# Jaureguy760/HaploHyped-VarAwareML

Measured on AMD Instinct MI355X. Metric: variants/sec encode+compress, 3M-variant x 2.5k-sample VCF, higher is better.
Workload: dtype u8

## Files before the change

### haplohyped_varawareml_amd/_lib.py

```python
import ctypes as C
import os

HERE = os.path.dirname(os.path.abspath(__file__))
LIB_PATH = os.environ.get("HHGT_LIB") or os.path.join(HERE, "libhhgt.so")

OK = 0
BLOSC1 = 1
BLOSC2 = 2
N_STAGES = 16
STAGE_NAMES = ["index", "fixed", "encode", "general", "lz4", "frame", "decode", "onehot", "inflate", "pairs", "ld_transpose",
               "ld", "ld_prune", "ld_walk", "grm", "assoc"]


class HhgtError(RuntimeError):

    def __init__(self, code, msg):
        super().__init__(f"{msg} (hhgt rc={code})")
        self.code = code


class Layout(C.Structure):
    _fields_ = [("n_samples", C.c_int32), ("sc", C.c_int32), ("vc", C.c_int32), ("ring", C.c_int32),
                ("v_capacity", C.c_uint64)]


class Window(C.Structure):
    _fields_ = [("ref_ptr", C.c_uint64), ("ref_len", C.c_uint64), ("win_start", C.c_int64),
                ("var_start_ptr", C.c_uint64), ("var_ref_ptr", C.c_uint64), ("var_alt_ptr", C.c_uint64),
                ("geno_ptr", C.c_uint64), ("geno_first", C.c_uint32), ("var_lo", C.c_uint32),
                ("var_hi", C.c_uint32), ("reserved", C.c_uint32)]


class BlockSel(C.Structure):
    _fields_ = [("src_ptr", C.c_uint64), ("src_bytes", C.c_uint64), ("dst_off", C.c_uint64), ("block", C.c_uint32),
                ("lo", C.c_uint32), ("hi", C.c_uint32), ("reserved", C.c_uint32)]


class CountSel(C.Structure):
    _fields_ = [("src_ptr", C.c_uint64), ("src_bytes", C.c_uint64), ("row_mask", C.c_uint64), ("out_row", C.c_uint64),
                ("part", C.c_uint32), ("lo", C.c_uint32), ("hi", C.c_uint32), ("reserved", C.c_uint32)]


class SampleSel(C.Structure):
    _fields_ = [("src_ptr", C.c_uint64), ("src_bytes", C.c_uint64), ("row_mask", C.c_uint64), ("out_row", C.c_uint64),
                ("mask_word", C.c_uint64), ("part", C.c_uint32), ("lo", C.c_uint32), ("hi", C.c_uint32),
                ("reserved", C.c_uint32)]


class PlaneSel(C.Structure):
    _fields_ = [("src_ptr", C.c_uint64), ("src_bytes", C.c_uint64), ("row_mask", C.c_uint64), ("out_row", C.c_uint64),
                ("mask_word", C.c_uint64), ("out_word", C.c_uint64), ("part", C.c_uint32), ("lo", C.c_uint32),
                ("hi", C.c_uint32), ("reserved", C.c_uint32)]


class GatherSel(C.Structure):
    _fields_ = [("src_ptr", C.c_uint64), ("src_bytes", C.c_uint64), ("row_mask", C.c_uint64), ("out_row", C.c_uint64),
                ("mask_word", C.c_uint64), ("out_col", C.c_uint64), ("part", C.c_uint32), ("lo", C.c_uint32),
                ("hi", C.c_uint32), ("reserved", C.c_uint32)]


class EncodeStats(C.Structure):
    _fields_ = [(n, C.c_uint64) for n in (
        "n_lines", "n_records", "n_kept", "n_drop_region", "n_drop_filter", "n_haploid_padded",
        "n_malformed", "n_general_lines", "n_chrom_runs")]

    def asdict(self):
        return {n: int(getattr(self, n)) for n, _ in self._fields_}


RESULT_RUNS = 16


class EncodeResultRec(C.Structure):
    _fields_ = [("stats", EncodeStats), ("cursor_before", C.c_uint64), ("cursor_after", C.c_uint64),
                ("n_lines_over", C.c_uint64), ("err_density", C.c_uint64), ("run_first", C.c_uint64 * RESULT_RUNS),
                ("run_names", (C.c_char * 32) * RESULT_RUNS), ("v_capacity", C.c_uint64), ("done", C.c_uint32),
                ("reserved", C.c_uint32)]

    def chrom_runs(self):
        n = min(int(self.stats.n_chrom_runs), RESULT_RUNS)
        return [(int(self.run_first[i]), bytes(self.run_names[i]).split(b"\0")[0].decode()) for i in range(n)]


_vp, _u64, _u32, _i32, _str = C.c_void_p, C.c_uint64, C.c_uint32, C.c_int, C.c_char_p
_lay, _pu64, _pi32, _pvp = C.POINTER(Layout), C.POINTER(C.c_uint64), C.POINTER(C.c_int), C.POINTER(C.c_void_p)
PROTOTYPES = {
    "hhgt_version": (_str, []),
    "hhgt_last_error": (_str, []),
    "hhgt_device_count": (_i32, []),
    "hhgt_ctx_create": (_i32, [_i32, C.POINTER(_vp)]),
    "hhgt_ctx_destroy": (None, [_vp]),
    "hhgt_layout_bytes": (_u64, [_lay]),
    "hhgt_layout_offset": (_u64, [_lay, _u32, _u64]),
    "hhgt_encode_text": (_i32, [_vp, _vp, _u64, _str, _lay, _u64, _vp, _vp, _vp, _vp, _vp, C.POINTER(EncodeStats), _vp]),
    "hhgt_encode_text_async": (_i32, [_vp, _vp, _u64, _str, _lay, _vp, _u32, _vp, _vp, _vp, _vp, _vp, _vp, _vp]),
    "hhgt_encode_text_planes_async": (_i32, [_vp, _vp, _u64, _str, _lay, _vp, _u32, _vp, _vp, _vp, _vp, _vp, _vp, _vp, _vp]),
    "hhgt_encode_result_status": (_i32, [_vp]),
    "hhgt_encode_chrom_runs": (_i32, [_vp, _u32, _vp, _vp, C.POINTER(_u32)]),
    "hhgt_pad_tail": (_i32, [_vp, _lay, _u64, _u64, _u64, _vp, _vp]),
    "hhgt_pad_tail_cursor": (_i32, [_vp, _lay, _vp, _vp, _vp]),
    "hhgt_planes_bytes": (_u64, [_lay]),
    "hhgt_pad_tail_planes": (_i32, [_vp, _lay, _u64, _u64, _u64, _vp, _vp]),
    "hhgt_pad_tail_planes_cursor": (_i32, [_vp, _lay, _vp, _vp, _vp]),
    "hhgt_compress_planes": (_i32, [_vp, _lay, _vp, _vp, _u32, _u32, _i32, _vp, _u64, _vp, _pu64, _vp]),
    "hhgt_planes_expand": (_i32, [_vp, _lay, _vp, _vp, _u32, _u32, _vp, _vp]),
    "hhgt_set_clevel": (_i32, [_vp, _i32]),
    "hhgt_reserve": (_i32, [_vp, _u64, _u32, _u64, _u64, _i32, _i32]),
    "hhgt_set_keep_multiallelic": (_i32, [_vp, _i32]),
    "hhgt_set_index_mode": (_i32, [_vp, _i32]),
    "hhgt_stream_create": (_i32, [_vp, _i32, C.POINTER(_vp)]),
    "hhgt_stream_destroy": (_i32, [_vp, _vp]),
    "hhgt_set_frame_stream": (_i32, [_vp, _vp]),
    "hhgt_compress_bound": (_u64, [_u64, _u64, _i32, _i32]),
    "hhgt_compress_chunks": (_i32, [_vp, _vp, _u64, _u64, _i32, _i32, _i32, _vp, _u64, _vp, _pu64, _vp]),
    "hhgt_decompress_chunks": (_i32, [_vp, _vp, _vp, _u64, _u64, _i32, _i32, _vp, _pu64, _vp]),
    "hhgt_decompress_blocks": (_i32, [_vp, _vp, _u32, _u64, _i32, _i32, _vp, _pu64, _vp]),
    "hhgt_count_alleles": (_i32, [_vp, _vp, _u32, _u32, _u32, _i32, _i32, _vp, _u64, _pu64, _vp]),
    "hhgt_count_samples": (_i32, [_vp, _vp, _u32, _u32, _u32, _i32, _i32, _vp, _u64, _vp, _u64, _pu64, _vp]),
    "hhgt_genotype_planes": (_i32, [_vp, _vp, _u32, _u32, _u32, _i32, _i32, _vp, _u64, _vp, _u64, _u64, _pu64, _vp]),
    "hhgt_gather_calls": (_i32, [_vp, _vp, _u32, _u32, _u32, _i32, _i32, _vp, _u64, _vp, _u64, _vp, _i32, _vp, _u64, _u64, _u64,
                                 _pu64, _vp]),
    "hhgt_pair_counts": (_i32, [_vp, _vp, _u64, _u64, _u64, _u64, _vp, _vp]),
    "hhgt_grm": (_i32, [_vp, _vp, _u64, _u64, _u64, _u64, _vp, _vp, _vp]),
    "hhgt_variant_planes": (_i32, [_vp, _vp, _u64, _u64, _u64, _u64, _vp, _vp]),
    "hhgt_ld_counts": (_i32, [_vp, _vp, _u64, _u64, _u32, _vp, _vp]),
    "hhgt_ld_prune": (_i32, [_vp, _vp, _u64, _u32, C.c_double, _vp, _vp]),
    "hhgt_ld_decisions": (_i32, [_vp, _vp, _u64, _u32, C.c_double, _vp, C.c_int64, _vp, _vp]),
    "hhgt_ld_clump": (_i32, [_vp, _vp, _u64, _u32, _vp, _vp, _vp, C.POINTER(_u32), _vp]),
    "hhgt_assoc_sums": (_i32, [_vp, _vp, _u64, _u64, _vp, _u32, _vp, _vp]),
    "hhgt_logistic_fit": (_i32, [_vp, _vp, _u64, _u64, _vp, _vp, _u32, _vp, _vp, _vp, _vp]),
    "hhgt_score_sums": (_i32, [_vp, _vp, _u64, _u64, _u64, _u64, _vp, _u32, _vp, _vp]),
    "hhgt_bgzf_scan": (_i32, [_vp, _u64, _u64, _vp, _vp, _vp, _vp, _pu64, _pu64]),
    "hhgt_inflate_members": (_i32, [_vp, _vp, _u64, _vp, _vp, _vp, _vp, _u64, _vp, _u64, _vp, _vp, _pu64, _vp]),
    "hhgt_onehot_windows": (_i32, [_vp, _vp, _u32, _u32, _vp, _i32, _vp, _vp, _vp]),
    "hhgt_onehot_bases_u8": (_i32, [_vp, _vp, _u64, _vp, _i32, _vp, _vp]),
    "hhgt_profile_enable": (_i32, [_vp, _i32]),
    "hhgt_profile_reset": (_i32, [_vp]),
    "hhgt_profile_read": (_i32, [_vp, C.POINTER(C.c_double), _pu64]),
    "hhgt_synth_render_fixed": (_i32, [_vp, _vp, _u64, _vp, _vp, _vp, _vp, _vp, _u64, _u64, _str, _i32, _u64, _vp]),
    "hhgt_synth_render_mixed": (_i32, [_vp, _vp, _u64, _vp, _vp, _vp, _vp, _vp, _vp, _u64, _u64, _str, _i32, _u64, _vp]),
    "hhgt_synth_write_bgzf": (_i32, [_str, _vp, _u64, _i32, _i32]),
    "hhgt_reader_open": (_i32, [_str, _u64, _i32, _i32, _pvp]),
    "hhgt_reader_close": (None, [_vp]),
    "hhgt_reader_is_bgzf": (_i32, [_vp]),
    "hhgt_reader_next": (_i32, [_vp, _pvp, _pu64]),
    "hhgt_reader_acquire": (_i32, [_vp, _pvp, _pu64, _pi32, _pi32]),
    "hhgt_reader_release": (_i32, [_vp, _i32]),
    "hhgt_reader_copy_async": (_i32, [_vp, _vp, _u64, _vp, _vp]),
    "hhgt_reader_stats": (_i32, [_vp, _pu64, _pu64]),
    "hhgt_reader_trim_pool": (None, []),
    "hhgt_reader_prewarm": (_i32, [_u64, _i32]),
    "hhgt_effective_cpus": (_i32, []),
    "hhgt_crc32": (_u32, [_vp, _u64]),
    "hhgt_fast_inflate": (_i32, [_vp, _u64, _vp, _u64]),
}

_lib = None


def load():
    global _lib
    if _lib is not None:
        return _lib
    import torch
    if not os.path.exists(LIB_PATH):
        raise ImportError(
            f"{LIB_PATH} is missing. Build it with `python -m haplohyped_varawareml_amd.build` "
            "(hipcc, gfx950). There is no CPU fallback for this path.")
    L = C.CDLL(LIB_PATH)
    for name, (restype, argtypes) in PROTOTYPES.items():
        fn = getattr(L, name)
        fn.restype, fn.argtypes = restype, argtypes
    _lib = L
    return L


def check(rc):
    if rc != OK:
        raise HhgtError(rc, load().hhgt_last_error().decode(errors="replace"))
```

### haplohyped_varawareml_amd/csrc/api.hip

```cpp
#include "common.h"
#include <chrono>
#include <vector>
#include <stdarg.h>
#include <stdio.h>
#include <string.h>
#include <stdlib.h>

static thread_local char g_err[512] = "";

void hhgt_set_error(const char *fmt, ...)
{
    va_list ap;
    va_start(ap, fmt);
    vsnprintf(g_err, sizeof(g_err), fmt, ap);
    va_end(ap);
}

extern "C" const char *hhgt_last_error(void) { return g_err; }
extern "C" const char *hhgt_version(void) { return "hhgt 0.1 (gfx950)"; }

extern "C" int hhgt_device_count(void)
{
    int n = 0;
    if (hipGetDeviceCount(&n) != hipSuccess) return 0;
// ... 109 lines not shown
    return on_device(c, stream, work, [&](hipStream_t st) { return timed(c, st, stage, [&] { return launch(st); }); });
}

extern "C" int hhgt_ctx_create(int device, hhgt_ctx **out)
{
    if (!out) return HHGT_ERR_ARG;
    *out = nullptr;
    int n = hhgt_device_count();
    if (n <= 0 || device < 0 || device >= n) {
        hhgt_set_error("no usable HIP device (count=%d, requested=%d): libhhgt has no CPU path", n, device);
        return HHGT_ERR_NO_DEVICE;
    }
    HIP_TRY(hipSetDevice(device));
    hhgt_ctx *c = new hhgt_ctx();
    c->device = device;
    int rc = HHGT_OK;
    hipError_t e = hipGetDeviceProperties(&c->prop, device);
    if (e != hipSuccess) {
        hhgt_set_error("hipGetDeviceProperties failed: %s", hipGetErrorString(e));
        rc = HHGT_ERR_HIP;
    } else if (strncmp(c->prop.gcnArchName, "gfx950", 6) != 0) {
        hhgt_set_error("device %d is %s; libhhgt carries gfx950 code objects only", device, c->prop.gcnArchName);
        rc = HHGT_ERR_NO_DEVICE;
    }
    if (rc == HHGT_OK && (e = hipHostMalloc(reinterpret_cast<void **>(&c->h_counters), sizeof(DevCounters), hipHostMallocDefault)) != hipSuccess) {
        hhgt_set_error("hipHostMalloc failed: %s", hipGetErrorString(e));
        rc = HHGT_ERR_HIP;
    }
    if (rc == HHGT_OK && (e = hipHostMalloc(reinterpret_cast<void **>(&c->h_result_pinned), sizeof(hhgt_encode_result), hipHostMallocDefault)) != hipSuccess) {
        hhgt_set_error("hipHostMalloc failed: %s", hipGetErrorString(e));
        rc = HHGT_ERR_HIP;
    }
    if (rc == HHGT_OK) rc = c->counters.ensure(sizeof(DevCounters));
    if (rc != HHGT_OK) {
        hhgt_ctx_destroy(c);
        return rc;
    }
    *out = c;
    return HHGT_OK;
}

extern "C" void hhgt_ctx_destroy(hhgt_ctx *c)
{
    if (!c) return;
    hipSetDevice(c->device);
    hipDeviceSynchronize();
    c->enc.each([](DevBuf &b) { b.release(); });
    DevBuf *bufs[] = {&c->counters, &c->cursor, &c->dec_bad, &c->oh_ovl, &c->oh_lut, &c->crc_x2n, &c->ld_bits, &c->score_part, &c->clump_ws};
    for (DevBuf *b : bufs) b->release();
    for (auto &w : c->cw) {
        DevBuf *wb[] = {&w.lz_scratch, &w.lz_csize, &w.lz_flags, &w.fr_bsize, &w.fr_csize, &w.fr_flags};
        for (DevBuf *b : wb) b->release();
        if (w.lz_done) hipEventDestroy(w.lz_done);
        if (w.fr_done) hipEventDestroy(w.fr_done);
    }
    if (c->h_counters) hipHostFree(c->h_counters);
    if (c->h_result_pinned) hipHostFree(c->h_result_pinned);
    for (auto &p : c->pending) {
        hipEventDestroy(p.a);
        hipEventDestroy(p.b);
    }
    for (auto e : c->event_pool) hipEventDestroy(e);
    delete c;
}

static hipEvent_t get_event(hhgt_ctx *c)
{
    if (!c->event_pool.empty()) {
        hipEvent_t e = c->event_pool.back();
        c->event_pool.pop_back();
        return e;
    }
    hipEvent_t e;
    hipEventCreate(&e);
    return e;
}

StageTimer::StageTimer(hhgt_ctx *c, hipStream_t s, int stage_) : ctx(c), st(s), stage(stage_)
{
    if (ctx->profiling) {
        a = get_event(ctx);
        b = get_event(ctx);
        hipEventRecord(a, st);
    }
}

void StageTimer::stop()
{
    if (a) {
        hipEventRecord(b, st);
        ctx->pending.push_back({stage, a, b});
        a = b = nullptr;
    }
}

int hhgt_profile_collect(hhgt_ctx *c)
{
    for (auto &p : c->pending) {
        hipEventSynchronize(p.b);
        float ms = 0.f;
        if (hipEventElapsedTime(&ms, p.a, p.b) == hipSuccess) {
            c->stage_ms[p.stage] += ms;
            c->stage_launches[p.stage] += 1;
        }
        c->event_pool.push_back(p.a);
        c->event_pool.push_back(p.b);
    }
    c->pending.clear();
    return HHGT_OK;
}

extern "C" int hhgt_profile_enable(hhgt_ctx *c, int on)
{
    if (!c) return HHGT_ERR_ARG;
    c->profiling = on ? 1 : 0;
    return HHGT_OK;
}

extern "C" int hhgt_profile_reset(hhgt_ctx *c)
{
    if (!c) return HHGT_ERR_ARG;
    hhgt_profile_collect(c);
    for (int i = 0; i < HHGT_N_STAGES; ++i) {
        c->stage_ms[i] = 0;
        c->stage_launches[i] = 0;
    }
    return HHGT_OK;
}

extern "C" int hhgt_profile_read(hhgt_ctx *c, double *ms, uint64_t *launches)
{
    if (!c) return HHGT_ERR_ARG;
    hhgt_profile_collect(c);
    for (int i = 0; i < HHGT_N_STAGES; ++i) {
        if (ms) ms[i] = c->stage_ms[i];
        if (launches) launches[i] = c->stage_launches[i];
    }
    return HHGT_OK;
}

static int make_layout(const hhgt_layout *lay, LayoutDev *L)
{
    if (!lay || lay->n_samples < 0) {
        hhgt_set_error("layout: bad n_samples");
        return HHGT_ERR_ARG;
    }
    L->S = (uint32_t)lay->n_samples;
    L->v_capacity = lay->v_capacity;
    L->ring = 0;
    L->pad_ = 0;
    if (lay->ring < 0 || (lay->ring > 0 && (lay->vc <= 0 || lay->v_capacity != (uint64_t)lay->ring * (uint64_t)lay->vc))) {
        hhgt_set_error("layout: a ring needs vc > 0 and v_capacity == ring * vc");
        return HHGT_ERR_ARG;
    }
    L->ring = (uint32_t)lay->ring;
    if (lay->vc == 0) {
        L->Vc = lay->v_capacity ? lay->v_capacity : TILE_V;
    } else {
        L->Vc = (uint64_t)lay->vc;
    }
    if (L->Vc % TILE_V) {
        hhgt_set_error("layout: variants per chunk (%llu) must be a multiple of %d (dense: v_capacity)",
                       (unsigned long long)L->Vc, TILE_V);
        return HHGT_ERR_ARG;
    }
    if (lay->v_capacity % L->Vc) {
        hhgt_set_error("layout: v_capacity must be a multiple of vc");
        return HHGT_ERR_ARG;
    }
    if (lay->sc == 0) {
        L->Sc = L->S ? L->S : 1;
        L->sc_log2 = 31;
        L->n_sc = 1;
    } else {
        uint32_t sc = (uint32_t)lay->sc;
        if (sc & (sc - 1)) {
            hhgt_set_error("layout: sc must be a power of two");
            return HHGT_ERR_ARG;
        }
        L->Sc = sc;
        uint32_t lg = 0;
        while ((1u << lg) < sc) ++lg;
        L->sc_log2 = lg;
        L->n_sc = (L->S + sc - 1) / sc;
        if (L->n_sc == 0) L->n_sc = 1;
    }
    return HHGT_OK;
}

extern "C" uint64_t hhgt_layout_bytes(const hhgt_layout *lay)
{
    LayoutDev L;
    if (make_layout(lay, &L) != HHGT_OK) return 0;
    return (uint64_t)L.n_sc * L.Sc * L.v_capacity * 2ull;
}

extern "C" uint64_t hhgt_layout_offset(const hhgt_layout *lay, uint32_t s, uint64_t v)
{
    LayoutDev L;
    if (make_layout(lay, &L) != HHGT_OK) return ~0ull;
    return layout_offset(L, s, v);
}

static int parse_region_host(const char *region, RegionFilter *rf)
{
    memset(rf, 0, sizeof(*rf));
    if (!region || !*region) return HHGT_OK;
    const char *colon = strrchr(region, ':');
    size_t clen = strlen(region);
    if (colon && colon[1] >= '0' && colon[1] <= '9') {
        char *p;
        long long b = strtoll(colon + 1, &p, 10), e = 0x7fffffffffffffffLL;
        while (*p == ',') p++;
        if (*p == '-' && p[1]) e = strtoll(p + 1, &p, 10);
        clen = (size_t)(colon - region);
        rf->has_range = 1;
        rf->beg = b;
        rf->end = e;
    }
    if (clen == 0 || clen >= sizeof(rf->contig)) {
        hhgt_set_error("region '%s': contig name empty or longer than 63 bytes", region);
        return HHGT_ERR_ARG;
    }
    memcpy(rf->contig, region, clen);
    rf->contig_len = (int)clen;
    return HHGT_OK;
}

__global__ void k_encode_finish(DevCounters *cnt, uint64_t *cursor, const uint64_t *__restrict__ run_first,
                                const uint8_t *__restrict__ run_names, uint64_t v_capacity, hhgt_encode_result *res,
                                uint32_t *region_tot, uint32_t n_region_tot)
{
    const uint32_t t = threadIdx.x;
    const uint64_t before = *cursor;
    const uint64_t kept = cnt->n_kept;
    __syncthreads();
    if (t == 0) {
        *cursor = before + kept;
        cnt->cursor_after = before + kept;
        res->stats.n_lines = cnt->n_lines;
        res->stats.n_records = cnt->n_records;
        res->stats.n_kept = kept;
        res->stats.n_drop_region = cnt->n_drop_region;
        res->stats.n_drop_filter = cnt->n_drop_filter;
        res->stats.n_haploid_padded = cnt->n_haploid;
        res->stats.n_malformed = cnt->n_malformed;
        res->stats.n_general_lines = cnt->n_general;
        res->stats.n_chrom_runs = cnt->n_chrom_runs;
        res->cursor_before = before;
        res->cursor_after = before + kept;
        res->n_lines_over = cnt->err_lines;
        res->err_density = cnt->err_density;
        res->v_capacity = v_capacity;
        res->reserved = cnt->n_other > 0xFFFFFFFFull ? 0xFFFFFFFFu : (uint32_t)cnt->n_other;
    }
    const uint64_t n_runs = cnt->n_chrom_runs;
    if (t < HHGT_RESULT_RUNS) res->run_first[t] = t < n_runs ? run_first[t] : 0ull;
    for (uint32_t q = t; q < HHGT_RESULT_RUNS * 32u; q += blockDim.x)
        res->run_names[q >> 5][q & 31u] = (q >> 5) < n_runs ? (char)run_names[q] : 0;
    __threadfence_system();
    __syncthreads();
    if (t == 0) __hip_atomic_store(&res->done, 1u, __ATOMIC_RELEASE, __HIP_MEMORY_SCOPE_SYSTEM);
    if (t < sizeof(DevCounters) / 8u) reinterpret_cast<unsigned long long *>(cnt)[t] = 0ull;
    for (uint32_t q = t; q < n_region_tot; q += blockDim.x) region_tot[q] = 0u;
}

__global__ void k_set_u64(uint64_t *p, uint64_t v) { *p = v; }

static int encode_check_args(hhgt_ctx *c, const void *d_text, uint64_t nbytes, const hhgt_layout *lay, LayoutDev *L,
                             const char *region, RegionFilter *rf, void *d_G)
{
    TRY(make_layout(lay, L));
    if (nbytes >= 0xFFFFFFF0ull) {
        hhgt_set_error("encode: text block of %llu bytes; split it below 4 GiB at a line boundary",
                       (unsigned long long)nbytes);
        return HHGT_ERR_ARG;
    }
    if (nbytes && (!d_text || (reinterpret_cast<uintptr_t>(d_text) & 15u))) {
        hhgt_set_error("encode: d_text must be a 16-byte aligned device pointer");
        return HHGT_ERR_ARG;
    }
    if (L->S > 0 && !d_G) {
        hhgt_set_error("encode: d_G is NULL");
        return HHGT_ERR_ARG;
    }
    const int rc = parse_region_host(region, rf);
    rf->keep_multi = c->keep_multi;
    return rc;
}

static uint32_t index_regions(uint64_t nbytes) { return (uint32_t)((nbytes + 1 + INDEX_REGION - 1) / INDEX_REGION); }

static int encode_begin_clean(hhgt_ctx *c, DevCounters *cnt, hipStream_t st)
{
    if (!c->counters_clean) {
        HIP_TRY(hipMemsetAsync(cnt, 0, sizeof(DevCounters), st));
        if (c->enc.region_tot.p) HIP_TRY(hipMemsetAsync(c->enc.region_tot.p, 0, c->enc.region_tot.cap, st));
    }
    c->counters_clean = false;
    return HHGT_OK;
}

static int encode_stage_index(hhgt_ctx *c, const uint8_t *text, uint64_t nbytes, uint32_t n_regions, uint32_t min_line, uint32_t S,
                              DevCounters *cnt, hipStream_t st)
{
    EncodeWs &w = c->enc;
    TRY(w.ensure_index(n_regions, st));
    return launch_index_newlines(text, nbytes, w.slots.as<uint32_t>(), w.counts.as<uint32_t>(), w.region_tot.as<uint32_t>(), n_regions,
                                 min_line, S, c->index_mode, cnt, st);
}

static int encode_stage_rest(hhgt_ctx *c, const uint8_t *text, uint64_t nbytes, uint32_t n_regions, uint32_t max_lines,
                             const RegionFilter &rf, const LayoutDev &L, const uint64_t *d_cursor, void *d_G, void *d_P, uint32_t *d_start, uint32_t *d_stop,
                             uint8_t *d_ref, uint8_t *d_alt, DevCounters *cnt, hipStream_t st)
{
    EncodeWs &w = c->enc;
    TRY(w.ensure_lines(max_lines));
    const uint32_t *nl = w.nl.as<uint32_t>(), *d_nlines = w.n_lines.as<uint32_t>();
    const LineCols l = w.line_cols(max_lines);
    const KeptCols k = w.kept_cols();
    TRY(timed(c, st, HHGT_STAGE_INDEX, [&] {
        return launch_compact_newlines(w.slots.as<uint32_t>(), w.counts.as<uint32_t>(), w.region_tot.as<uint32_t>(), n_regions,
                                       w.nl.as<uint32_t>(), max_lines, w.n_lines.as<uint32_t>(), st);
    }));
    if (max_lines == 0) return HHGT_OK;
    TRY(timed(c, st, HHGT_STAGE_FIXED, [&] {
        TRY(launch_parse_fixed(text, nbytes, nl, d_nlines, max_lines, rf, L.S, l, c->index_mode, cnt, st));
        if (chain_scanned(max_lines))
            TRY(launch_scan_exclusive_u32_pair(l.keep, l.kidx, l.cnew, l.crun, max_lines, w.scan_tmp.as<uint32_t>(), w.scan_tmp.cap / 4, st));
        return launch_compact_kept(text, nbytes, nl, d_nlines, max_lines, l, k, MAX_CHROM_RUNS, d_cursor, L.v_capacity, L.ring,
                                   d_start, d_stop, d_ref, d_alt, cnt, d_P != nullptr, st);
    }));
    if (L.S == 0) return HHGT_OK;
    TRY(timed(c, st, HHGT_STAGE_ENCODE, [&] {
        return d_P ? launch_encode_planes(text, nbytes, k.soff, k.meta, max_lines, d_cursor, L, static_cast<uint8_t *>(d_P),
                                          static_cast<int8_t *>(d_G), k.redo_list, k.redo_flag, cnt, st)
                   : launch_encode_tiles(text, nbytes, k.soff, k.meta, max_lines, d_cursor, L, static_cast<int8_t *>(d_G),
                                         k.redo_list, k.redo_flag, cnt, st);
    }));
    return timed(c, st, HHGT_STAGE_GENERAL, [&] {
        return launch_encode_general(text, nbytes, k.soff, k.lend, k.meta, k.redo_list, d_cursor, L, static_cast<int8_t *>(d_G),
                                     static_cast<uint8_t *>(d_P), cnt, c->prop.multiProcessorCount, st);
    });
}

static hhgt_encode_result *result_on_device(const hhgt_ctx *c, hhgt_encode_result *h_result)
{
    hipPointerAttribute_t a;
    if (hipPointerGetAttributes(&a, h_result) != hipSuccess) {
        (void)hipGetLastError();
        return nullptr;
    }
    if (a.type != hipMemoryTypeHost || !a.devicePointer || a.device != c->device) return nullptr;
    return static_cast<hhgt_encode_result *>(a.devicePointer);
}

static int encode_finish(hhgt_ctx *c, uint64_t *d_cursor, const LayoutDev &L, DevCounters *cnt, uint32_t n_regions,
                         hhgt_encode_result *h_result, hipStream_t st)
{
    TRY(c->enc.ensure_runs());
    const KeptCols k = c->enc.kept_cols();
    hhgt_encode_result *staging = c->enc.result.as<hhgt_encode_result>();
    hhgt_encode_result *direct = h_result ? result_on_device(c, h_result) : nullptr;
    if (h_result) h_result->done = 0u;
    hipLaunchKernelGGL(k_encode_finish, dim3(1), dim3(256), 0, st, cnt, d_cursor, k.run_first, k.run_names,
                       L.ring ? 0ull : L.v_capacity, direct ? direct : staging, c->enc.region_tot.as<uint32_t>(),
                       c->enc.region_tot.p ? chain_groups(n_regions) : 0u);
    HIP_TRY(hipGetLastError());
    c->counters_clean = true;
    if (h_result && !direct) HIP_TRY(hipMemcpyAsync(h_result, staging, sizeof(hhgt_encode_result), hipMemcpyDeviceToHost, st));
    return HHGT_OK;
}

extern "C" int hhgt_encode_result_status(const hhgt_encode_result *r)
{
    if (!r) return HHGT_ERR_ARG;
    if (!r->done) {
        hhgt_set_error("encode: the result record is not complete yet (synchronise the stream first)");
        return HHGT_ERR_ARG;
    }
    if (r->err_density) {
        hhgt_set_error("encode: more than %u newlines inside one %u-byte region (not VCF text)", INDEX_CAP, INDEX_REGION);
        return HHGT_ERR_LINE_DENSITY;
    }
    if (r->n_lines_over) {
        hhgt_set_error("encode: %llu lines beyond max_lines were not encoded", (unsigned long long)r->n_lines_over);
        return HHGT_ERR_CAPACITY;
    }
    if (r->stats.n_malformed) {
        hhgt_set_error("Error parsing VCF file: %llu malformed record(s) (too few columns, bad POS, FORMAT without GT)",
                       (unsigned long long)r->stats.n_malformed);
        return HHGT_ERR_MALFORMED;
    }
    if (r->v_capacity && r->cursor_after > r->v_capacity) {
        hhgt_set_error("encode: %llu kept records at v_base %llu exceed v_capacity %llu",
                       (unsigned long long)r->stats.n_kept, (unsigned long long)r->cursor_before,
                       (unsigned long long)r->v_capacity);
        return HHGT_ERR_CAPACITY;
    }
    if (r->stats.n_chrom_runs > MAX_CHROM_RUNS) {
        hhgt_set_error("encode: %llu CHROM runs in one text block, more than the limit of %u (a run starts at every change of CHROM "
                       "and behind every empty or header line)",
                       (unsigned long long)r->stats.n_chrom_runs, MAX_CHROM_RUNS);
        return HHGT_ERR_CAPACITY;
    }
    return HHGT_OK;
}

static void empty_result(hhgt_encode_result *r)
{
    memset(r, 0, sizeof(*r));
    r->done = 1u;
}

static int planes_check_layout(const LayoutDev &L)
{
    if (L.Vc % 4096ull) {
        hhgt_set_error("planes: variants per chunk (%llu; dense: v_capacity) must be a multiple of 4096", (unsigned long long)L.Vc);
        return HHGT_ERR_ARG;
    }
    return HHGT_OK;
}

extern "C" uint64_t hhgt_planes_bytes(const hhgt_layout *lay)
{
    LayoutDev L;
    if (make_layout(lay, &L) != HHGT_OK || planes_check_layout(L) != HHGT_OK) return 0;
    return (uint64_t)L.n_sc * L.Sc * L.v_capacity / 2ull;
}

static int planes_columns(const hhgt_layout *lay, uint32_t col0, uint32_t n_cols, LayoutDev *L, PlanesGeom *pg)
{
    TRY(make_layout(lay, L));
    TRY(planes_check_layout(*L));
    if ((uint64_t)col0 + n_cols > L->v_capacity / L->Vc) {
        hhgt_set_error("planes: columns [%u, %u) outside the layout's %llu", col0, col0 + n_cols, (unsigned long long)(L->v_capacity / L->Vc));
        return HHGT_ERR_ARG;
    }
    *pg = planes_geom(*L, col0);
    return HHGT_OK;
}

static int pad_tail_begin(hhgt_ctx *c, const void *d_buf, const hhgt_layout *lay, bool planes, LayoutDev *L)
{
    if (!c || !d_buf) return HHGT_ERR_ARG;
    HIP_TRY(hipSetDevice(c->device));
    TRY(make_layout(lay, L));
    return planes ? planes_check_layout(*L) : HHGT_OK;
}

static int pad_tail_range(const LayoutDev &L, uint64_t v_end, uint64_t vcol_end)
{
    if (v_end > L.v_capacity || vcol_end > L.v_capacity / L.Vc) {
        hhgt_set_error("pad_tail: range outside the layout");
        return HHGT_ERR_ARG;
    }
    return HHGT_OK;
}

static int encode_async_impl(hhgt_ctx *c, const void *d_text, uint64_t nbytes, const char *region, const hhgt_layout *lay,
                             uint64_t *d_cursor, uint32_t max_lines, void *d_G, void *d_P, bool planes, uint32_t *d_start,
                             uint32_t *d_stop, uint8_t *d_ref, uint8_t *d_alt, hhgt_encode_result *h_result, void *stream)
{
    if (!c || !d_cursor) return HHGT_ERR_ARG;
    hipStream_t st = reinterpret_cast<hipStream_t>(stream);
    HIP_TRY(hipSetDevice(c->device));
    LayoutDev L;
    RegionFilter rf;
    TRY(encode_check_args(c, d_text, nbytes, lay, &L, region, &rf, planes ? d_P : d_G));
    if (planes) TRY(planes_check_layout(L));
    const uint8_t *text = static_cast<const uint8_t *>(d_text);
    DevCounters *cnt = c->counters.as<DevCounters>();
    TRY(encode_begin_clean(c, cnt, st));
    const uint32_t n_regions = index_regions(nbytes);
    if (nbytes) {
        TRY(timed(c, st, HHGT_STAGE_INDEX, [&] { return encode_stage_index(c, text, nbytes, n_regions, L.S ? 2u * L.S + 17u : 0u, L.S, cnt, st); }));
        TRY(encode_stage_rest(c, text, nbytes, n_regions, max_lines, rf, L, d_cursor, d_G, planes ? d_P : nullptr, d_start, d_stop, d_ref,
                              d_alt, cnt, st));
    }
    return encode_finish(c, d_cursor, L, cnt, n_regions, h_result, st);
}

extern "C" int hhgt_encode_text_async(hhgt_ctx *c, const void *d_text, uint64_t nbytes, const char *region,
                                      const hhgt_layout *lay, uint64_t *d_cursor, uint32_t max_lines, void *d_G,
                                      uint32_t *d_start, uint32_t *d_stop, uint8_t *d_ref, uint8_t *d_alt,
                                      hhgt_encode_result *h_result, void *stream)
{
    return encode_async_impl(c, d_text, nbytes, region, lay, d_cursor, max_lines, d_G, nullptr, false, d_start, d_stop, d_ref, d_alt,
                             h_result, stream);
}

extern "C" int hhgt_encode_text_planes_async(hhgt_ctx *c, const void *d_text, uint64_t nbytes, const char *region,
                                             const hhgt_layout *lay, uint64_t *d_cursor, uint32_t max_lines, void *d_P, void *d_G,
                                             uint32_t *d_start, uint32_t *d_stop, uint8_t *d_ref, uint8_t *d_alt,
                                             hhgt_encode_result *h_result, void *stream)
{
    return encode_async_impl(c, d_text, nbytes, region, lay, d_cursor, max_lines, d_G, d_P, true, d_start, d_stop, d_ref, d_alt,
                             h_result, stream);
}

extern "C" int hhgt_pad_tail_planes(hhgt_ctx *c, const hhgt_layout *lay, uint64_t v_end, uint64_t vcol_begin, uint64_t vcol_end,
                                    void *d_P, void *stream)
{
    LayoutDev L;
    TRY(pad_tail_begin(c, d_P, lay, true, &L));
    TRY(pad_tail_range(L, v_end, vcol_end));
    return launch_pad_tail_planes(L, v_end, vcol_begin, vcol_end, static_cast<uint8_t *>(d_P), reinterpret_cast<hipStream_t>(stream));
}

extern "C" int hhgt_pad_tail_planes_cursor(hhgt_ctx *c, const hhgt_layout *lay, const uint64_t *d_cursor, void *d_P, void *stream)
{
    LayoutDev L;
    if (!d_cursor) return HHGT_ERR_ARG;
    TRY(pad_tail_begin(c, d_P, lay, true, &L));
    return launch_pad_tail_planes_cursor(L, d_cursor, static_cast<uint8_t *>(d_P), reinterpret_cast<hipStream_t>(stream));
}

extern "C" int hhgt_planes_expand(hhgt_ctx *c, const hhgt_layout *lay, const void *d_P, const void *d_G, uint32_t col0, uint32_t n_cols,
                                  void *d_out, void *stream)
{
    if (!c || !d_P || !d_out) return HHGT_ERR_ARG;
    HIP_TRY(hipSetDevice(c->device));
    LayoutDev L;
    PlanesGeom pg;
    TRY(planes_columns(lay, col0, n_cols, &L, &pg));
    if (n_cols == 0) return HHGT_OK;
    return launch_planes_expand(L, static_cast<const uint8_t *>(d_P), static_cast<const uint8_t *>(d_G), col0, n_cols,
                                static_cast<uint8_t *>(d_out), reinterpret_cast<hipStream_t>(stream));
}

static int encode_text_once(hhgt_ctx *c, const void *d_text, uint64_t nbytes, const char *region, const hhgt_layout *lay, uint64_t v_base,
                            void *d_G, uint32_t *d_start, uint32_t *d_stop, uint8_t *d_ref, uint8_t *d_alt, hhgt_encode_stats *stats,
                            void *stream);

extern "C" int hhgt_encode_text(hhgt_ctx *c, const void *d_text, uint64_t nbytes, const char *region,
                                const hhgt_layout *lay, uint64_t v_base, void *d_G, uint32_t *d_start,
                                uint32_t *d_stop, uint8_t *d_ref, uint8_t *d_alt, hhgt_encode_stats *stats,
                                void *stream)
{
    int rc = encode_text_once(c, d_text, nbytes, region, lay, v_base, d_G, d_start, d_stop, d_ref, d_alt, stats, stream);
    if (rc == HHGT_ERR_MALFORMED && c && lay && lay->n_samples >= 760) {
        const int mode = c->index_mode < 0 ? index_mode_default() : c->index_mode;
        if (mode > 0) {
            const int saved = c->index_mode;
            c->index_mode = 0;
            rc = encode_text_once(c, d_text, nbytes, region, lay, v_base, d_G, d_start, d_stop, d_ref, d_alt, stats, stream);
            c->index_mode = saved;
        }
    }
    return rc;
}

static int encode_text_once(hhgt_ctx *c, const void *d_text, uint64_t nbytes, const char *region, const hhgt_layout *lay, uint64_t v_base,
                            void *d_G, uint32_t *d_start, uint32_t *d_stop, uint8_t *d_ref, uint8_t *d_alt, hhgt_encode_stats *stats,
                            void *stream)
{
    if (!c) return HHGT_ERR_ARG;
    hipStream_t st = reinterpret_cast<hipStream_t>(stream);
    HIP_TRY(hipSetDevice(c->device));
    if (stats) memset(stats, 0, sizeof(*stats));
    LayoutDev L;
    RegionFilter rf;
    TRY(encode_check_args(c, d_text, nbytes, lay, &L, region, &rf, d_G));
    c->run_first_kept.clear();
    c->run_names_host.clear();
    if (nbytes == 0) return HHGT_OK;

    const uint8_t *text = static_cast<const uint8_t *>(d_text);
    DevCounters *cnt = c->counters.as<DevCounters>();
    TRY(c->cursor.ensure(8));
    TRY(encode_begin_clean(c, cnt, st));
    hipLaunchKernelGGL(k_set_u64, dim3(1), dim3(1), 0, st, c->cursor.as<uint64_t>(), v_base);
    const uint32_t n_regions = index_regions(nbytes);
    uint32_t n_lines = 0;
    {
        StageTimer t(c, st, HHGT_STAGE_INDEX);
        TRY(encode_stage_index(c, text, nbytes, n_regions, L.S ? 2u * L.S + 17u : 0u, L.S, cnt, st));
        std::vector<uint32_t> totals(chain_groups(n_regions));
        c->h_counters->err_density = 0;
        HIP_TRY(hipMemcpyAsync(totals.data(), c->enc.region_tot.p, totals.size() * 4, hipMemcpyDeviceToHost, st));
        HIP_TRY(hipMemcpyAsync(&c->h_counters->err_density, &cnt->err_density, 8, hipMemcpyDeviceToHost, st));
        HIP_TRY(hipStreamSynchronize(st));
        t.stop();
        for (uint32_t x : totals) n_lines += x;
        if (c->h_counters->err_density) {
            hhgt_set_error("encode: more than %u newlines inside one %u-byte region (not VCF text)", INDEX_CAP,
                           INDEX_REGION);
            return HHGT_ERR_LINE_DENSITY;
        }
    }
    if (stats) stats->n_lines = n_lines;
    if (n_lines == 0) return HHGT_OK;
    TRY(encode_stage_rest(c, text, nbytes, n_regions, n_lines, rf, L, c->cursor.as<uint64_t>(), d_G, nullptr, d_start, d_stop, d_ref,
                          d_alt, cnt, st));
    TRY(encode_finish(c, c->cursor.as<uint64_t>(), L, cnt, n_regions, c->h_result_pinned, st));
    hhgt_encode_result *hr = &c->h_result;
    HIP_TRY(hipStreamSynchronize(st));
    *hr = *c->h_result_pinned;
    if (stats) *stats = hr->stats;
    TRY(hhgt_encode_result_status(hr));
    const uint32_t n_runs = (uint32_t)hr->stats.n_chrom_runs;
    if (n_runs) {
        std::vector<uint64_t> first(n_runs);
        std::vector<char> names((size_t)n_runs * 32);
        if (n_runs <= HHGT_RESULT_RUNS) {
            memcpy(first.data(), hr->run_first, n_runs * 8);
            memcpy(names.data(), hr->run_names, (size_t)n_runs * 32);
        } else {
            HIP_TRY(hipMemcpy(first.data(), c->enc.run_first.p, (size_t)n_runs * 8, hipMemcpyDeviceToHost));
            HIP_TRY(hipMemcpy(names.data(), c->enc.run_names.p, (size_t)n_runs * 32, hipMemcpyDeviceToHost));
        }
        for (uint32_t r = 0; r < n_runs; ++r) {
            c->run_first_kept.push_back(first[r]);
            c->run_names_host.emplace_back(names.data() + (size_t)r * 32, strnlen(names.data() + (size_t)r * 32, 31));
        }
    }
    return HHGT_OK;
}

extern "C" int hhgt_encode_chrom_runs(hhgt_ctx *c, uint32_t max_runs, uint64_t *first_kept, char *names,
                                      uint32_t *n_runs)
{
    if (!c || !n_runs) return HHGT_ERR_ARG;
    uint32_t n = (uint32_t)c->run_first_kept.size();
    *n_runs = n;
    if (n > max_runs) n = max_runs;
    for (uint32_t r = 0; r < n; ++r) {
        if (first_kept) first_kept[r] = c->run_first_kept[r];
        if (names) {
            memset(names + (size_t)r * 32, 0, 32);
            size_t l = c->run_names_host[r].size() < 31 ? c->run_names_host[r].size() : 31;
            memcpy(names + (size_t)r * 32, c->run_names_host[r].data(), l);
        }
    }
    return HHGT_OK;
}

extern "C" int hhgt_pad_tail(hhgt_ctx *c, const hhgt_layout *lay, uint64_t v_end, uint64_t vcol_begin,
                             uint64_t vcol_end, void *d_G, void *stream)
{
    LayoutDev L;
    TRY(pad_tail_begin(c, d_G, lay, false, &L));
    TRY(pad_tail_range(L, v_end, vcol_end));
    return launch_pad_tail(L, v_end, vcol_begin, vcol_end, static_cast<int8_t *>(d_G),
                           reinterpret_cast<hipStream_t>(stream));
}

extern "C" int hhgt_pad_tail_cursor(hhgt_ctx *c, const hhgt_layout *lay, const uint64_t *d_cursor, void *d_G, void *stream)
{
    LayoutDev L;
    if (!d_cursor) return HHGT_ERR_ARG;
    TRY(pad_tail_begin(c, d_G, lay, false, &L));
    return launch_pad_tail_cursor(L, d_cursor, static_cast<int8_t *>(d_G), reinterpret_cast<hipStream_t>(stream));
}

static int check_codec_args(uint64_t chunk_nbytes, int typesize, int blocksize, int format)
{
    if (typesize < 1 || typesize > 255 || blocksize < 16 || blocksize > 65536 || blocksize % typesize ||
        chunk_nbytes == 0 || chunk_nbytes >= 0x7fffffffull || (format != HHGT_BLOSC1 && format != HHGT_BLOSC2)) {
        hhgt_set_error("compress: bad arguments (chunk_nbytes=%llu typesize=%d blocksize=%d format=%d)",
                       (unsigned long long)chunk_nbytes, typesize, blocksize, format);
        return HHGT_ERR_ARG;
    }
    return HHGT_OK;
}

static int effective_blocksize(uint64_t chunk_nbytes, int typesize, int blocksize)
{
    if ((uint64_t)blocksize > chunk_nbytes) {
        blocksize = (int)chunk_nbytes;
        if (typesize > 1 && blocksize >= typesize) blocksize -= blocksize % typesize;
    }
    return blocksize > 0 ? blocksize : 1;
}

static int check_decode_block(int typesize, int blocksize)
{
    if (blocksize > 65536) {
        hhgt_set_error("decode: block of %d bytes x typesize %d does not fit LDS (blocks of at most 65536 bytes)",
                       blocksize, typesize);
        return HHGT_ERR_ARG;
    }
    return HHGT_OK;
}

static void codec_geometry(uint64_t chunk_nbytes, int typesize, int blocksize, uint32_t *nblocks, uint32_t *nwaves,
                           size_t *slot_bytes)
{
    const bool split = typesize >= 2 && typesize <= 16 && blocksize / typesize >= 128;
    *nblocks = (uint32_t)((chunk_nbytes + blocksize - 1) / blocksize);
    *nwaves = split ? (uint32_t)typesize : 1u;
    size_t max_stream = split ? (size_t)blocksize / typesize : (size_t)blocksize;
    if (split && chunk_nbytes % blocksize && chunk_nbytes % blocksize > max_stream) max_stream = chunk_nbytes % blocksize;
    *slot_bytes = lz4_slot_bytes((int)max_stream);
}

extern "C" uint64_t hhgt_compress_bound(uint64_t n_chunks, uint64_t chunk_nbytes, int typesize, int blocksize)
{
    if (check_codec_args(chunk_nbytes, typesize, blocksize, HHGT_BLOSC2) != HHGT_OK) return 0;
    return n_chunks * (chunk_nbytes + 32);
}

static int compress_impl(hhgt_ctx *c, const void *d_src, const void *d_planes, PlanesGeom pg, uint64_t n_chunks, uint64_t chunk_nbytes,
                         int typesize, int blocksize, int format, void *d_dst, uint64_t dst_cap,
                         uint64_t *d_chunk_off, uint64_t *total_bytes, void *stream)
{
    if (!c || (!d_src && !d_planes) || !d_dst || !d_chunk_off) return HHGT_ERR_ARG;
    hipStream_t st = reinterpret_cast<hipStream_t>(stream);
    HIP_TRY(hipSetDevice(c->device));
    TRY(check_codec_args(chunk_nbytes, typesize, blocksize, format));
    if (total_bytes) *total_bytes = 0;
    if (n_chunks == 0) return HHGT_OK;
    if (!total_bytes && dst_cap < n_chunks * (chunk_nbytes + 32)) {
        hhgt_set_error("compress: the asynchronous form (total_bytes == NULL) needs dst_cap >= hhgt_compress_bound() = %llu, got %llu",
                       (unsigned long long)(n_chunks * (chunk_nbytes + 32)), (unsigned long long)dst_cap);
        return HHGT_ERR_CAPACITY;
    }
    blocksize = effective_blocksize(chunk_nbytes, typesize, blocksize);
    uint32_t nblocks, nwaves;
    size_t slot;
    codec_geometry(chunk_nbytes, typesize, blocksize, &nblocks, &nwaves, &slot);
    hipStream_t fst = c->frame_stream ? c->frame_stream : st;
    hhgt_ctx::CodecWs &w = c->cw[c->frame_stream ? (c->cmp_seq++ & 1u) : 0u];
    TRY(w.ensure(n_chunks, nblocks, nwaves, slot));
    if (w.fr_pending) {
        HIP_TRY(hipStreamWaitEvent(st, w.fr_done, 0));
        w.fr_pending = false;
    }
    TRY(timed(c, st, HHGT_STAGE_LZ4, [&] {
        if (!w.lz_flags.p) {
            TRY(w.lz_flags.ensure(4));
            HIP_TRY(hipMemsetAsync(w.lz_flags.p, 0, 4, st));
        }
        if (++w.lz_tag == 0) w.lz_tag = 1;
        return launch_lz4_blocks(static_cast<const uint8_t *>(d_src), static_cast<const uint8_t *>(d_planes), pg, n_chunks, chunk_nbytes,
                                 typesize, blocksize, w.lz_scratch.as<uint8_t>(), slot, w.lz_csize.as<uint32_t>(), c->clevel,
                                 w.lz_flags.as<uint32_t>(), w.lz_tag, st);
    }));
    if (fst != st) {
        if (!w.lz_done) HIP_TRY(hipEventCreateWithFlags(&w.lz_done, hipEventDisableTiming));
        if (!w.fr_done) HIP_TRY(hipEventCreateWithFlags(&w.fr_done, hipEventDisableTiming));
        HIP_TRY(hipEventRecord(w.lz_done, st));
        HIP_TRY(hipStreamWaitEvent(fst, w.lz_done, 0));
    }
    TRY(timed(c, fst, HHGT_STAGE_FRAME, [&] {
        return launch_frame(w.lz_scratch.as<uint8_t>(), slot, w.lz_csize.as<uint32_t>(), static_cast<const uint8_t *>(d_src),
                            static_cast<const uint8_t *>(d_planes), pg, n_chunks, chunk_nbytes, typesize, blocksize, format,
                            w.fr_bsize.as<uint32_t>(), w.fr_csize.as<uint64_t>(), static_cast<uint8_t *>(d_dst), dst_cap, d_chunk_off,
                            w.fr_flags.as<uint32_t>(), fst);
    }));
    if (fst != st) {
        HIP_TRY(hipEventRecord(w.fr_done, fst));
        w.fr_pending = true;
        if (total_bytes) HIP_TRY(hipStreamWaitEvent(st, w.fr_done, 0));
    }
    if (total_bytes) {
        uint64_t tot = 0;
        HIP_TRY(hipMemcpyAsync(&tot, d_chunk_off + n_chunks, 8, hipMemcpyDeviceToHost, st));
        HIP_TRY(hipStreamSynchronize(st));
        *total_bytes = tot;
        if (tot > dst_cap) {
            hhgt_set_error("compress: need %llu bytes, dst_cap is %llu", (unsigned long long)tot,
                           (unsigned long long)dst_cap);
            return HHGT_ERR_CAPACITY;
        }
    }
    return HHGT_OK;
}

extern "C" int hhgt_compress_chunks(hhgt_ctx *c, const void *d_src, uint64_t n_chunks, uint64_t chunk_nbytes,
                                    int typesize, int blocksize, int format, void *d_dst, uint64_t dst_cap,
                                    uint64_t *d_chunk_off, uint64_t *total_bytes, void *stream)
{
    if (!d_src) return HHGT_ERR_ARG;
    return compress_impl(c, d_src, nullptr, PlanesGeom{0, 0, 0, 0}, n_chunks, chunk_nbytes, typesize, blocksize, format, d_dst, dst_cap,
                         d_chunk_off, total_bytes, stream);
}

extern "C" int hhgt_compress_planes(hhgt_ctx *c, const hhgt_layout *lay, const void *d_P, const void *d_G, uint32_t col0, uint32_t n_cols,
                                    int format, void *d_dst, uint64_t dst_cap, uint64_t *d_chunk_off, uint64_t *total_bytes,
                                    void *stream)
{
    if (!c || !d_P) return HHGT_ERR_ARG;
    LayoutDev L;
    PlanesGeom pg;
    TRY(planes_columns(lay, col0, n_cols, &L, &pg));
    const uint64_t chunk_nbytes = (uint64_t)L.Sc * L.Vc * 2ull, col_bytes = chunk_nbytes * L.n_sc;
    const uint8_t *g = d_G ? static_cast<const uint8_t *>(d_G) + (uint64_t)col0 * col_bytes : nullptr;
    return compress_impl(c, g, d_P, pg, (uint64_t)n_cols * L.n_sc, chunk_nbytes, 2, 8192, format, d_dst, dst_cap, d_chunk_off, total_bytes,
                         stream);
}

extern "C" int hhgt_reserve(hhgt_ctx *c, uint64_t text_bytes, uint32_t max_lines, uint64_t n_chunks, uint64_t chunk_nbytes, int typesize,
                            int blocksize)
{
    if (!c) return HHGT_ERR_ARG;
    HIP_TRY(hipSetDevice(c->device));
    if (text_bytes) {
        const uint32_t n_regions = index_regions(text_bytes);
        TRY(c->enc.ensure_index(n_regions, nullptr));
        TRY(c->enc.ensure_lines(max_lines));
        HIP_TRY(hipStreamSynchronize(nullptr));
    }
    if (n_chunks) {
        TRY(check_codec_args(chunk_nbytes, typesize, blocksize, HHGT_BLOSC2));
        blocksize = effective_blocksize(chunk_nbytes, typesize, blocksize);
        uint32_t nblocks, nwaves;
        size_t slot;
        codec_geometry(chunk_nbytes, typesize, blocksize, &nblocks, &nwaves, &slot);
        TRY(c->cw[0].ensure(n_chunks, nblocks, nwaves, slot));
    }
    return HHGT_OK;
}

extern "C" int hhgt_set_clevel(hhgt_ctx *c, int clevel)
{
    if (!c || clevel < 1 || clevel > 9) {
        hhgt_set_error("clevel must be 1..9");
        return HHGT_ERR_ARG;
    }
    c->clevel = clevel;
    return HHGT_OK;
}

extern "C" int hhgt_stream_create(hhgt_ctx *c, int kind, void **out)
{
    if (!c || !out || (kind != HHGT_STREAM_ENCODE && kind != HHGT_STREAM_COMPRESS && kind != HHGT_STREAM_FRAME)) {
        hhgt_set_error("hhgt_stream_create: bad arguments");
        return HHGT_ERR_ARG;
    }
    HIP_TRY(hipSetDevice(c->device));
    hipStream_t st = nullptr;
    if (kind == HHGT_STREAM_FRAME) {
        HIP_TRY(hipStreamCreateWithFlags(&st, hipStreamNonBlocking));
    } else if (kind == HHGT_STREAM_ENCODE) {
        int lo = 0, hi = 0;
        HIP_TRY(hipDeviceGetStreamPriorityRange(&lo, &hi));
        HIP_TRY(hipStreamCreateWithPriority(&st, hipStreamNonBlocking, hi));
    } else {
        const uint32_t n_cu = (uint32_t)c->prop.multiProcessorCount;
        uint32_t use = n_cu >= 128u ? (n_cu * 3u / 4u) / 32u * 32u : n_cu;
        if (const char *e = getenv("HHGT_COMPRESS_CUS")) {
            const int v = atoi(e);
            use = v <= 0 || (uint32_t)v >= n_cu ? n_cu : (uint32_t)v;
        }
        if (use >= n_cu) {
            HIP_TRY(hipStreamCreateWithFlags(&st, hipStreamNonBlocking));
        } else {
            std::vector<uint32_t> mask((n_cu + 31u) / 32u, 0u);
            for (uint32_t i = n_cu - use; i < n_cu; ++i) mask[i >> 5] |= 1u << (i & 31u);
            if (hipExtStreamCreateWithCUMask(&st, (uint32_t)mask.size(), mask.data()) != hipSuccess) {
                (void)hipGetLastError();
                st = nullptr;
                HIP_TRY(hipStreamCreateWithFlags(&st, hipStreamNonBlocking));
            }
        }
    }
    *out = st;
    return HHGT_OK;
}

extern "C" int hhgt_set_frame_stream(hhgt_ctx *c, void *stream)
{
    if (!c) return HHGT_ERR_ARG;
    HIP_TRY(hipSetDevice(c->device));
    if (c->frame_stream) HIP_TRY(hipStreamSynchronize(c->frame_stream));
    for (auto &w : c->cw) w.fr_pending = false;
    c->frame_stream = reinterpret_cast<hipStream_t>(stream);
    return HHGT_OK;
}

extern "C" int hhgt_stream_destroy(hhgt_ctx *c, void *stream)
{
    if (!c) return HHGT_ERR_ARG;
    if (stream) {
        HIP_TRY(hipSetDevice(c->device));
        if (reinterpret_cast<hipStream_t>(stream) == c->frame_stream) TRY(hhgt_set_frame_stream(c, nullptr));
        HIP_TRY(hipStreamDestroy(reinterpret_cast<hipStream_t>(stream)));
    }
    return HHGT_OK;
}

extern "C" int hhgt_set_index_mode(hhgt_ctx *c, int mode)
{
    if (!c || mode < -1 || mode > 2) {
        hhgt_set_error("index mode must be -1 (default), 0 (scan), 1 (hop) or 2 (walk)");
        return HHGT_ERR_ARG;
    }
    c->index_mode = mode;
    return HHGT_OK;
}

extern "C" int hhgt_set_keep_multiallelic(hhgt_ctx *c, int on)
{
    if (!c) return HHGT_ERR_ARG;
    c->keep_multi = on ? 1 : 0;
    return HHGT_OK;
}

__global__ void k_count_nonzero_u32(const uint32_t *__restrict__ v, uint64_t n, unsigned long long *out)
{
    uint64_t i = (uint64_t)blockIdx.x * blockDim.x + threadIdx.x;
    const unsigned long long m = __ballot(i < n && v[i] != 0u);
    if ((threadIdx.x & 63u) == 0u && m) atomicAdd(out, (unsigned long long)__builtin_popcountll(m));
}

extern "C" int hhgt_inflate_members(hhgt_ctx *c, const void *d_src, uint64_t src_bytes, const uint64_t *d_comp_off,
                                    const uint32_t *d_comp_len, const uint64_t *d_out_off, const uint32_t *d_isize,
                                    uint64_t n_members, void *d_dst, uint64_t dst_bytes, const uint32_t *d_crc32,
                                    uint32_t *d_status, uint64_t *n_bad, void *stream)
{
    if (!c || !d_src || !d_comp_off || !d_comp_len || !d_out_off || !d_isize || !d_status || (!d_dst && dst_bytes))
        return HHGT_ERR_ARG;
    hipStream_t st = reinterpret_cast<hipStream_t>(stream);
    HIP_TRY(hipSetDevice(c->device));
    if (n_bad) *n_bad = 0;
    if (n_members == 0) return HHGT_OK;
    if (d_crc32 && !c->crc_x2n_ready) {
        uint32_t t[32];
        crc32_x2n_table(t);
        TRY(c->crc_x2n.ensure(sizeof(t)));
        HIP_TRY(hipMemcpy(c->crc_x2n.p, t, sizeof(t), hipMemcpyHostToDevice));
        c->crc_x2n_ready = true;
    }
    TRY(timed(c, st, HHGT_STAGE_INFLATE, [&] {
        return launch_inflate(static_cast<const uint8_t *>(d_src), src_bytes, d_comp_off, d_comp_len, d_out_off, d_isize, n_members,
                              static_cast<uint8_t *>(d_dst), dst_bytes, d_status, d_crc32, c->crc_x2n.as<uint32_t>(), st);
    }));
    if (n_bad) {
        TRY(c->dec_bad.ensure(8));
        HIP_TRY(hipMemsetAsync(c->dec_bad.p, 0, 8, st));
        hipLaunchKernelGGL(k_count_nonzero_u32, dim3((uint32_t)((n_members + 255) / 256)), dim3(256), 0, st, d_status,
                           n_members, c->dec_bad.as<unsigned long long>());
        HIP_TRY(hipGetLastError());
        uint64_t nb = 0;
        HIP_TRY(hipMemcpyAsync(&nb, c->dec_bad.p, 8, hipMemcpyDeviceToHost, st));
        HIP_TRY(hipStreamSynchronize(st));
        *n_bad = nb;
    }
    return HHGT_OK;
}

template <typename Launch>
static int with_bad_counter(hhgt_ctx *c, hipStream_t st, uint64_t *n_bad, Launch launch)
{
    TRY(c->dec_bad.ensure(8));
    HIP_TRY(hipMemsetAsync(c->dec_bad.p, 0, 8, st));
    TRY(timed(c, st, HHGT_STAGE_DECODE, [&] { return launch(c->dec_bad.as<unsigned long long>()); }));
    if (n_bad) {
        uint64_t nb = 0;
        HIP_TRY(hipMemcpyAsync(&nb, c->dec_bad.p, 8, hipMemcpyDeviceToHost, st));
        HIP_TRY(hipStreamSynchronize(st));
        *n_bad = nb;
    }
    return HHGT_OK;
}

extern "C" int hhgt_decompress_chunks(hhgt_ctx *c, const void *d_src, const uint64_t *d_chunk_off, uint64_t n_chunks,
                                      uint64_t chunk_nbytes, int typesize, int blocksize, void *d_dst,
                                      uint64_t *n_bad, void *stream)
{
    if (!c || !d_src || !d_dst || !d_chunk_off) return HHGT_ERR_ARG;
    hipStream_t st = reinterpret_cast<hipStream_t>(stream);
    HIP_TRY(hipSetDevice(c->device));
    TRY(check_decode_block(typesize, blocksize));
    TRY(check_codec_args(chunk_nbytes, typesize, blocksize, HHGT_BLOSC2));
    if (n_bad) *n_bad = 0;
    if (n_chunks == 0) return HHGT_OK;
    blocksize = effective_blocksize(chunk_nbytes, typesize, blocksize);
    return with_bad_counter(c, st, n_bad, [&](unsigned long long *d_bad) {
        return launch_decode(static_cast<const uint8_t *>(d_src), d_chunk_off, n_chunks, chunk_nbytes, typesize, blocksize,
                             static_cast<uint8_t *>(d_dst), d_bad, st);
    });
}

extern "C" int hhgt_decompress_blocks(hhgt_ctx *c, const hhgt_block_sel *d_sel, uint32_t n_sel, uint64_t chunk_nbytes,
                                      int typesize, int blocksize, void *d_dst, uint64_t *n_bad, void *stream)
{
    TRY(check_not_null("decompress_blocks", c, !n_sel ? nullptr : !d_sel ? "selection array" : !d_dst ? "destination" : nullptr));
    hipStream_t st = reinterpret_cast<hipStream_t>(stream);
    HIP_TRY(hipSetDevice(c->device));
    TRY(check_decode_block(typesize, blocksize));
    TRY(check_codec_args(chunk_nbytes, typesize, blocksize, HHGT_BLOSC2));
    if (n_bad) *n_bad = 0;
    if (n_sel == 0) return HHGT_OK;
    blocksize = effective_blocksize(chunk_nbytes, typesize, blocksize);
    return with_bad_counter(c, st, n_bad, [&](unsigned long long *d_bad) {
        return launch_decode_sel(d_sel, n_sel, chunk_nbytes, typesize, blocksize, static_cast<uint8_t *>(d_dst), d_bad, st);
    });
}

static int check_row_kernel_args(const char *who, uint32_t sc, uint32_t vc, int typesize, int blocksize)
{
    if (typesize != 2) {
        hhgt_set_error("%s: typesize %d (only 2: one diploid int8 call)", who, typesize);
        return HHGT_ERR_ARG;
    }
    if (sc < 1 || sc > 64 || vc < 1) {
        hhgt_set_error("%s: chunk of %u samples x %u variants (1 to 64 samples)", who, sc, vc);
        return HHGT_ERR_ARG;
    }
    TRY(check_codec_args((uint64_t)sc * vc * 2u, typesize, blocksize, HHGT_BLOSC2));
    if (blocksize > 8192 || ((uint64_t)vc * 2u) % (uint64_t)blocksize) {
        hhgt_set_error("%s: blocksize %d does not cut a row of %u variants into whole blocks of at most 8192 bytes", who,
                       blocksize, vc);
        return HHGT_ERR_ARG;
    }
    return HHGT_OK;
}

template <typename Launch>
static int run_row_kernel(const char *who, const char *out, hhgt_ctx *c, const void *d_sel, uint32_t n_sel, const void *d_out,
                          uint32_t sc, uint32_t vc, int typesize, int blocksize, uint64_t *n_bad, void *stream, Launch launch)
{
    TRY(check_not_null(who, c, !n_sel ? nullptr : !d_sel ? "selection array" : !d_out ? out : nullptr));
    TRY(check_row_kernel_args(who, sc, vc, typesize, blocksize));
    hipStream_t st = reinterpret_cast<hipStream_t>(stream);
    HIP_TRY(hipSetDevice(c->device));
    if (n_bad) *n_bad = 0;
    if (n_sel == 0) return HHGT_OK;
    return with_bad_counter(c, st, n_bad, [&](unsigned long long *d_bad) { return launch(d_bad, st); });
}

extern "C" int hhgt_count_alleles(hhgt_ctx *c, const hhgt_count_sel *d_sel, uint32_t n_sel, uint32_t sc, uint32_t vc,
                                  int typesize, int blocksize, uint32_t *d_counts, uint64_t n_out, uint64_t *n_bad,
                                  void *stream)
{
    return run_row_kernel("count_alleles", "counts", c, d_sel, n_sel, d_counts, sc, vc, typesize, blocksize, n_bad, stream,
                          [&](unsigned long long *d_bad, hipStream_t st) {
                              return launch_count_alleles(d_sel, n_sel, sc, vc, blocksize, d_counts, n_out, d_bad, st);
                          });
}

extern "C" int hhgt_count_samples(hhgt_ctx *c, const hhgt_sample_sel *d_sel, uint32_t n_sel, uint32_t sc, uint32_t vc,
                                  int typesize, int blocksize, const uint32_t *d_vmask, uint64_t vmask_words,
                                  uint32_t *d_counts, uint64_t n_out, uint64_t *n_bad, void *stream)
{
    return run_row_kernel("count_samples", "counts", c, d_sel, n_sel, d_counts, sc, vc, typesize, blocksize, n_bad, stream,
                          [&](unsigned long long *d_bad, hipStream_t st) {
                              return launch_count_samples(d_sel, n_sel, sc, vc, blocksize, d_vmask, vmask_words, d_counts,
                                                          n_out, d_bad, st);
                          });
}

extern "C" int hhgt_genotype_planes(hhgt_ctx *c, const hhgt_plane_sel *d_sel, uint32_t n_sel, uint32_t sc, uint32_t vc,
                                    int typesize, int blocksize, const uint32_t *d_vmask, uint64_t vmask_words,
                                    uint32_t *d_planes, uint64_t n_rows, uint64_t row_words, uint64_t *n_bad,
                                    void *stream)
{
    return run_row_kernel("genotype_planes", "planes", c, d_sel, n_sel, d_planes, sc, vc, typesize, blocksize, n_bad, stream,
                          [&](unsigned long long *d_bad, hipStream_t st) {
                              return launch_genotype_planes(d_sel, n_sel, sc, vc, blocksize, d_vmask, vmask_words, d_planes,
                                                            n_rows, row_words, d_bad, st);
                          });
}

extern "C" int hhgt_gather_calls(hhgt_ctx *c, const hhgt_gather_sel *d_sel, uint32_t n_sel, uint32_t sc, uint32_t vc,
                                 int typesize, int blocksize, const uint32_t *d_vmask, uint64_t vmask_words,
                                 const uint32_t *d_row_map, uint64_t n_map, const void *d_values, int elem_bytes,
                                 void *d_out, uint64_t n_rows, uint64_t n_cols, uint64_t row_stride, uint64_t *n_bad,
                                 void *stream)
{
    const bool table = d_values != nullptr;
    if (table ? (elem_bytes != 1 && elem_bytes != 2 && elem_bytes != 4 && elem_bytes != 8) : elem_bytes != 2) {
        hhgt_set_error("gather_calls: elem_bytes %d (%s)", elem_bytes, table ? "1, 2, 4 or 8" : "2 without a table: an allele pair");
        return HHGT_ERR_ARG;
    }
    if (row_stride < n_cols) {
        hhgt_set_error("gather_calls: row_stride %llu below n_cols %llu", (unsigned long long)row_stride, (unsigned long long)n_cols);
        return HHGT_ERR_ARG;
    }
    const uintptr_t off = (uintptr_t)elem_bytes - 1u;
    if ((reinterpret_cast<uintptr_t>(d_out) & off) || (reinterpret_cast<uintptr_t>(d_values) & off)) {
        hhgt_set_error("gather_calls: %s not aligned to elem_bytes %d", (reinterpret_cast<uintptr_t>(d_out) & off) ? "d_out" : "d_values",
                       elem_bytes);
        return HHGT_ERR_ARG;
    }
    return run_row_kernel("gather_calls", "output", c, d_sel, n_sel, d_out, sc, vc, typesize, blocksize, n_bad, stream,
                          [&](unsigned long long *d_bad, hipStream_t st) {
                              return launch_gather_calls(d_sel, n_sel, sc, vc, blocksize, d_vmask, vmask_words, d_row_map, n_map,
                                                         d_values, elem_bytes, d_out, n_rows, n_cols, row_stride, d_bad, st);
                          });
}

template <typename Launch>
static int run_plane_kernel(const char *who, int stage, hhgt_ctx *c, const char *null_arg, const char *misaligned, uint64_t n_rows,
                            uint64_t row_words, uint64_t w_lo, uint64_t w_hi, uint64_t row_limit, void *stream, Launch launch)
{
    const bool work = n_rows && w_lo < w_hi;
    TRY(check_not_null(who, c, work ? null_arg : nullptr));
    if (w_lo > w_hi || w_hi > row_words || n_rows > row_limit) {
        hhgt_set_error("%s: words [%llu, %llu) of rows of %llu words, %llu rows", who, (unsigned long long)w_lo,
                       (unsigned long long)w_hi, (unsigned long long)row_words, (unsigned long long)n_rows);
        return HHGT_ERR_ARG;
    }
    if (misaligned) {
        hhgt_set_error("%s: %s", who, misaligned);
        return HHGT_ERR_ARG;
    }
    return launch_on_device(c, stream, stage, work, launch);
}

static bool off_alignment(const void *p, uintptr_t align) { return reinterpret_cast<uintptr_t>(p) & (align - 1u); }

extern "C" int hhgt_pair_counts(hhgt_ctx *c, const uint32_t *d_planes, uint64_t n_rows, uint64_t row_words, uint64_t w_lo,
                                uint64_t w_hi, uint32_t *d_table, void *stream)
{
    return run_plane_kernel("pair_counts", HHGT_STAGE_PAIRS, c, !d_planes ? "planes" : !d_table ? "table" : nullptr,
                            off_alignment(d_table, 16) ? "the table must be 16-byte aligned" : nullptr, n_rows, row_words, w_lo, w_hi,
                            64ull * 65535ull, stream, [&](hipStream_t st) {
                                return launch_pair_counts(d_planes, (uint32_t)n_rows, row_words, w_lo, w_hi, d_table, st);
                            });
}

extern "C" int hhgt_grm(hhgt_ctx *c, const uint32_t *d_planes, uint64_t n_rows, uint64_t row_words, uint64_t w_lo, uint64_t w_hi,
                        const float *d_z, double *d_table, void *stream)
{
    return run_plane_kernel("grm", HHGT_STAGE_GRM, c, !d_planes ? "planes" : !d_z ? "weights" : !d_table ? "table" : nullptr,
                            off_alignment(d_table, 8) || off_alignment(d_z, 16)
                                ? "the table must be 8-byte aligned, the weights 16-byte aligned" : nullptr,
                            n_rows, row_words, w_lo, w_hi, 64ull * 65535ull, stream, [&](hipStream_t st) {
                                return launch_grm(d_planes, (uint32_t)n_rows, row_words, w_lo, w_hi, d_z, d_table, st);
                            });
}

extern "C" int hhgt_variant_planes(hhgt_ctx *c, const uint32_t *d_planes, uint64_t n_rows, uint64_t row_words, uint64_t w_lo,
                                   uint64_t w_hi, uint32_t *d_vplanes, void *stream)
{
    return run_plane_kernel("variant_planes", HHGT_STAGE_LD_TRANSPOSE, c, !d_planes ? "planes" : !d_vplanes ? "variant planes" : nullptr,
                            nullptr, n_rows, row_words, w_lo, w_hi, 256ull * 65535ull, stream, [&](hipStream_t st) {
                                return launch_variant_planes(d_planes, (uint32_t)n_rows, row_words, w_lo, w_hi, d_vplanes, st);
                            });
}

static int check_ld_args(const char *who, hhgt_ctx *c, uint32_t window, const double *r2, const char *null_arg, const uint32_t *d_table)
{
    if (window < 1u || window > 1024u || (r2 && !(*r2 >= 0.0 && *r2 <= 1.0))) {
        if (r2)
            hhgt_set_error("%s: window %u, r2 %g (1 to 1024, 0 to 1)", who, window, *r2);
        else
            hhgt_set_error("%s: window %u (1 to 1024)", who, window);
        return HHGT_ERR_ARG;
    }
    TRY(check_not_null(who, c, null_arg));
    if (off_alignment(d_table, 32)) {
        hhgt_set_error("%s: the table must be 32-byte aligned", who);
        return HHGT_ERR_ARG;
    }
    return HHGT_OK;
}

extern "C" int hhgt_ld_counts(hhgt_ctx *c, const uint32_t *d_vplanes, uint64_t n_var, uint64_t sw, uint32_t window,
                              uint32_t *d_table, void *stream)
{
    const bool work = n_var && sw;
    TRY(check_ld_args("ld_counts", c, window, nullptr, !work ? nullptr : !d_vplanes ? "variant planes" : !d_table ? "table" : nullptr, d_table));
    return launch_on_device(c, stream, HHGT_STAGE_LD, work,
                            [&](hipStream_t st) { return launch_ld_counts(d_vplanes, n_var, sw, window, d_table, st); });
}

extern "C" int hhgt_ld_prune(hhgt_ctx *c, const uint32_t *d_table, uint64_t n_var, uint32_t window, double r2,
                             uint8_t *d_keep, void *stream)
{
    TRY(check_ld_args("ld_prune", c, window, &r2, !n_var ? nullptr : !d_table ? "table" : !d_keep ? "keep flags" : nullptr, d_table));
    return on_device(c, stream, n_var != 0, [&](hipStream_t st) {
        TRY(c->ld_bits.ensure((size_t)n_var * ld_walk_words(window) * sizeof(uint64_t)));
        uint64_t *bits = c->ld_bits.as<uint64_t>();
        TRY(timed(c, st, HHGT_STAGE_LD_PRUNE, [&] { return launch_ld_exceeds(d_table, n_var, window, r2, bits, st); }));
        return timed(c, st, HHGT_STAGE_LD_WALK, [&] { return launch_ld_walk(bits, n_var, window, d_keep, st); });
    });
}

static int check_clump_variants(const char *who, uint64_t n_var)
{
    if (n_var <= 0x7fffffffull) return HHGT_OK;
    hhgt_set_error("%s: %llu variants (below 2^31)", who, (unsigned long long)n_var);
    return HHGT_ERR_ARG;
}

extern "C" int hhgt_ld_decisions(hhgt_ctx *c, const uint32_t *d_table, uint64_t n_var, uint32_t window, double r2,
                                 const int64_t *d_pos, int64_t max_dist, uint64_t *d_bits, void *stream)
{
    TRY(check_ld_args("ld_decisions", c, window, &r2, !n_var ? nullptr : !d_table ? "table" : !d_bits ? "link bits" : nullptr, d_table));
    TRY(check_clump_variants("ld_decisions", n_var));
    if (max_dist < 0) {
        hhgt_set_error("ld_decisions: max_dist %lld (at least 0)", (long long)max_dist);
        return HHGT_ERR_ARG;
    }
    return launch_on_device(c, stream, HHGT_STAGE_LD_PRUNE, n_var != 0, [&](hipStream_t st) {
        return launch_ld_decisions(d_table, n_var, window, r2, d_pos, max_dist, d_bits, st);
    });
}
// ... 98 lines not shown
```

### haplohyped_varawareml_amd/csrc/common.h

```cpp
#pragma once
#include <hip/hip_runtime.h>
#include <stdint.h>
#include <stddef.h>
#include <string>
#include <vector>
#include "../../include/hhgt.h"

#define HHGT_WAVE 64
#ifdef HHGT_ENC_PRIO
#define HHGT_WAVE_PRIO() __builtin_amdgcn_s_setprio(HHGT_ENC_PRIO)
#else
#define HHGT_WAVE_PRIO()
#endif

#ifdef __HIPCC__
__device__ __forceinline__ uint32_t wave_scan_sum_dpp(uint32_t x, uint32_t lane, uint32_t *total)
{
    x += (uint32_t)__builtin_amdgcn_update_dpp(0, (int)x, 0x111, 0xf, 0xf, false);
    x += (uint32_t)__builtin_amdgcn_update_dpp(0, (int)x, 0x112, 0xf, 0xf, false);
    x += (uint32_t)__builtin_amdgcn_update_dpp(0, (int)x, 0x114, 0xf, 0xf, false);
    x += (uint32_t)__builtin_amdgcn_update_dpp(0, (int)x, 0x118, 0xf, 0xf, false);
    const uint32_t t0 = (uint32_t)__builtin_amdgcn_readlane((int)x, 15);
    const uint32_t t1 = (uint32_t)__builtin_amdgcn_readlane((int)x, 31) + t0;
    const uint32_t t2 = (uint32_t)__builtin_amdgcn_readlane((int)x, 47) + t1;
    *total = (uint32_t)__builtin_amdgcn_readlane((int)x, 63) + t2;
    const uint32_t row = lane >> 4;
    return x + (row == 0u ? 0u : (row == 1u ? t0 : (row == 2u ? t1 : t2)));
}

__device__ __forceinline__ uint32_t wave_scan_sum_dpp(uint32_t x, uint32_t lane)
{
    uint32_t total;
    return wave_scan_sum_dpp(x, lane, &total);
}

__device__ __forceinline__ uint32_t wave_incl_scan(uint32_t v)
{
    const int lane = threadIdx.x & 63;
#pragma unroll
    for (int d = 1; d < 64; d <<= 1) {
        uint32_t t = __shfl_up(v, d, 64);
        if (lane >= d) v += t;
    }
    return v;
}

__device__ __forceinline__ uint32_t block_excl_scan(uint32_t v, uint32_t *total, uint32_t *sm )
{
    const int lane = threadIdx.x & 63, w = threadIdx.x >> 6;
    uint32_t inc = wave_incl_scan(v);
    if (lane == 63) sm[w] = inc;
    __syncthreads();
    uint32_t base = 0, tot = 0;
#pragma unroll
    for (int i = 0; i < 4; ++i) {
        uint32_t x = sm[i];
        if (i < w) base += x;
        tot += x;
    }
    __syncthreads();
    *total = tot;
    return base + inc - v;
}
#endif

void hhgt_set_error(const char *fmt, ...);
#define HIP_TRY(expr)                                                                      \
    do {                                                                                   \
        hipError_t _e = (expr);                                                            \
        if (_e != hipSuccess) {                                                            \
            hhgt_set_error("%s failed: %s (%s:%d)", #expr, hipGetErrorString(_e), __FILE__, \
                           __LINE__);                                                      \
            return HHGT_ERR_HIP;                                                           \
        }                                                                                  \
    } while (0)

enum : uint32_t {
    LF_RECORD = 1u,
    LF_KEEP = 2u,
    LF_FAST = 4u,
    LF_MALFORMED = 8u,
    LF_DROP_REGION = 16u,
    LF_DROP_FILTER = 32u,
    LF_CHROM_NEW = 64u,
};

struct DevCounters {
    unsigned long long n_lines;
    unsigned long long n_records;
    unsigned long long n_kept;
    unsigned long long n_drop_region;
    unsigned long long n_drop_filter;
    unsigned long long n_haploid;
    unsigned long long n_malformed;
    unsigned long long n_general;
    unsigned long long n_chrom_runs;
    unsigned long long err_density;
    unsigned long long err_lines;
    unsigned long long cursor_after;
    unsigned long long n_other;
    unsigned long long pad[3];
};

#define MAX_CHROM_RUNS 4096u

struct RegionFilter {
    char contig[64];
    int contig_len;
    int has_range;
    long long beg, end;
    int keep_multi;
};

#define INDEX_REGION 16384u
#define INDEX_CAP 1024u

#define TILE_V 128
#define TILE_S 256

struct LayoutDev {
    uint32_t S;
    uint32_t sc_log2;
    uint32_t n_sc;
    uint32_t Sc;
    uint64_t Vc;
    uint64_t v_capacity;
    uint32_t ring;
    uint32_t pad_;
};

#define PL_TILE 256u
struct PlanesGeom {
    uint32_t S_pad;
    uint32_t bpr;
    uint32_t tpc;
    uint32_t col0;
};
static inline __host__ __device__ uint64_t planes_piece(const PlanesGeom &g, uint64_t col, uint32_t tile, uint32_t kp, uint32_t row)
{
    return ((((col * g.tpc + tile) * 4ull + kp) * g.S_pad) + row) * 32ull;
}
static inline __host__ __device__ PlanesGeom planes_geom(const LayoutDev &L, uint32_t col0)
{
    PlanesGeom g;
    g.S_pad = L.n_sc * L.Sc;
    g.bpr = (uint32_t)(L.Vc >> 12);
    g.tpc = (uint32_t)(L.Vc / PL_TILE);
    g.col0 = col0;
    return g;
}
static inline __host__ __device__ void planes_block(const PlanesGeom &g, uint64_t id, uint64_t *col, uint32_t *row, uint32_t *bi)
{
    const uint64_t per_col = (uint64_t)g.S_pad * g.bpr;
    const uint64_t c = id / per_col;
    const uint32_t rem = (uint32_t)(id - c * per_col);
    *col = g.col0 + c;
    *row = rem / g.bpr;
    *bi = rem - (rem / g.bpr) * g.bpr;
}
struct PlanesDiv {
    uint32_t mul_col, sh_col;
    uint32_t mul_row, sh_row;
};
static inline __host__ __device__ void planes_recip(uint32_t d, uint32_t *mul, uint32_t *sh)
{
    uint32_t l = 0;
    while (l < 31u && (1u << l) < d) ++l;
    *mul = (uint32_t)(((1ull << (31u + l)) + d - 1u) / d);
    *sh = l;
}
static inline __host__ __device__ uint32_t planes_div32(uint32_t n, uint32_t mul, uint32_t sh)
{
    return (uint32_t)(((uint64_t)mul * (n << 1)) >> 32) >> sh;
}
static inline __host__ __device__ PlanesDiv planes_div(const PlanesGeom &g)
{
    PlanesDiv dv;
    planes_recip(g.S_pad * g.bpr, &dv.mul_col, &dv.sh_col);
    planes_recip(g.bpr, &dv.mul_row, &dv.sh_row);
    return dv;
}
static inline __host__ __device__ void planes_block32(const PlanesGeom &g, const PlanesDiv &dv, uint32_t id, uint64_t *col, uint32_t *row, uint32_t *bi)
{
    const uint32_t c = planes_div32(id, dv.mul_col, dv.sh_col);
    const uint32_t rem = id - c * (g.S_pad * g.bpr);
    const uint32_t r = planes_div32(rem, dv.mul_row, dv.sh_row);
    *col = (uint64_t)g.col0 + c;
    *row = r;
    *bi = rem - r * g.bpr;
}
static inline __host__ __device__ void planes_wg_plane(uint32_t wg, uint32_t *bid, uint32_t *h)
{
    const uint32_t r = wg & 127u, k = r >> 3;
    *bid = (wg >> 7) * 64u + (r & 7u) * 8u + (k >> 1);
    *h = k & 1u;
}
static inline __host__ __device__ uint64_t planes_lane_bytes(const PlanesGeom &g, const PlanesDiv &dv, uint32_t bid, uint32_t h, uint32_t lane)
{
    uint64_t col;
    uint32_t row, bi;
    planes_block32(g, dv, bid, &col, &row, &bi);
    return planes_piece(g, col, bi * 16u + (lane >> 2), h, row) + (lane & 3u) * 8ull;
}
static inline __host__ __device__ uint64_t planes_exc_step(const PlanesGeom &g) { return (uint64_t)g.S_pad * 64ull; }

struct DevBuf {
    void *p = nullptr;
    size_t cap = 0;
    int ensure(size_t bytes);
    void release();
    template <typename T> T *as() const { return reinterpret_cast<T *>(p); }
};

#define CHAIN_GROUP 256u
#define CHAIN_FANIN_MAX 2048u
static_assert(((0xFFFFFFF0ull + 1 + INDEX_REGION - 1) / INDEX_REGION + CHAIN_GROUP - 1) / CHAIN_GROUP <= CHAIN_FANIN_MAX,
              "the region totals of the largest text block must stay inside the fan-in bound");
static inline uint32_t chain_groups(uint32_t n) { return (n + CHAIN_GROUP - 1u) / CHAIN_GROUP; }
static inline bool chain_scanned(uint32_t max_lines) { return chain_groups(max_lines) > CHAIN_FANIN_MAX; }

struct LineCols {
    uint32_t *soff, *lend, *pos, *refalt, *flags, *tot, *keep, *kidx, *cnew, *crun;
};
struct KeptCols {
    uint32_t *soff, *lend, *meta, *redo_list, *redo_flag;
    uint64_t *run_first;
    uint8_t *run_names;
};

struct EncodeWs {
    DevBuf slots, counts, nl, scan_tmp;
    DevBuf region_tot;
    DevBuf n_lines;
    DevBuf line_tot;
    enum { L_SOFF, L_LEND, L_POS, L_REFALT, L_FLAGS, K_SOFF, K_LEND, K_META, REDO_LIST, REDO_FLAG, N_LINE };
    enum { S_KEEP, S_KIDX, S_CNEW, S_CRUN, N_SCANNED };
    DevBuf line[N_LINE];
    DevBuf scanned[N_SCANNED];
    DevBuf run_first, run_names;
    DevBuf result;
    int ensure_index(uint32_t n_regions, hipStream_t st);
    int ensure_lines(uint32_t max_lines);
    int ensure_runs();
    template <typename F> void each(F f)
    {
        for (DevBuf *b : {&slots, &counts, &nl, &scan_tmp, &region_tot, &n_lines, &line_tot, &run_first, &run_names, &result}) f(*b);
        for (DevBuf &b : line) f(b);
        for (DevBuf &b : scanned) f(b);
    }
    uint32_t *col(int i) const { return line[i].as<uint32_t>(); }
    LineCols line_cols(uint32_t max_lines) const
    {
        LineCols l;
        l.soff = col(L_SOFF), l.lend = col(L_LEND), l.pos = col(L_POS), l.refalt = col(L_REFALT), l.flags = col(L_FLAGS);
        l.tot = line_tot.as<uint32_t>();
        const bool sc = chain_scanned(max_lines);
        l.keep = sc ? scanned[S_KEEP].as<uint32_t>() : nullptr, l.kidx = sc ? scanned[S_KIDX].as<uint32_t>() : nullptr;
        l.cnew = sc ? scanned[S_CNEW].as<uint32_t>() : nullptr, l.crun = sc ? scanned[S_CRUN].as<uint32_t>() : nullptr;
        return l;
    }
    KeptCols kept_cols() const
    {
        KeptCols k;
        k.soff = col(K_SOFF), k.lend = col(K_LEND), k.meta = col(K_META), k.redo_list = col(REDO_LIST), k.redo_flag = col(REDO_FLAG);
        k.run_first = run_first.as<uint64_t>(), k.run_names = run_names.as<uint8_t>();
        return k;
    }
};

struct hhgt_ctx {
    int device = 0;
    hipDeviceProp_t prop;
    EncodeWs enc;
    DevBuf counters;
    DevBuf cursor;
    struct CodecWs {
        DevBuf lz_scratch, lz_csize, lz_flags, fr_bsize, fr_csize, fr_flags;
        uint32_t lz_tag = 0;
        hipEvent_t lz_done = nullptr, fr_done = nullptr;
        bool fr_pending = false;
        int ensure(uint64_t n_chunks, uint32_t nblocks, uint32_t nwaves, size_t slot);
    } cw[2];
    uint64_t cmp_seq = 0;
    hipStream_t frame_stream = nullptr;
    DevBuf dec_bad, oh_ovl, oh_lut, crc_x2n;
    DevBuf ld_bits;
    DevBuf score_part;
    DevBuf clump_ws;
    bool crc_x2n_ready = false;
    DevCounters *h_counters = nullptr;
    hhgt_encode_result *h_result_pinned = nullptr;
    hhgt_encode_result h_result;
    std::vector<uint64_t> run_first_kept;
    std::vector<std::string> run_names_host;
    int clevel = 5;
    int keep_multi = 0;
    int index_mode = -1;
    bool counters_clean = false;
    int profiling = 0;
    double stage_ms[HHGT_N_STAGES] = {0};
    uint64_t stage_launches[HHGT_N_STAGES] = {0};
    struct Pending { int stage; hipEvent_t a, b; };
    std::vector<Pending> pending;
    std::vector<hipEvent_t> event_pool;
};

struct StageTimer {
    hhgt_ctx *ctx;
    hipStream_t st;
    int stage;
    hipEvent_t a = nullptr, b = nullptr;
    StageTimer(hhgt_ctx *c, hipStream_t s, int stage_);
    void stop();
};
int hhgt_profile_collect(hhgt_ctx *ctx);

int launch_scan_exclusive_u32(const uint32_t *d_in, uint32_t *d_out, uint64_t n, uint32_t *d_tmp,
                              size_t tmp_elems, hipStream_t st);
int launch_scan_exclusive_u32_pair(const uint32_t *in_a, uint32_t *out_a, const uint32_t *in_b, uint32_t *out_b, uint64_t n,
                                   uint32_t *d_tmp, size_t tmp_elems, hipStream_t st);
size_t scan_tmp_elems(uint64_t n);

int launch_index_newlines(const uint8_t *d_text, uint64_t n, uint32_t *d_slots, uint32_t *d_counts, uint32_t *d_region_tot,
                          uint32_t n_regions, uint32_t min_line, uint32_t S, int mode, DevCounters *d_cnt, hipStream_t st);
int index_mode_default();
int launch_compact_newlines(const uint32_t *d_slots, const uint32_t *d_counts, const uint32_t *d_region_tot,
                            uint32_t n_regions, uint32_t *d_nl, uint32_t max_lines, uint32_t *d_nlines, hipStream_t st);
int launch_parse_fixed(const uint8_t *d_text, uint64_t n, const uint32_t *d_nl, const uint32_t *d_nlines,
                       uint32_t max_lines, const RegionFilter &region, uint32_t S, const LineCols &l, int mode,
                       DevCounters *d_cnt, hipStream_t st);
int launch_compact_kept(const uint8_t *d_text, uint64_t n, const uint32_t *d_nl, const uint32_t *d_nlines, uint32_t max_lines,
                        const LineCols &l, const KeptCols &k, uint32_t max_runs, const uint64_t *d_cursor, uint64_t v_capacity,
                        uint32_t ring, uint32_t *d_start, uint32_t *d_stop, uint8_t *d_ref, uint8_t *d_alt, DevCounters *d_cnt,
                        bool strided, hipStream_t st);

int launch_encode_tiles(const uint8_t *d_text, uint64_t n, const uint32_t *k_soff, const uint32_t *k_meta,
                        uint32_t n_lines_bound, const uint64_t *d_cursor, LayoutDev lay, int8_t *d_G,
                        uint32_t *redo_list, uint32_t *redo_flag, DevCounters *d_cnt, hipStream_t st);
int launch_encode_general(const uint8_t *d_text, uint64_t n, const uint32_t *k_soff, const uint32_t *k_lend,
                          const uint32_t *k_meta, const uint32_t *redo_list, const uint64_t *d_cursor, LayoutDev lay,
                          int8_t *d_G, uint8_t *d_P, DevCounters *d_cnt, int n_cu, hipStream_t st);
int launch_encode_planes(const uint8_t *d_text, uint64_t n, const uint32_t *k_soff, const uint32_t *k_meta,
                         uint32_t n_lines_bound, const uint64_t *d_cursor, LayoutDev lay, uint8_t *d_P, int8_t *d_G,
                         uint32_t *redo_list, uint32_t *redo_flag, DevCounters *d_cnt, hipStream_t st);
int launch_pad_tail_planes(LayoutDev lay, uint64_t v_end, uint64_t vcol_begin, uint64_t vcol_end, uint8_t *d_P, hipStream_t st);
int launch_pad_tail_planes_cursor(LayoutDev lay, const uint64_t *d_cursor, uint8_t *d_P, hipStream_t st);
int launch_planes_expand(LayoutDev lay, const uint8_t *d_P, const uint8_t *d_G, uint32_t col0, uint32_t n_cols, uint8_t *d_out, hipStream_t st);
int launch_pad_tail(LayoutDev lay, uint64_t v_end, uint64_t vcol_begin, uint64_t vcol_end, int8_t *d_G,
                    hipStream_t st);
int launch_pad_tail_cursor(LayoutDev lay, const uint64_t *d_cursor, int8_t *d_G, hipStream_t st);

size_t lz4_slot_bytes(int neblock);
int launch_lz4_blocks(const uint8_t *d_src, const uint8_t *d_planes, PlanesGeom pg, uint64_t n_chunks, uint64_t chunk_nbytes, int typesize,
                      int blocksize, uint8_t *d_scratch, size_t slot_bytes, uint32_t *d_csize, int clevel, uint32_t *d_flags, uint32_t tag,
                      hipStream_t st);
int launch_lz4_bitplanes(const uint8_t *d_src, bool planes, PlanesGeom pg, uint64_t n_blocks, uint8_t *d_scratch, size_t slot_bytes, uint32_t *d_csize,
                         int depth, uint32_t *d_flags, uint32_t tag, hipStream_t st);
int launch_frame(const uint8_t *d_scratch, size_t slot_bytes, const uint32_t *d_csize, const uint8_t *d_src, const uint8_t *d_planes,
                 PlanesGeom pg, uint64_t n_chunks, uint64_t chunk_nbytes, int typesize, int blocksize, int format,
                 uint32_t *d_bstart, uint64_t *d_chunk_csize, uint8_t *d_dst, uint64_t dst_cap,
                 uint64_t *d_chunk_off, uint32_t *d_chunk_flags, hipStream_t st);
int launch_decode(const uint8_t *d_src, const uint64_t *d_chunk_off, uint64_t n_chunks, uint64_t chunk_nbytes,
                  int typesize, int blocksize, uint8_t *d_dst, unsigned long long *d_bad, hipStream_t st);
int launch_decode_sel(const hhgt_block_sel *d_sel, uint32_t n_sel, uint64_t chunk_nbytes, int typesize, int blocksize,
                      uint8_t *d_dst, unsigned long long *d_bad, hipStream_t st);
int launch_count_alleles(const hhgt_count_sel *d_sel, uint32_t n_sel, uint32_t sc, uint32_t vc, int blocksize,
                         uint32_t *d_counts, uint64_t n_out, unsigned long long *d_bad, hipStream_t st);
int launch_count_samples(const hhgt_sample_sel *d_sel, uint32_t n_sel, uint32_t sc, uint32_t vc, int blocksize,
                         const uint32_t *d_vmask, uint64_t vmask_words, uint32_t *d_counts, uint64_t n_out,
                         unsigned long long *d_bad, hipStream_t st);
int launch_genotype_planes(const hhgt_plane_sel *d_sel, uint32_t n_sel, uint32_t sc, uint32_t vc, int blocksize,
                           const uint32_t *d_vmask, uint64_t vmask_words, uint32_t *d_planes, uint64_t n_rows,
                           uint64_t row_words, unsigned long long *d_bad, hipStream_t st);
int launch_gather_calls(const hhgt_gather_sel *d_sel, uint32_t n_sel, uint32_t sc, uint32_t vc, int blocksize,
                        const uint32_t *d_vmask, uint64_t vmask_words, const uint32_t *d_row_map, uint64_t n_map,
                        const void *d_values, int elem_bytes, void *d_out, uint64_t n_rows, uint64_t n_cols,
                        uint64_t row_stride, unsigned long long *d_bad, hipStream_t st);
int launch_pair_counts(const uint32_t *d_planes, uint32_t n_rows, uint64_t row_words, uint64_t w_lo, uint64_t w_hi,
                       uint32_t *d_table, hipStream_t st);
int launch_grm(const uint32_t *d_planes, uint32_t n_rows, uint64_t row_words, uint64_t w_lo, uint64_t w_hi, const float *d_z,
               double *d_table, hipStream_t st);
int launch_variant_planes(const uint32_t *d_planes, uint32_t n_rows, uint64_t row_words, uint64_t w_lo, uint64_t w_hi,
                          uint32_t *d_vplanes, hipStream_t st);
int launch_ld_counts(const uint32_t *d_vplanes, uint64_t n_var, uint64_t sw, uint32_t window, uint32_t *d_table,
                     hipStream_t st);
uint32_t ld_walk_words(uint32_t window);
int launch_ld_exceeds(const uint32_t *d_table, uint64_t n_var, uint32_t window, double r2, uint64_t *d_bits, hipStream_t st);
int launch_ld_walk(const uint64_t *d_bits, uint64_t n_var, uint32_t window, uint8_t *d_keep, hipStream_t st);
int launch_ld_decisions(const uint32_t *d_table, uint64_t n_var, uint32_t window, double r2, const int64_t *d_pos, int64_t max_dist,
                        uint64_t *d_bits, hipStream_t st);
#define CLUMP_BATCH 8u
struct ClumpWs {
    uint64_t *fwd, *blk;
    uint32_t *counters;
    uint8_t *state[2];
    static size_t bytes(uint64_t n, uint32_t nq) { return (size_t)n * nq * 24u + CLUMP_BATCH * 4u + 2u * (size_t)n; }
    ClumpWs(void *p, uint64_t n, uint32_t nq)
    {
        fwd = reinterpret_cast<uint64_t *>(p), blk = fwd + n * nq;
        counters = reinterpret_cast<uint32_t *>(blk + 2u * n * nq);
        state[0] = reinterpret_cast<uint8_t *>(counters + CLUMP_BATCH), state[1] = state[0] + n;
    }
};
int launch_clump_blockers(const uint64_t *d_bits, uint64_t n_var, uint32_t window, const uint32_t *d_rank, const uint8_t *d_eligible,
                          const ClumpWs &ws, hipStream_t st);
int launch_clump_round(uint64_t n_var, uint32_t window, const ClumpWs &ws, uint32_t from, uint32_t *d_counter, hipStream_t st);
int launch_clump_owners(const uint64_t *d_bits, uint64_t n_var, uint32_t window, const uint32_t *d_rank, const ClumpWs &ws,
                        uint32_t from, int32_t *d_owner, hipStream_t st);
int launch_assoc_sums(const uint32_t *d_vplanes, uint64_t n_var, uint64_t sw, const double *d_w, uint32_t n_cols,
                      double *d_sums, hipStream_t st);
int launch_logistic_fit(const uint32_t *d_vplanes, uint64_t n_var, uint64_t sw, const uint32_t *d_valid, const double *d_x,
                        uint32_t q, const double *d_y, const double *d_beta0, double *d_out, hipStream_t st);
uint64_t score_spans(uint64_t n_words);
int launch_score_sums(const uint32_t *d_planes, uint32_t n_rows, uint64_t row_words, uint64_t w_lo, uint64_t w_hi, const double *d_w,
                      uint32_t n_cols, double *d_part, double *d_sums, hipStream_t st);
int launch_inflate(const uint8_t *d_src, uint64_t src_bytes, const uint64_t *d_comp_off, const uint32_t *d_comp_len,
                   const uint64_t *d_out_off, const uint32_t *d_isize, uint64_t n_members, uint8_t *d_dst,
                   uint64_t dst_bytes, uint32_t *d_status, const uint32_t *d_crc32, const uint32_t *d_x2n, hipStream_t st);
void crc32_x2n_table(uint32_t *t );

static inline __host__ __device__ uint64_t layout_offset(const LayoutDev &L, uint32_t s, uint64_t v)
{
    uint64_t vcol = v / L.Vc, vin = v - vcol * L.Vc;
    if (L.ring) vcol %= L.ring;
    uint32_t scol = (L.sc_log2 >= 31) ? 0u : (s >> L.sc_log2);
    uint32_t sin = s - scol * L.Sc;
    return (((vcol * L.n_sc + scol) * L.Sc + sin) * L.Vc + vin) * 2ull;
}
```

### haplohyped_varawareml_amd/csrc/index.hip

```cpp
#include "common.h"

typedef uint32_t u32x4_unaligned __attribute__((ext_vector_type(4), aligned(1)));
typedef uint32_t u32x4_t __attribute__((ext_vector_type(4)));

__device__ __forceinline__ uint32_t nl_mask4(uint32_t x)
{
    uint32_t t = x ^ 0x0A0A0A0Au;
    uint32_t z = ~(((t & 0x7F7F7F7Fu) + 0x7F7F7F7Fu) | t | 0x7F7F7F7Fu);
    return (((z >> 7) * 0x01020408u) >> 24) & 0xFu;
}

__global__ __launch_bounds__(256) void k_index_newlines(const uint8_t *__restrict__ text, uint64_t n,
                                                        uint32_t *__restrict__ slots,
                                                        uint32_t *__restrict__ counts, uint32_t *__restrict__ region_tot,
                                                        uint32_t n_regions, DevCounters *cnt)
{
    HHGT_WAVE_PRIO();
    const uint32_t lane = threadIdx.x & 63u;
    const uint32_t r = blockIdx.x * 4u + (threadIdx.x >> 6);
    if (r >= n_regions) return;
    const bool virt = n > 0 && text[n - 1] != '\n';
    const uint64_t rbase = (uint64_t)r * INDEX_REGION;
    uint32_t *my = slots + (size_t)r * INDEX_CAP;
    uint32_t wcount = 0;
    bool overflow = false;
    uint32_t masks[INDEX_REGION / 1024];
#pragma unroll
    for (int it = 0; it < (int)(INDEX_REGION / 1024); ++it) {
        uint64_t g0 = rbase + (uint64_t)it * 1024u + lane * 16u;
        uint32_t m = 0;
        if (g0 + 16 <= n) {
            const u32x4_t v4 = __builtin_nontemporal_load(reinterpret_cast<const u32x4_t *>(text + g0));
            uint4 v = make_uint4(v4.x, v4.y, v4.z, v4.w);
            m = nl_mask4(v.x) | (nl_mask4(v.y) << 4) | (nl_mask4(v.z) << 8) | (nl_mask4(v.w) << 12);
        } else if (g0 <= n) {
            for (int j = 0; j < 16; ++j) {
                uint64_t g = g0 + j;
                if (g < n) {
                    if (text[g] == '\n') m |= 1u << j;
                } else if (g == n && virt)
                    m |= 1u << j;
            }
        }
        masks[it] = m;
    }
#pragma unroll
    for (int it = 0; it < (int)(INDEX_REGION / 1024); ++it) {
        uint32_t m = masks[it];
        if (__ballot(m != 0) == 0ull) continue;
        uint32_t c = __popc(m);
        uint32_t inc = c;
#pragma unroll
        for (int d = 1; d < 64; d <<= 1) {
            uint32_t t = __shfl_up(inc, d, 64);
            if (lane >= (uint32_t)d) inc += t;
        }
        uint32_t idx = wcount + inc - c;
        uint32_t g0 = (uint32_t)(rbase + (uint64_t)it * 1024u + lane * 16u);
        while (m) {
            int j = __ffs(m) - 1;
            m &= m - 1;
            if (idx < INDEX_CAP) my[idx] = g0 + (uint32_t)j;
            else overflow = true;
            ++idx;
        }
        wcount += __shfl(inc, 63, 64);
    }
    if (__ballot(overflow) != 0ull && lane == 0) atomicAdd(&cnt->err_density, 1ull);
    if (lane == 0) {
        const uint32_t c = wcount < INDEX_CAP ? wcount : INDEX_CAP;
        counts[r] = c;
        if (c) atomicAdd(&region_tot[r / CHAIN_GROUP], c);
    }
}

__device__ __forceinline__ uint32_t eq_mask4(uint32_t x, uint32_t c4)
{
    const uint32_t t = x ^ c4;
    const uint32_t z = ~(((t & 0x7F7F7F7Fu) + 0x7F7F7F7Fu) | t | 0x7F7F7F7Fu);
    return (((z >> 7) * 0x01020408u) >> 24) & 0xFu;
}

__device__ __forceinline__ uint32_t eq_mask16(const u32x4_t &v, uint32_t c4)
{
    return eq_mask4(v.x, c4) | (eq_mask4(v.y, c4) << 4) | (eq_mask4(v.z, c4) << 8) | (eq_mask4(v.w, c4) << 12);
}

__device__ __forceinline__ uint32_t head_byte(const u32x4_t &v, uint32_t off)
{
    const uint32_t q = (off >> 2) & 3u;
    const uint32_t d = q == 0u ? v.x : (q == 1u ? v.y : (q == 2u ? v.z : v.w));
    return ((uint32_t)__builtin_amdgcn_readlane((int)d, (int)(off >> 4)) >> (8u * (off & 3u))) & 0xFFu;
}

__device__ __forceinline__ uint32_t head_kth(uint32_t m16, uint32_t cum, uint32_t k)
{
    const unsigned long long b = __builtin_amdgcn_ballot_w64(cum < k && cum + (uint32_t)__popc(m16) >= k);
    const int l = __builtin_ctzll(b);
    uint32_t m = (uint32_t)__builtin_amdgcn_readlane((int)m16, l);
    const uint32_t r = k - (uint32_t)__builtin_amdgcn_readlane((int)cum, l);
    for (uint32_t i = 1; i < r; ++i) m &= m - 1u;
    return 16u * (uint32_t)l + (uint32_t)__builtin_ctz(m);
}

#ifndef WALK_BATCH
#define WALK_BATCH 1
#endif
#ifndef WALK_PF
#define WALK_PF 0
#endif
template <int U, bool WALK>
__global__ __launch_bounds__(256) void k_index_hop(const uint8_t *__restrict__ text, uint64_t n, uint32_t *__restrict__ slots,
                                                   uint32_t *__restrict__ counts, uint32_t *__restrict__ region_tot, uint32_t n_regions,
                                                   uint32_t skip, uint32_t S, DevCounters *cnt, uint32_t HOP_K)
{
    HHGT_WAVE_PRIO();
    const uint32_t lane = threadIdx.x & 63u;
    const uint32_t w = (uint32_t)__builtin_amdgcn_readfirstlane((int)(blockIdx.x * 4u + (threadIdx.x >> 6)));
    const uint32_t r_first = w * HOP_K;
    if (r_first >= n_regions) return;
    const uint32_t r_cnt = n_regions - r_first < HOP_K ? n_regions - r_first : HOP_K;
    const bool virt = n > 0 && text[n - 1] != '\n';
    const uint64_t beg = (uint64_t)r_first * INDEX_REGION;
    uint64_t endw = beg + (uint64_t)r_cnt * INDEX_REGION;
    if (endw > n + 1) endw = n + 1;
    const uint64_t last_term = virt ? n : n - 1;
    uint32_t cntv = 0;
    bool overflow = false;
    uint64_t pos = beg;
    uint64_t cand = 0, fb = 0;
    bool have_cand = false;
    uint64_t est_len = 0, pf_wb = 0;
    bool pf_valid = false;
    u32x4_t pf = u32x4_t{0u, 0u, 0u, 0u};
    auto record = [&](uint64_t q) {
        const uint32_t rr = (uint32_t)(q / INDEX_REGION), local = rr - r_first;
        const uint32_t c = (uint32_t)__builtin_amdgcn_readlane((int)cntv, (int)local);
        if (c < INDEX_CAP) {
            if (lane == 0) slots[(size_t)rr * INDEX_CAP + c] = (uint32_t)q;
        } else
            overflow = true;
        cntv += lane == local ? 1u : 0u;
    };
    bool no_batch = false, bat_off = false;
    uint32_t bat_fail = 0;
    uint64_t head_p = 0;
    bool cand_batch = false;
    bool rehead = false;
    while (have_cand || pos < endw) {
        if (WALK && WALK_BATCH && have_cand && !no_batch && !bat_off && est_len != 0ull && cand >= 40ull && cand + 3ull * est_len + 216ull <= n) {
            const uint32_t g = lane >> 4, li = lane & 15u;
            const uint64_t L0 = est_len;
            const uint8_t *wbase = text + (cand - 40ull);
            const uint64_t voff = (uint64_t)g * L0 + 16ull * li;
            const u32x4_t v = *reinterpret_cast<const u32x4_unaligned *>(wbase + voff);
            const uint32_t nlm = eq_mask16(v, 0x0A0A0A0Au), tbm = eq_mask16(v, 0x09090909u);
            const unsigned long long nlb = __builtin_amdgcn_ballot_w64(nlm != 0u);
            uint32_t og[4];
            bool vg[4];
#pragma unroll
            for (int k = 0; k < 4; ++k) {
                const uint32_t mg = (uint32_t)(nlb >> (16 * k)) & 0xFFFFu;
                vg[k] = mg != 0u;
                const int fl = 16 * k + __builtin_ctz(mg | 0x10000u);
                og[k] = 16u * ((uint32_t)fl & 15u) + (uint32_t)__builtin_ctz((uint32_t)__builtin_amdgcn_readlane((int)nlm, fl & 63) | 0x10000u);
            }
            const uint32_t o = g == 0u ? og[0] : (g == 1u ? og[1] : (g == 2u ? og[2] : og[3]));
            const uint32_t l0 = 16u * li;
            const uint32_t keep = l0 > o ? 0xFFFFu : (l0 + 15u <= o ? 0u : (0xFFFFu << (o - l0 + 1u)) & 0xFFFFu);
            const unsigned long long nl2 = __builtin_amdgcn_ballot_w64((nlm & keep) != 0u);
            const uint32_t tk = tbm & keep, tc = (uint32_t)__popc(tk);
            uint32_t incl = tc;
            incl += (uint32_t)__builtin_amdgcn_update_dpp(0, (int)incl, 0x111, 0xf, 0xf, false);
            incl += (uint32_t)__builtin_amdgcn_update_dpp(0, (int)incl, 0x112, 0xf, 0xf, false);
            incl += (uint32_t)__builtin_amdgcn_update_dpp(0, (int)incl, 0x114, 0xf, 0xf, false);
            incl += (uint32_t)__builtin_amdgcn_update_dpp(0, (int)incl, 0x118, 0xf, 0xf, false);
            const uint32_t cum = incl - tc;
            const bool has9 = cum < 9u && incl >= 9u;
            uint32_t m9 = tk;
            const uint32_t r1 = 8u - cum;
#pragma unroll
            for (uint32_t i = 0; i < 8u; ++i) m9 = i < r1 ? (m9 & (m9 - 1u)) : m9;
            const uint32_t j9 = (uint32_t)__builtin_ctz(m9 | 0x10000u) & 15u;
            const uint32_t pw = (uint32_t)__builtin_amdgcn_update_dpp(0, (int)v.w, 0x111, 0xf, 0xf, false);
            const uint32_t ptb = (uint32_t)__builtin_amdgcn_update_dpp(0, (int)tbm, 0x111, 0xf, 0xf, false);
            const uint32_t tb20 = (tbm << 4) | (ptb >> 12);
            const bool tab8 = ((tb20 >> (j9 + 1u)) & 1u) != 0u;
            const uint32_t ix = j9 + 2u, di = ix >> 2;
            const uint32_t w0 = di == 0u ? pw : (di == 1u ? v.x : (di == 2u ? v.y : (di == 3u ? v.z : v.w)));
            const uint32_t w1 = di == 0u ? v.x : (di == 1u ? v.y : (di == 2u ? v.z : v.w));
            const uint32_t gt2 = __builtin_amdgcn_alignbyte(w1, w0, ix & 3u) & 0xFFFFu;
            const bool ok9 = has9 && tab8 && gt2 == 0x5447u;
            const uint32_t t9 = l0 + j9;
            const unsigned long long b9 = __builtin_amdgcn_ballot_w64(ok9);
            uint64_t expected = cand, fbx = fb, exp_head = head_p;
            bool exp_batch = cand_batch;
            bool stop = false, handed = false;
            uint32_t advanced = 0;
#pragma unroll
            for (int k = 0; k < 4; ++k) {
                if (stop || handed) continue;
                const uint64_t nlpos = cand - 40ull + (uint64_t)k * L0 + og[k];
                const bool cr = vg[k] && og[k] != 0u && head_byte(v, 256u * (uint32_t)k + og[k] - 1u) == '\r';
                if (!vg[k] || nlpos != expected || cr) {
                    handed = true;
                    continue;
                }
                exp_head = expected;
                exp_batch = true;
                if (expected >= endw) {
                    stop = true;
                    continue;
                }
                const uint32_t bits = (uint32_t)(b9 >> (16 * k)) & 0xFFFFu;
                if (bits == 0u || ((nl2 >> (16 * k)) & 0xFFFFull) != 0ull) {
                    have_cand = false;
                    pos = expected;
                    handed = true;
                    expected = ~0ull;
                    continue;
                }
                record(expected);
                ++advanced;
                const int l9 = 16 * k + __builtin_ctz(bits);
                const uint32_t t9s = (uint32_t)__builtin_amdgcn_readlane((int)t9, l9);
                const uint64_t soff = cand - 40ull + (uint64_t)k * L0 + t9s + 1ull;
                const uint64_t nxt = soff + 4ull * S - 1ull;
                est_len = nxt - expected;
                expected = nxt;
                fbx = soff + 2ull * S - 17ull;
            }
            if (stop) break;
            if (expected != ~0ull) {
                if (expected > last_term) {
                    have_cand = false;
                    pos = fbx;
                    if (pos > last_term) pos = last_term;
                } else {
                    cand = expected;
                    fb = fbx > last_term ? last_term : fbx;
                    have_cand = true;
                }
                head_p = exp_head;
                cand_batch = exp_batch;
            }
            no_batch = handed;
            bat_fail = advanced ? 0u : bat_fail + 1u;
            bat_off = bat_fail >= 2u;
            continue;
        }
        no_batch = false;
        bool found = false, nb_have = false, have_head = false;
        uint32_t nb_reg = 0, ho = 15u;
        uint64_t p = 0;
        u32x4_t hd = u32x4_t{0u, 0u, 0u, 0u};
        if (WALK && have_cand) {
            have_cand = false;
            uint32_t c15 = 0, c14 = 0;
            const bool use_pf = pf_valid && cand >= pf_wb + 15ull && cand <= pf_wb + 79ull;
            pf_valid = false;
            if (use_pf || cand + 1009ull <= n) {
                if (use_pf) {
                    hd = pf;
                    ho = (uint32_t)(cand - pf_wb);
                } else
                    hd = *reinterpret_cast<const u32x4_unaligned *>(text + (cand - 15ull) + 16ull * lane);
                const uint64_t pred = cand + est_len;
                if (WALK_PF && est_len != 0ull && pred + 977ull <= n && cand < endw) {
                    pf_wb = pred - 47ull;
                    pf = *reinterpret_cast<const u32x4_unaligned *>(text + pf_wb + 16ull * lane);
                    pf_valid = true;
                }
                c15 = head_byte(hd, ho);
                c14 = head_byte(hd, ho - 1u);
                have_head = true;
            } else if (cand < n) {
                c15 = text[cand];
                c14 = text[cand - 1];
            } else if (cand == n && virt) {
                c15 = 0x0Au;
                c14 = text[n - 1];
            }
            if (c15 == 0x0Au && c14 != '\r') {
                found = true;
                p = cand;
            } else if (cand_batch) {
                cand_batch = false;
                rehead = true;
                found = true;
                have_head = false;
                p = head_p;
            } else {
                pos = fb;
                continue;
            }
        } else {
        const uint64_t a0 = pos & ~15ull;
        uint32_t any[U];
        u32x4_t v[U];
#pragma unroll
        for (int u = 0; u < U; ++u) {
            const uint64_t g0 = a0 + (uint64_t)u * 1024u + lane * 16u;
            uint32_t f = 0;
            v[u] = u32x4_t{0u, 0u, 0u, 0u};
            if (g0 + 16 <= n) {
                v[u] = __builtin_nontemporal_load(reinterpret_cast<const u32x4_t *>(text + g0));
                const uint32_t d[4] = {v[u].x, v[u].y, v[u].z, v[u].w};
#pragma unroll
                for (int q = 0; q < 4; ++q) {
                    const uint32_t t = d[q] ^ 0x0A0A0A0Au;
                    f |= (t - 0x01010101u) & ~t & 0x80808080u;
                }
            } else if (g0 <= n) {
                uint32_t d[4] = {0x20202020u, 0x20202020u, 0x20202020u, 0x20202020u};
                for (int j = 0; j < 16; ++j) {
                    const uint64_t g = g0 + j;
                    uint32_t ch = 0x20u;
                    if (g < n) ch = text[g];
                    else if (g == n && virt) ch = 0x0Au;
                    d[j >> 2] = (d[j >> 2] & ~(0xFFu << (8 * (j & 3)))) | (ch << (8 * (j & 3)));
                    if (ch == 0x0Au) f = 1u;
                }
                v[u] = u32x4_t{d[0], d[1], d[2], d[3]};
            }
            if (g0 + 16 <= pos) f = 0;
            any[u] = f;
        }
#pragma unroll
        for (int u = 0; u < U; ++u) {
            if (found) continue;
            unsigned long long b = __builtin_amdgcn_ballot_w64(any[u] != 0u);
            while (b != 0ull && !found) {
                const int l = __builtin_ctzll(b);
                b &= b - 1ull;
                const uint32_t x0 = (uint32_t)__builtin_amdgcn_readlane((int)v[u].x, l), x1 = (uint32_t)__builtin_amdgcn_readlane((int)v[u].y, l);
                const uint32_t x2 = (uint32_t)__builtin_amdgcn_readlane((int)v[u].z, l), x3 = (uint32_t)__builtin_amdgcn_readlane((int)v[u].w, l);
                uint32_t m = nl_mask4(x0) | (nl_mask4(x1) << 4) | (nl_mask4(x2) << 8) | (nl_mask4(x3) << 12);
                const uint64_t g0 = a0 + (uint64_t)u * 1024u + (uint64_t)l * 16u;
                if (g0 < pos) m &= ~((1u << (uint32_t)(pos - g0)) - 1u);
                if (m) {
                    found = true;
                    const uint32_t j = (uint32_t)__builtin_ctz(m);
                    p = g0 + j;
                    if (j < 15u && g0 + 16 <= n) {
                        const uint32_t k = j + 1u, dw = k >> 2;
                        const uint32_t xd = dw == 0u ? x0 : (dw == 1u ? x1 : (dw == 2u ? x2 : x3));
                        nb_reg = (xd >> (8u * (k & 3u))) & 0xFFu;
                        nb_have = true;
                    }
                }
            }
        }
        if (!found) {
            pos = a0 + (uint64_t)U * 1024u;
            continue;
        }
        }
        if (!rehead) {
            if (p >= endw) break;
            record(p);
        } else
            no_batch = true;
        rehead = false;
        bool hopped = false;
        if (WALK) {
            if (!have_head && p >= 15ull && p + 1009ull <= n) {
                hd = *reinterpret_cast<const u32x4_unaligned *>(text + (p - 15ull) + 16ull * lane);
                have_head = true;
            }
            if (have_head) {
                const uint64_t wb = p - (uint64_t)ho;
                const uint32_t nb = head_byte(hd, ho + 1u);
                const uint32_t l0 = 16u * lane;
                const uint32_t keep = l0 > ho ? 0xFFFFu : (l0 + 15u <= ho ? 0u : (0xFFFFu << (ho - l0 + 1u)) & 0xFFFFu);
                if (nb == '#' || nb == 0x0Au) {
                    pos = p + 1;
                    hopped = true;
                } else {
                    const uint32_t nlm = eq_mask16(hd, 0x0A0A0A0Au) & keep;
                    const unsigned long long nlb = __builtin_amdgcn_ballot_w64(nlm != 0u);
                    if (nlb != 0ull) {
                        const int l = __builtin_ctzll(nlb);
                        pos = wb + 16ull * (uint64_t)l + (uint64_t)__builtin_ctz((uint32_t)__builtin_amdgcn_readlane((int)nlm, l));
                        hopped = true;
                    } else {
                        const uint32_t tbm = eq_mask16(hd, 0x09090909u) & keep;
                        const uint32_t tc = (uint32_t)__popc(tbm);
                        const uint32_t incl = wave_scan_sum_dpp(tc, lane);
                        const uint32_t total = (uint32_t)__builtin_amdgcn_readlane((int)incl, 63);
                        if (total >= 9u) {
                            const uint32_t t8 = head_kth(tbm, incl - tc, 8u), t9 = head_kth(tbm, incl - tc, 9u);
                            const uint64_t soff = wb + t9 + 1ull;
                            const uint64_t lo = soff + 2ull * S - 17ull;
                            const bool gt = t9 - t8 == 3u && head_byte(hd, t8 + 1u) == 'G' && head_byte(hd, t8 + 2u) == 'T';
                            if (gt && soff + 4ull * S - 1ull <= last_term) {
                                cand = soff + 4ull * S - 1ull;
                                fb = lo;
                                have_cand = true;
                                est_len = cand - p;
                                head_p = p;
                                cand_batch = false;
                            } else {
                                pos = lo;
                            }
                            hopped = true;
                        }
                    }
                }
            }
        }
        if (!hopped) {
            uint32_t nb = 0x0Au;
            if (nb_have) nb = nb_reg;
            else if (p + 1 < n) nb = text[p + 1];
            pos = p + 1 + ((nb == '#' || nb == 0x0Au || nb == '\r') ? 0u : skip);
        }
        if (pos > last_term) pos = p + 1 > last_term ? p + 1 : last_term;
        if (have_cand && fb > last_term) fb = p + 1 > last_term ? p + 1 : last_term;
    }
    if (overflow && lane == 0) atomicAdd(&cnt->err_density, 1ull);
    const uint32_t mine = lane < r_cnt ? (cntv < INDEX_CAP ? cntv : INDEX_CAP) : 0u;
    if (lane < r_cnt) counts[r_first + lane] = mine;
    const uint32_t g0 = r_first / CHAIN_GROUP;
    const uint32_t split = (g0 + 1u) * CHAIN_GROUP - r_first;
    const uint32_t a = lane < split ? mine : 0u;
    const uint32_t sum_a = (uint32_t)__builtin_amdgcn_readlane((int)wave_scan_sum_dpp(a, lane), 63);
    const uint32_t sum_b = (uint32_t)__builtin_amdgcn_readlane((int)wave_scan_sum_dpp(mine - a, lane), 63);
    if (lane == 0) {
        if (sum_a) atomicAdd(&region_tot[g0], sum_a);
        if (sum_b) atomicAdd(&region_tot[g0 + 1u], sum_b);
    }
}

__global__ __launch_bounds__(CHAIN_GROUP) void k_compact_newlines(const uint32_t *__restrict__ slots,
                                                                  const uint32_t *__restrict__ counts,
                                                                  const uint32_t *__restrict__ region_tot,
                                                                  uint32_t n_regions, uint32_t *__restrict__ nl,
                                                                  uint32_t max_lines, uint32_t *__restrict__ d_nlines)
{
    HHGT_WAVE_PRIO();
    __shared__ uint32_t sm[8];
    const uint32_t r = blockIdx.x * CHAIN_GROUP + threadIdx.x;
    uint32_t pre = 0;
    for (uint32_t g = threadIdx.x; g < blockIdx.x; g += CHAIN_GROUP) pre += region_tot[g];
    uint32_t front, own;
    block_excl_scan(pre, &front, sm);
    const uint32_t c = r < n_regions ? counts[r] : 0u;
    const uint32_t p = front + block_excl_scan(c, &own, sm);
    if (blockIdx.x == gridDim.x - 1u && threadIdx.x == 0u) *d_nlines = front + own;
    const uint32_t *my = slots + (size_t)r * INDEX_CAP;
    for (uint32_t k = 0; k < c && p + k < max_lines; ++k) nl[p + k] = my[k];
}

__global__ __launch_bounds__(256) void k_parse_fixed(const uint8_t *__restrict__ text, uint64_t n,
                                                     const uint32_t *__restrict__ nl, const uint32_t *__restrict__ d_nlines,
                                                     uint32_t max_lines, const RegionFilter rfv, uint32_t S,
                                                     uint32_t *__restrict__ l_soff, uint32_t *__restrict__ l_lend,
                                                     uint32_t *__restrict__ l_pos, uint32_t *__restrict__ l_refalt,
                                                     uint32_t *__restrict__ l_flags, uint32_t *__restrict__ l_tot,
                                                     uint32_t *__restrict__ l_keep, uint32_t *__restrict__ l_cnew,
                                                     DevCounters *cnt, uint32_t hop_skip)
{
    static_assert(CHAIN_GROUP == 256u, "one k_parse_fixed workgroup is one group of k_compact_kept's prefix");
    HHGT_WAVE_PRIO();
    __shared__ uint32_t stage[256][17];
    const RegionFilter *rf = &rfv;
    const uint32_t i = blockIdx.x * blockDim.x + threadIdx.x;
    const uint32_t n_found = *d_nlines;
    const uint32_t n_lines = n_found < max_lines ? n_found : max_lines;
    if (i == 0) {
        cnt->n_lines = n_found;
        cnt->err_lines = n_found > max_lines ? (unsigned long long)(n_found - max_lines) : 0ull;
    }
    if (blockIdx.x * blockDim.x >= n_lines) {
        if (threadIdx.x == 0u) l_tot[blockIdx.x] = l_tot[gridDim.x + blockIdx.x] = 0u;
        if (l_keep && i < max_lines) l_keep[i] = l_cnew[i] = 0u;
        return;
    }
    uint32_t flags = 0;
    uint32_t s = 0, e = 0;
    bool staged = false;
    if (i < n_lines) {
        s = i ? nl[i - 1] + 1u : 0u;
        e = nl[i];
        staged = (uint64_t)s + 64ull <= n;
        if (staged) {
            u32x4_unaligned c[4];
#pragma unroll
            for (int k = 0; k < 4; ++k) c[k] = *reinterpret_cast<const u32x4_unaligned *>(text + s + 16 * k);
#pragma unroll
            for (int k = 0; k < 4; ++k) {
                stage[threadIdx.x][4 * k + 0] = c[k].x;
                stage[threadIdx.x][4 * k + 1] = c[k].y;
                stage[threadIdx.x][4 * k + 2] = c[k].z;
                stage[threadIdx.x][4 * k + 3] = c[k].w;
            }
        }
    }
    __syncthreads();
    const uint8_t *mine = reinterpret_cast<const uint8_t *>(stage[threadIdx.x]);
    auto rd = [&](uint32_t x) -> uint32_t { return (staged && x - s < 64u) ? (uint32_t)mine[x - s] : (uint32_t)text[x]; };
    uint32_t soff = 0, pos0 = 0, refalt = 0, gtidx = 0, stride = 0;
    if (i < n_lines) {
        if (e > s && rd(e - 1u) == '\r') --e;
        soff = e;
        if (e > s && rd(s) != '#') {
            flags = LF_RECORD;
            uint32_t fs[10];
            uint32_t nf = 0;
            uint32_t p = s;
            fs[0] = s;
            while (p < e && nf < 9) {
                if (rd(p) == '\t') fs[++nf] = p + 1;
                ++p;
            }
            bool bad = false;
            uint32_t fe[9];
#pragma unroll
            for (int k = 0; k < 9; ++k) fe[k] = (uint32_t)k < nf ? fs[k + 1] - 1u : e;
            if (nf < 7 || (S > 0 && nf < 9)) bad = true;
            if (!bad) {
                unsigned long long pos = 0;
                if (fe[1] == fs[1]) bad = true;
                for (uint32_t q = fs[1]; q < fe[1]; ++q) {
                    uint32_t c = rd(q);
                    if (c < '0' || c > '9') {
                        bad = true;
                        break;
                    }
                    pos = pos * 10ull + (c - '0');
                }
                bool in_region = true;
                if (!bad && rf->contig_len > 0) {
                    uint32_t cl = fe[0] - fs[0];
                    in_region = cl == (uint32_t)rf->contig_len;
                    for (uint32_t q = 0; in_region && q < cl; ++q)
                        in_region = rd(fs[0] + q) == (uint32_t)(uint8_t)rf->contig[q];
                    if (in_region && rf->has_range)
                        in_region = (long long)pos >= rf->beg && (long long)pos <= rf->end;
                }
                if (!bad) {
                    if (!in_region)
                        flags |= LF_DROP_REGION;
                    else {
                        uint32_t reflen = fe[3] - fs[3], altlen = fe[4] - fs[4];
                        uint32_t a = altlen >= 1 ? rd(fs[4]) : 0;
                        bool snp = reflen == 1 && altlen == 1 && (a == 'A' || a == 'C' || a == 'G' || a == 'T');
                        if (rf->keep_multi && reflen == 1 && altlen > 1 && (altlen & 1u)) {
                            snp = true;
                            for (uint32_t q = 0; snp && q < altlen; ++q) {
                                const uint32_t ch = rd(fs[4] + q);
                                snp = (q & 1u) ? ch == ',' : (ch == 'A' || ch == 'C' || ch == 'G' || ch == 'T');
                            }
                        }
                        if (!snp)
                            flags |= LF_DROP_FILTER;
                        else {
                            pos0 = (uint32_t)(pos - 1ull);
                            refalt = rd(fs[3]) | (a << 8);
                            if (S > 0) {
                                uint32_t q = fs[8], k = 0;
                                bool found = false;
                                while (q <= fe[8]) {
                                    uint32_t q2 = q;
                                    while (q2 < fe[8] && rd(q2) != ':') ++q2;
                                    if (q2 - q == 2 && rd(q) == 'G' && rd(q + 1u) == 'T') {
                                        found = true;
                                        break;
                                    }
                                    ++k;
                                    q = q2 + 1;
                                }
                                if (!found || k > 0xFFFu) bad = true;
                                gtidx = k;
                                soff = fs[9];
                                if (!bad) {
                                    flags |= LF_KEEP;
                                    if (k == 0 && fe[8] - fs[8] == 2 && e - soff == 4u * S - 1u) flags |= LF_FAST;
                                    else if (k == 0 && (e - soff + 1u) % S == 0u) {
                                        const uint32_t wd = (e - soff + 1u) / S;
                                        if (wd >= 5u && wd <= 8u) stride = wd;
                                    }
                                }
                            } else {
                                flags |= LF_KEEP;
                            }
                        }
                    }
                }
            }
            if (bad) flags = LF_RECORD | LF_MALFORMED;
            bool cnew = true;
            if (i > 0) {
                uint32_t ps = i > 1 ? nl[i - 2] + 1u : 0u;
                uint32_t pe = nl[i - 1];
                const bool pstaged = threadIdx.x > 0u && (uint64_t)ps + 64ull <= n;
                const uint8_t *prev = reinterpret_cast<const uint8_t *>(stage[threadIdx.x > 0u ? threadIdx.x - 1u : 0u]);
                auto rdp = [&](uint32_t x) -> uint32_t { return (pstaged && x - ps < 64u) ? (uint32_t)prev[x - ps] : (uint32_t)text[x]; };
                if (pe > ps && rdp(ps) != '#') {
                    uint32_t q = 0;
                    cnew = false;
                    for (;;) {
                        uint32_t a = fs[0] + q < e ? rd(fs[0] + q) : '\t';
                        uint32_t b = ps + q < pe ? rdp(ps + q) : '\t';
                        if (a != b) {
                            cnew = true;
                            break;
                        }
                        if (a == '\t') break;
                        ++q;
                    }
                }
            }
            if (cnew) flags |= LF_CHROM_NEW;
        }
    }
    if (hop_skip) {
        const uint32_t lane = threadIdx.x & 63u;
        const bool chk = (flags & LF_RECORD) && !(flags & (LF_KEEP | LF_MALFORMED));
        unsigned long long todo = __ballot(chk);
        while (todo != 0ull) {
            const int l = __builtin_ctzll(todo);
            todo &= todo - 1ull;
            const uint32_t ss = (uint32_t)__builtin_amdgcn_readlane((int)s, l), ee = (uint32_t)__builtin_amdgcn_readlane((int)e, l);
            const uint32_t hi = ee - ss < hop_skip ? ee : ss + hop_skip;
            uint32_t hit = 0;
            for (uint32_t x0 = ss + 16u * lane; x0 < hi; x0 += 8192u) {
                u32x4_t tv[8];
#pragma unroll
                for (int u = 0; u < 8; ++u) {
                    const uint32_t x = x0 + 1024u * (uint32_t)u;
                    tv[u] = u32x4_t{0u, 0u, 0u, 0u};
                    if (x < hi && (uint64_t)x + 16ull <= n) tv[u] = *reinterpret_cast<const u32x4_unaligned *>(text + x);
                }
#pragma unroll
                for (int u = 0; u < 8; ++u) {
                    const uint32_t x = x0 + 1024u * (uint32_t)u;
                    if (x >= hi) continue;
                    uint32_t d[4] = {tv[u].x, tv[u].y, tv[u].z, tv[u].w};
                    if ((uint64_t)x + 16ull > n)
                        for (uint32_t k = 0; k < 16u && (uint64_t)x + k < n; ++k) d[k >> 2] |= (uint32_t)text[x + k] << (8u * (k & 3u));
                    const uint32_t m = nl_mask4(d[0]) | (nl_mask4(d[1]) << 4) | (nl_mask4(d[2]) << 8) | (nl_mask4(d[3]) << 12);
                    hit |= hi - x >= 16u ? m : (m & ((1u << (hi - x)) - 1u));
                }
            }
            if (__ballot(hit != 0u) != 0ull && (int)lane == l) flags = (flags & LF_CHROM_NEW) | LF_RECORD | LF_MALFORMED;
        }
    }
    if (i < n_lines) {
        l_soff[i] = soff;
        l_lend[i] = e;
        l_pos[i] = pos0;
        l_refalt[i] = refalt | ((gtidx & 0xFFFu) << 16) | (stride << 28);
        l_flags[i] = flags;
    }
    if (l_keep && i < max_lines) {
        l_keep[i] = (flags & LF_KEEP) ? 1u : 0u;
        l_cnew[i] = (flags & LF_CHROM_NEW) ? 1u : 0u;
    }
    __shared__ uint32_t s_stat[6];
    const uint32_t lane = threadIdx.x & 63u;
    if (threadIdx.x < 6u) s_stat[threadIdx.x] = 0u;
    __syncthreads();
    const uint32_t kinds[6] = {LF_RECORD, LF_DROP_REGION, LF_DROP_FILTER, LF_MALFORMED, LF_KEEP, LF_CHROM_NEW};
#pragma unroll
    for (int k = 0; k < 6; ++k) {
        const unsigned long long b = __ballot(flags & kinds[k]);
        if (lane == 0 && b) atomicAdd(&s_stat[k], (uint32_t)__popcll(b));
    }
    __syncthreads();
    if (threadIdx.x < 4u && s_stat[threadIdx.x]) {
        unsigned long long *dst = threadIdx.x == 0u ? &cnt->n_records : (threadIdx.x == 1u ? &cnt->n_drop_region : (threadIdx.x == 2u ? &cnt->n_drop_filter : &cnt->n_malformed));
        atomicAdd(dst, (unsigned long long)s_stat[threadIdx.x]);
    }
    if (threadIdx.x == 4u) l_tot[blockIdx.x] = s_stat[4];
    if (threadIdx.x == 5u) l_tot[gridDim.x + blockIdx.x] = s_stat[5];
}

template <bool SCANNED>
__global__ __launch_bounds__(CHAIN_GROUP) void k_compact_kept(
    const uint8_t *__restrict__ text, uint64_t n, const uint32_t *__restrict__ nl, const uint32_t *__restrict__ d_nlines,
    uint32_t max_lines, const uint32_t *__restrict__ l_soff,
    const uint32_t *__restrict__ l_lend, const uint32_t *__restrict__ l_pos, const uint32_t *__restrict__ l_refalt,
    const uint32_t *__restrict__ l_flags, const uint32_t *__restrict__ l_tot, const uint32_t *__restrict__ l_kidx,
    const uint32_t *__restrict__ l_crun,
    uint32_t *__restrict__ k_soff, uint32_t *__restrict__ k_lend, uint32_t *__restrict__ k_meta,
    uint32_t *__restrict__ redo_list, uint32_t *__restrict__ redo_flag, uint64_t *__restrict__ run_first, uint8_t *__restrict__ run_names,
    uint32_t max_runs, const uint64_t *__restrict__ d_cursor, uint64_t v_capacity, uint32_t ring, uint32_t *__restrict__ d_start,
    uint32_t *__restrict__ d_stop, uint8_t *__restrict__ d_ref, uint8_t *__restrict__ d_alt, DevCounters *cnt, uint32_t strided)
{
    HHGT_WAVE_PRIO();
    const uint32_t i = blockIdx.x * CHAIN_GROUP + threadIdx.x;
    const uint32_t n_found = *d_nlines;
    const uint32_t n_lines = n_found < max_lines ? n_found : max_lines;
    if (blockIdx.x * CHAIN_GROUP >= n_lines) return;
    const bool live = i < n_lines;
    const uint32_t flags = live ? l_flags[i] : 0u;
    uint32_t kidx, crun;
    if (SCANNED) {
        kidx = live ? l_kidx[i] : 0u;
        crun = live ? l_crun[i] : 0u;
    } else {
        __shared__ uint32_t sm[8];
        uint32_t pre_k = 0, pre_c = 0;
        for (uint32_t g = threadIdx.x; g < blockIdx.x; g += CHAIN_GROUP) {
            pre_k += l_tot[g];
            pre_c += l_tot[gridDim.x + g];
        }
        uint32_t front_k, front_c, own;
        block_excl_scan(pre_k, &front_k, sm);
        block_excl_scan(pre_c, &front_c, sm);
        const uint32_t ex = block_excl_scan(((flags & LF_KEEP) ? 1u : 0u) | ((flags & LF_CHROM_NEW) ? 0x10000u : 0u), &own, sm);
        kidx = front_k + (ex & 0xFFFFu);
        crun = front_c + (ex >> 16);
    }
    if (i == n_lines - 1) {
        cnt->n_kept = (unsigned long long)kidx + ((flags & LF_KEEP) ? 1u : 0u);
        cnt->n_chrom_runs = (unsigned long long)crun + ((flags & LF_CHROM_NEW) ? 1u : 0u);
    }
    const uint64_t v_base = *d_cursor;
    if (flags & LF_CHROM_NEW) {
        uint32_t rid = crun;
        if (rid < max_runs) {
            run_first[rid] = kidx;
            const uint32_t s0 = i ? nl[i - 1] + 1u : 0u;
            uint8_t *nm = run_names + (size_t)rid * 32u;
            uint32_t q = 0;
            for (; q < 31u && (uint64_t)s0 + q < n; ++q) {
                const uint8_t ch = text[s0 + q];
                if (ch == '\t' || ch == '\n') break;
                nm[q] = ch;
            }
            for (; q < 32u; ++q) nm[q] = 0;
        }
    }
    const bool keep = (flags & LF_KEEP) != 0u;
    const bool slow = keep && !(flags & LF_FAST) && !(strided && (l_refalt[live ? i : 0u] >> 28) != 0u);
    const unsigned long long sm = __ballot(slow);
    unsigned long long slot0 = 0ull;
    if (sm != 0ull) {
        const uint32_t lane = threadIdx.x & 63u;
        const int leader = __builtin_ctzll(sm);
        unsigned long long base = 0ull;
        if ((int)lane == leader) base = atomicAdd(&cnt->n_general, (unsigned long long)__popcll(sm));
        base = (unsigned long long)__shfl((long long)base, leader, 64);
        slot0 = base + (unsigned long long)__popcll(sm & ((1ull << lane) - 1ull));
    }
    if (!keep) return;
    const uint32_t k = kidx;
    uint64_t v = v_base + k;
    const uint32_t ra = l_refalt[i];
    k_soff[k] = l_soff[i];
    k_lend[k] = l_lend[i];
    k_meta[k] = (flags & LF_FAST) | ((ra >> 16) << 8);
    redo_flag[k] = 0u;
    if (slow) redo_list[slot0] = k;
    if (ring) v %= v_capacity;
    if (v < v_capacity) {
        uint32_t pos0 = l_pos[i];
        if (d_start) d_start[v] = pos0;
        if (d_stop) d_stop[v] = pos0 + 1u;
        if (d_ref) d_ref[v] = (uint8_t)(ra & 0xFFu);
        if (d_alt) d_alt[v] = (uint8_t)((ra >> 8) & 0xFFu);
    }
}

int index_mode_default()
{
    static const int m = [] {
        if (const char *e = getenv("HHGT_INDEX_MODE")) return atoi(e);
        if (const char *e = getenv("HHGT_INDEX_HOP")) return atoi(e) ? 2 : 0;
        return 2;
    }();
    return m < 0 ? 0 : (m > 2 ? 2 : m);
}

static uint32_t index_hop_skip(uint32_t min_line, int mode)
{
    if (mode < 0) mode = index_mode_default();
    return mode && min_line >= 1536u ? min_line - 16u : 0u;
}

int launch_index_newlines(const uint8_t *d_text, uint64_t n, uint32_t *d_slots, uint32_t *d_counts, uint32_t *d_region_tot,
                          uint32_t n_regions, uint32_t min_line, uint32_t S, int mode, DevCounters *d_cnt, hipStream_t st)
{
    if (mode < 0) mode = index_mode_default();
    if (const uint32_t skip = index_hop_skip(min_line, mode)) {
        const bool walk = mode >= 2 && S > 0;
        const uint32_t k_walk = (n_regions + 8191u) / 8192u;
        uint32_t K = walk ? (k_walk < 6u ? 6u : k_walk) : 6u;
        K = K > 64u ? 64u : K;
#define HOP_LAUNCH(U, W)                                                                                                      \
    hipLaunchKernelGGL((k_index_hop<U, W>), dim3(((n_regions + K - 1) / K + 3) / 4), dim3(256), 0, st, d_text, n, d_slots, d_counts, \
                       d_region_tot, n_regions, skip, S, d_cnt, K)
        if (min_line >= 4096u) {
            if (walk) HOP_LAUNCH(5, true);
            else HOP_LAUNCH(5, false);
        } else {
            if (walk) HOP_LAUNCH(3, true);
            else HOP_LAUNCH(3, false);
        }
#undef HOP_LAUNCH
        HIP_TRY(hipGetLastError());
        return HHGT_OK;
    }
    hipLaunchKernelGGL(k_index_newlines, dim3((n_regions + 3) / 4), dim3(256), 0, st, d_text, n, d_slots,
                       d_counts, d_region_tot, n_regions, d_cnt);
    HIP_TRY(hipGetLastError());
    return HHGT_OK;
}

int launch_compact_newlines(const uint32_t *d_slots, const uint32_t *d_counts, const uint32_t *d_region_tot,
                            uint32_t n_regions, uint32_t *d_nl, uint32_t max_lines, uint32_t *d_nlines, hipStream_t st)
{
    hipLaunchKernelGGL(k_compact_newlines, dim3(chain_groups(n_regions)), dim3(CHAIN_GROUP), 0, st, d_slots, d_counts,
                       d_region_tot, n_regions, d_nl, max_lines, d_nlines);
    HIP_TRY(hipGetLastError());
    return HHGT_OK;
}

int launch_parse_fixed(const uint8_t *d_text, uint64_t n, const uint32_t *d_nl, const uint32_t *d_nlines,
                       uint32_t max_lines, const RegionFilter &region, uint32_t S, const LineCols &l, int mode,
                       DevCounters *d_cnt, hipStream_t st)
{
    if (max_lines == 0) return HHGT_OK;
    if (mode < 0) mode = index_mode_default();
    uint32_t hop_skip = index_hop_skip(S ? 2u * S + 17u : 0u, mode);
    if (hop_skip && mode >= 2) hop_skip = 0xFFFFFFFFu;
    hipLaunchKernelGGL(k_parse_fixed, dim3(chain_groups(max_lines)), dim3(CHAIN_GROUP), 0, st, d_text, n, d_nl, d_nlines,
                       max_lines, region, S, l.soff, l.lend, l.pos, l.refalt, l.flags, l.tot, l.keep, l.cnew, d_cnt, hop_skip);
    HIP_TRY(hipGetLastError());
    return HHGT_OK;
}

int launch_compact_kept(const uint8_t *d_text, uint64_t n, const uint32_t *d_nl, const uint32_t *d_nlines, uint32_t max_lines,
                        const LineCols &l, const KeptCols &k, uint32_t max_runs, const uint64_t *d_cursor, uint64_t v_capacity,
                        uint32_t ring, uint32_t *d_start, uint32_t *d_stop, uint8_t *d_ref, uint8_t *d_alt, DevCounters *d_cnt,
                        bool strided, hipStream_t st)
{
    if (max_lines == 0) return HHGT_OK;
#define KEPT_LAUNCH(SCANNED)                                                                                                         \
    hipLaunchKernelGGL(k_compact_kept<SCANNED>, dim3(chain_groups(max_lines)), dim3(CHAIN_GROUP), 0, st, d_text, n, d_nl, d_nlines, \
                       max_lines, l.soff, l.lend, l.pos, l.refalt, l.flags, l.tot, l.kidx, l.crun, k.soff, k.lend, k.meta,          \
                       k.redo_list, k.redo_flag, k.run_first, k.run_names, max_runs, d_cursor, v_capacity, ring, d_start, d_stop,   \
                       d_ref, d_alt, d_cnt, strided ? 1u : 0u)
    if (chain_scanned(max_lines)) KEPT_LAUNCH(true);
    else KEPT_LAUNCH(false);
#undef KEPT_LAUNCH
    HIP_TRY(hipGetLastError());
    return HHGT_OK;
}
```

### haplohyped_varawareml_amd/device.py

```python
import collections
import ctypes as C
from dataclasses import dataclass, field

import numpy as np
import torch

from . import _lib
from ._lib import BLOSC1, BLOSC2, EncodeResultRec, EncodeStats, HhgtError, Layout, check

DEFAULT_SC = 64
DEFAULT_VC = 8192
DEFAULT_TYPESIZE = 2
DEFAULT_BLOCKSIZE = 8192


SEL_DTYPE = np.dtype(_lib.BlockSel)
COUNT_SEL_DTYPE = np.dtype(_lib.CountSel)
SAMPLE_SEL_DTYPE = np.dtype(_lib.SampleSel)
PLANE_SEL_DTYPE = np.dtype(_lib.PlaneSel)
GATHER_SEL_DTYPE = np.dtype(_lib.GatherSel)

GATHER_DTYPES = (torch.int8, torch.uint8, torch.int16, torch.float16, torch.bfloat16, torch.int32, torch.float32,
                 torch.int64, torch.float64)


def make_ring_layout(n_samples, ring_cols, sc=DEFAULT_SC, vc=DEFAULT_VC):
    return Layout(int(n_samples), int(sc), int(vc), int(ring_cols), int(ring_cols) * int(vc))


class PendingEncode:

    def __init__(self):
        self.buf = torch.zeros(C.sizeof(EncodeResultRec), dtype=torch.uint8).pin_memory()
        self.rec = EncodeResultRec.from_address(self.buf.data_ptr())
        self.event = torch.cuda.Event()

    def wait(self):
        self.event.synchronize()
        check(_lib.load().hhgt_encode_result_status(C.c_void_p(self.buf.data_ptr())))
        return self.rec


def make_layout(n_samples, v_capacity, sc=DEFAULT_SC, vc=DEFAULT_VC):
    if vc:
        v_capacity = -(-max(int(v_capacity), 1) // vc) * vc
    else:
        v_capacity = -(-max(int(v_capacity), 1) // 128) * 128
    return Layout(int(n_samples), int(sc), int(vc), 0, int(v_capacity))


def layout_bytes(lay):
    return int(_lib.load().hhgt_layout_bytes(C.byref(lay)))


def planes_bytes(lay):
    return int(_lib.load().hhgt_planes_bytes(C.byref(lay)))


def _ptr(t):
    return C.c_void_p(t.data_ptr()) if t is not None else None


def _ptr_if_any(t):
    return _ptr(t) if t.numel() else None


_Geometry = collections.namedtuple("_Geometry", "Vc Sc n_vc n_sc")


def _geometry(lay):
    Vc, Sc = lay.vc or lay.v_capacity, lay.sc or max(lay.n_samples, 1)
    return _Geometry(Vc, Sc, lay.v_capacity // Vc if Vc else 0, -(-lay.n_samples // Sc) if lay.sc else 1)


def _default_blocksize(nbytes, typesize=1):
    blocksize = min(int(nbytes), DEFAULT_BLOCKSIZE)
    return blocksize - blocksize % typesize


def _planes_arg(planes, what="planes: a contiguous int32 tensor [3, n_rows, row_words]"):
    if (planes.dtype not in (torch.int32, torch.uint32) or planes.dim() != 3 or planes.shape[0] != 3
            or not planes.is_contiguous()):
        raise ValueError(what)
    return int(planes.shape[1]), int(planes.shape[2])


def _plane_words(planes, w_lo, w_hi):
    n, words = _planes_arg(planes)
    return n, words, int(w_lo), words if w_hi is None else int(w_hi)


def _weights_arg(w, lead, planes):
    if (w.dtype != torch.float64 or w.dim() != len(lead) + 1 or tuple(w.shape[:-1]) != lead or not w.is_contiguous()
            or w.device != planes.device):
        raise ValueError(f"w: a contiguous float64 tensor [{', '.join(map(str, lead))}, n_cols] on the planes' device")
    n_cols = int(w.shape[-1])
    if not 0 <= n_cols < 1 << 32:
        raise ValueError(f"n_cols {n_cols}")
    return n_cols


def _stream():
    return C.c_void_p(torch.cuda.current_stream().cuda_stream)


@dataclass
class EncodeResult:
    G: torch.Tensor
    layout: Layout
    start: torch.Tensor
    stop: torch.Tensor
    ref: torch.Tensor
    alt: torch.Tensor
    n_kept: int
    stats: dict
    chrom_runs: list = field(default_factory=list)
    P: torch.Tensor = None

    def dense(self):
        lay = self.layout
        S, n = lay.n_samples, self.n_kept
        if lay.sc == 0 and lay.vc == 0:
            return self.G.view(torch.int8).view(max(S, 1), lay.v_capacity, 2)[:S, :n]
        Vc, Sc, n_vc, n_sc = _geometry(lay)
        g = self.G.view(torch.int8).view(n_vc, n_sc, Sc, Vc, 2).permute(1, 2, 0, 3, 4)
        return g.reshape(n_sc * Sc, n_vc * Vc, 2)[:S, :n]


def bgzf_scan(raw):
    from ._lib import load
    lib = load()
    data = np.frombuffer(raw, dtype=np.uint8) if isinstance(raw, (bytes, bytearray, memoryview)) else np.ascontiguousarray(raw, dtype=np.uint8)
    offs, lens, isz, crcs = [], [], [], []
    pos, cap = 0, 1 << 16
    while pos < data.size:
        co = np.zeros(cap, dtype=np.uint64)
        cl = np.zeros(cap, dtype=np.uint32)
        iz = np.zeros(cap, dtype=np.uint32)
        cr = np.zeros(cap, dtype=np.uint32)
        n, used = C.c_uint64(0), C.c_uint64(0)
        check(lib.hhgt_bgzf_scan(C.c_void_p(data.ctypes.data + pos), data.size - pos, cap, C.c_void_p(co.ctypes.data),
                                 C.c_void_p(cl.ctypes.data), C.c_void_p(iz.ctypes.data), C.c_void_p(cr.ctypes.data),
                                 C.byref(n), C.byref(used)))
        if n.value == 0:
            break
        offs.append(co[:n.value] + np.uint64(pos))
        lens.append(cl[:n.value])
        isz.append(iz[:n.value])
        crcs.append(cr[:n.value])
        pos += used.value
    cat = lambda parts, dt: np.concatenate(parts) if parts else np.zeros(0, dtype=dt)
    return dict(data=data, comp_off=cat(offs, np.uint64), comp_len=cat(lens, np.uint32), isize=cat(isz, np.uint32),
                crc32=cat(crcs, np.uint32), consumed=pos)


class Context:

    def __init__(self, device=0):
        self.lib = _lib.load()
        if not torch.cuda.is_available():
            raise HhgtError(-6, "no HIP device visible to torch: libhhgt has no CPU path")
        self.device = torch.device("cuda", device)
        h = C.c_void_p()
        check(self.lib.hhgt_ctx_create(device, C.byref(h)))
        self.h = h
        self.clevel = 5

    def close(self):
        if getattr(self, "h", None):
            for st in getattr(self, "_streams", []):
                self.lib.hhgt_stream_destroy(self.h, st)
            self._streams = []
            self.lib.hhgt_ctx_destroy(self.h)
            self.h = None

    def __del__(self):
        try:
            self.close()
        except Exception:
            pass

    def encode_text(self, text, n_samples, region="", layout=None, v_base=0, out=None):
        assert text.is_cuda and text.dtype == torch.uint8 and text.is_contiguous()
        nbytes = text.numel()
        with torch.cuda.device(self.device):
            if out is None:
                if layout is None:
                    bound = nbytes // (16 + 2 * max(n_samples, 0)) + 1
                    layout = make_layout(n_samples, bound)
                G = torch.zeros(max(layout_bytes(layout), 16), dtype=torch.uint8, device=self.device)
                cap = layout.v_capacity
                start = torch.zeros(cap, dtype=torch.int32, device=self.device)
                stop = torch.zeros(cap, dtype=torch.int32, device=self.device)
                ref = torch.zeros(cap, dtype=torch.uint8, device=self.device)
                alt = torch.zeros(cap, dtype=torch.uint8, device=self.device)
                out = EncodeResult(G, layout, start, stop, ref, alt, 0, {})
            st = EncodeStats()
            rc = self.lib.hhgt_encode_text(self.h, _ptr(text), nbytes, (region or "").encode(),
                                           C.byref(out.layout), int(v_base), _ptr(out.G), _ptr(out.start),
                                           _ptr(out.stop), _ptr(out.ref), _ptr(out.alt), C.byref(st), _stream())
            check(rc)
            out.stats = st.asdict()
            out.n_kept = int(v_base) + int(st.n_kept)
            out.chrom_runs = self.chrom_runs()
        return out

    def _encode_async(self, planes, text, n_samples, out, cursor, max_lines, region, pending):
        assert text.is_cuda and text.dtype == torch.uint8 and text.is_contiguous() and (out.P is not None or not planes)
        nbytes = text.numel()
        if max_lines is None:
            max_lines = nbytes // (16 + 2 * max(n_samples, 0)) + 64
        pending = pending or PendingEncode()
        fn, mats = (self.lib.hhgt_encode_text_planes_async, (_ptr(out.P), _ptr(out.G))) if planes else \
            (self.lib.hhgt_encode_text_async, (_ptr(out.G),))
        with torch.cuda.device(self.device):
            check(fn(self.h, _ptr(text), nbytes, (region or "").encode(), C.byref(out.layout), _ptr(cursor), int(max_lines), *mats,
                     _ptr(out.start), _ptr(out.stop), _ptr(out.ref), _ptr(out.alt), C.c_void_p(pending.buf.data_ptr()), _stream()))
            pending.event.record(torch.cuda.current_stream())
        return pending

    def encode_text_async(self, text, n_samples, out, cursor, max_lines=None, region="", pending=None):
        return self._encode_async(False, text, n_samples, out, cursor, max_lines, region, pending)

    def pad_tail_cursor(self, res, cursor):
        with torch.cuda.device(self.device):
            check(self.lib.hhgt_pad_tail_cursor(self.h, C.byref(res.layout), _ptr(cursor), _ptr(res.G), _stream()))

    def encode_text_planes_async(self, text, n_samples, out, cursor, max_lines=None, region="", pending=None):
        return self._encode_async(True, text, n_samples, out, cursor, max_lines, region, pending)

    def pad_tail_planes_cursor(self, res, cursor):
        with torch.cuda.device(self.device):
            check(self.lib.hhgt_pad_tail_planes_cursor(self.h, C.byref(res.layout), _ptr(cursor), _ptr(res.P), _stream()))

    def pad_tail_planes(self, res, v_end, vcol_begin=0, vcol_end=None):
        lay = res.layout
        if vcol_end is None:
            vcol_end = -(-max(v_end, 1) // _geometry(lay).Vc)
        with torch.cuda.device(self.device):
            check(self.lib.hhgt_pad_tail_planes(self.h, C.byref(lay), int(v_end), int(vcol_begin), int(vcol_end), _ptr(res.P), _stream()))

    def compress_planes(self, res, col0=0, n_cols=None, fmt=BLOSC2, dst=None, chunk_off=None, sync=True):
        lay = res.layout
        Vc, Sc, n_vc, n_sc = _geometry(lay)
        if n_cols is None:
            n_cols = n_vc - col0
        n_chunks = n_cols * n_sc
        chunk_nbytes = Sc * Vc * 2
        with torch.cuda.device(self.device):
            cap = int(self.lib.hhgt_compress_bound(n_chunks, chunk_nbytes, 2, 8192))
            if dst is None:
                dst = torch.empty(cap, dtype=torch.uint8, device=self.device)
            if chunk_off is None:
                chunk_off = torch.zeros(n_chunks + 1, dtype=torch.int64, device=self.device)
            total = C.c_uint64(0)
            check(self.lib.hhgt_compress_planes(self.h, C.byref(lay), _ptr(res.P), _ptr(res.G), int(col0), int(n_cols), fmt, _ptr(dst),
                                                dst.numel(), _ptr(chunk_off), C.byref(total) if sync else None, _stream()))
        return dst, chunk_off, (int(total.value) if sync else None)

    def planes_expand(self, res, col0=0, n_cols=None, out=None):
        lay = res.layout
        if n_cols is None:
            n_cols = _geometry(lay).n_vc - col0
        with torch.cuda.device(self.device):
            if out is None:
                out = torch.zeros(layout_bytes(lay), dtype=torch.uint8, device=self.device)
            check(self.lib.hhgt_planes_expand(self.h, C.byref(lay), _ptr(res.P), _ptr(res.G), int(col0), int(n_cols), _ptr(out), _stream()))
        return out

    def chrom_runs(self):
        n = C.c_uint32(0)
        check(self.lib.hhgt_encode_chrom_runs(self.h, 0, None, None, C.byref(n)))
        if n.value == 0:
            return []
        first = np.zeros(n.value, np.uint64)
        names = np.zeros((n.value, 32), np.uint8)
        check(self.lib.hhgt_encode_chrom_runs(self.h, n.value, first.ctypes.data, names.ctypes.data, C.byref(n)))
        return [(int(first[i]), bytes(names[i]).rstrip(b"\0").decode()) for i in range(n.value)]

    def pad_tail(self, res, v_end=None, vcol_begin=0, vcol_end=None):
        lay = res.layout
        v_end = res.n_kept if v_end is None else v_end
        if vcol_end is None:
            vcol_end = -(-max(v_end, 1) // _geometry(lay).Vc)
        with torch.cuda.device(self.device):
            check(self.lib.hhgt_pad_tail(self.h, C.byref(lay), int(v_end), int(vcol_begin), int(vcol_end),
                                         _ptr(res.G), _stream()))

    def create_stream(self, kind):
        h = C.c_void_p()
        check(self.lib.hhgt_stream_create(self.h, {"encode": 0, "compress": 1, "frame": 2}[kind], C.byref(h)))
        self._streams = getattr(self, "_streams", [])
        self._streams.append(h)
        return torch.cuda.ExternalStream(h.value, device=self.device)

    def set_frame_stream(self, stream):
        check(self.lib.hhgt_set_frame_stream(self.h, C.c_void_p(stream.cuda_stream) if stream is not None else None))

    def set_keep_multiallelic(self, on=True):
        check(self.lib.hhgt_set_keep_multiallelic(self.h, 1 if on else 0))

    def set_index_mode(self, mode):
        check(self.lib.hhgt_set_index_mode(self.h, int(mode)))

    def set_clevel(self, clevel):
        check(self.lib.hhgt_set_clevel(self.h, int(clevel)))
        self.clevel = int(clevel)

    def compress(self, src, chunk_nbytes, typesize=DEFAULT_TYPESIZE, blocksize=None, fmt=BLOSC2,
                 dst=None, chunk_off=None, sync=True):
        assert src.is_cuda and src.dtype == torch.uint8 and src.is_contiguous()
        chunk_nbytes = int(chunk_nbytes)
        assert src.numel() % chunk_nbytes == 0
        n_chunks = src.numel() // chunk_nbytes
        if blocksize is None:
            blocksize = _default_blocksize(chunk_nbytes, typesize)
        with torch.cuda.device(self.device):
            cap = int(self.lib.hhgt_compress_bound(n_chunks, chunk_nbytes, typesize, blocksize))
            if cap == 0:
                check(-1)
            if dst is None:
                dst = torch.empty(cap, dtype=torch.uint8, device=self.device)
            if chunk_off is None:
                chunk_off = torch.zeros(n_chunks + 1, dtype=torch.int64, device=self.device)
            total = C.c_uint64(0)
            check(self.lib.hhgt_compress_chunks(self.h, _ptr(src), n_chunks, chunk_nbytes, typesize, blocksize,
                                                fmt, _ptr(dst), dst.numel(), _ptr(chunk_off),
                                                C.byref(total) if sync else None, _stream()))
        return dst, chunk_off, (int(total.value) if sync else None)

    def decompress(self, src, chunk_off, n_chunks, chunk_nbytes, typesize=DEFAULT_TYPESIZE, blocksize=None,
                   dst=None):
        if blocksize is None:
            blocksize = _default_blocksize(chunk_nbytes, typesize)
        with torch.cuda.device(self.device):
            if dst is None:
                dst = torch.empty(int(n_chunks) * int(chunk_nbytes), dtype=torch.uint8, device=self.device)
            bad = C.c_uint64(0)
            check(self.lib.hhgt_decompress_chunks(self.h, _ptr(src), _ptr(chunk_off), int(n_chunks),
                                                  int(chunk_nbytes), typesize, blocksize, _ptr(dst),
                                                  C.byref(bad), _stream()))
        return dst, int(bad.value)

    def decompress_blocks(self, sel, chunk_nbytes, typesize=DEFAULT_TYPESIZE, blocksize=None, dst=None):
        if blocksize is None:
            blocksize = _default_blocksize(chunk_nbytes, typesize)
        sel = np.ascontiguousarray(sel, dtype=SEL_DTYPE)
        n = len(sel)
        with torch.cuda.device(self.device):
            if dst is None:
                size = int((sel["dst_off"] + sel["hi"] - sel["lo"]).max()) if n else 0
                dst = torch.empty(size, dtype=torch.uint8, device=self.device)
            d_sel = torch.from_numpy(sel.view(np.uint8)).to(self.device) if n else None
            bad = C.c_uint64(0)
            check(self.lib.hhgt_decompress_blocks(self.h, _ptr(d_sel), n, int(chunk_nbytes), typesize, blocksize,
                                                  _ptr(dst), C.byref(bad), _stream()))
        return dst, int(bad.value)

    def _vmask_arg(self, vmask):
        if vmask is None:
            return None, 0
        if not torch.is_tensor(vmask):
            vmask = torch.from_numpy(np.ascontiguousarray(vmask, dtype=np.uint32).view(np.int32))
        vmask = vmask.to(self.device)
        if vmask.dtype not in (torch.int32, torch.uint32) or vmask.dim() != 1 or not vmask.is_contiguous():
            raise ValueError("vmask: contiguous uint32 words (store.pack_variant_mask)")
        words = vmask.numel()
        if words == 0:
            vmask = torch.zeros(1, dtype=torch.int32, device=self.device)
        return vmask, words

    def _row_kernel(self, fn, sel, sc, vc, typesize, blocksize, out, *args):
        n = len(sel)
        with torch.cuda.device(self.device):
            d_sel = torch.from_numpy(sel.view(np.uint8)).to(self.device) if n else None
            bad = C.c_uint64(0)
            check(fn(self.h, _ptr(d_sel), n, int(sc), int(vc), typesize, blocksize, *args, C.byref(bad), _stream()))
        return out, int(bad.value)

    @staticmethod
    def _row_sel(sel, sel_dtype, vc, blocksize):
        if blocksize is None:
            blocksize = _default_blocksize(int(vc) * 2)
        return np.ascontiguousarray(sel, dtype=sel_dtype), blocksize

    def _out_arg(self, tensor, dtype, shape, name, loose=()):
        if tensor is None:
            return torch.zeros(shape, dtype=dtype, device=self.device)
        same = tensor.dim() == len(shape) and all(a == b for i, (a, b) in enumerate(zip(tensor.shape, shape)) if i not in loose)
        if tensor.dtype not in ((dtype, torch.uint32) if dtype == torch.int32 else (dtype,)) or not same or not tensor.is_contiguous():
            raise ValueError(f"{name}: a contiguous {str(dtype).split('.')[1]} tensor {list(shape)}")
        return tensor

    def _counts_arg(self, counts, n_out):
        if counts is None:
            counts = torch.zeros((int(n_out()), 4), dtype=torch.int32, device=self.device)
        if (counts.dtype not in (torch.int32, torch.uint32) or counts.dim() != 2 or counts.shape[1] != 4
                or not counts.is_contiguous()):
            raise ValueError("counts: a contiguous int32 tensor [n_out, 4]")
        return counts

    def count_alleles(self, sel, sc, vc, n_out=None, typesize=DEFAULT_TYPESIZE, blocksize=None, counts=None):
        sel, blocksize = self._row_sel(sel, COUNT_SEL_DTYPE, vc, blocksize)
        with torch.cuda.device(self.device):
            counts = self._counts_arg(counts, lambda: n_out if n_out is not None else
                                      int((sel["out_row"] + sel["hi"] - sel["lo"]).max()) if len(sel) else 0)
            return self._row_kernel(self.lib.hhgt_count_alleles, sel, sc, vc, typesize, blocksize, counts,
                                    _ptr(counts), counts.shape[0])

    def count_samples(self, sel, sc, vc, n_out=None, typesize=DEFAULT_TYPESIZE, blocksize=None, vmask=None, counts=None):
        sel, blocksize = self._row_sel(sel, SAMPLE_SEL_DTYPE, vc, blocksize)
        with torch.cuda.device(self.device):
            counts = self._counts_arg(counts, lambda: n_out if n_out is not None else
                                      int(sel["out_row"].max()) + int(sc) if len(sel) else 0)
            vmask, words = self._vmask_arg(vmask)
            return self._row_kernel(self.lib.hhgt_count_samples, sel, sc, vc, typesize, blocksize, counts,
                                    _ptr(vmask), words, _ptr(counts), counts.shape[0])

    def genotype_planes(self, sel, sc, vc, n_rows=None, row_words=None, typesize=DEFAULT_TYPESIZE, blocksize=None,
                        vmask=None, planes=None):
        sel, blocksize = self._row_sel(sel, PLANE_SEL_DTYPE, vc, blocksize)
        n = len(sel)
        with torch.cuda.device(self.device):
            if planes is None:
                if n_rows is None:
                    n_rows = int(sel["out_row"].max()) + int(sc) if n else 0
                if row_words is None:
                    row_words = int(sel["out_word"].max()) + -(-(int(blocksize) // 2) // 32) if n else 0
                planes = torch.zeros((3, int(n_rows), int(row_words)), dtype=torch.int32, device=self.device)
            n_rows, row_words = _planes_arg(planes)
            vmask, words = self._vmask_arg(vmask)
            return self._row_kernel(self.lib.hhgt_genotype_planes, sel, sc, vc, typesize, blocksize, planes,
                                    _ptr(vmask), words, _ptr_if_any(planes), n_rows, row_words)

    def gather_calls(self, sel, sc, vc, values=None, out=None, n_rows=None, n_cols=None, row_map=None, vmask=None,
                     typesize=DEFAULT_TYPESIZE, blocksize=None):
        sel, blocksize = self._row_sel(sel, GATHER_SEL_DTYPE, vc, blocksize)
        n, raw = len(sel), values is None
        with torch.cuda.device(self.device):
            if not raw:
                if (not torch.is_tensor(values) or values.dtype not in GATHER_DTYPES or values.dim() != 2 or values.shape[0] != 4
                        or not values.is_contiguous() or not values.is_cuda):
                    raise ValueError("values: a contiguous device tensor [4, n_cols] of an 8, 16, 32 or 64 bit type")
                if n_cols is not None and int(n_cols) != values.shape[1]:
                    raise ValueError(f"n_cols {int(n_cols)} with a table of {values.shape[1]} columns")
                n_cols = int(values.shape[1])
            if row_map is not None:
                if not torch.is_tensor(row_map):
                    row_map = torch.from_numpy(np.ascontiguousarray(row_map, dtype=np.uint32).view(np.int32))
                row_map = row_map.to(self.device)
                if row_map.dtype not in (torch.int32, torch.uint32) or row_map.dim() != 1 or not row_map.is_contiguous():
                    raise ValueError("row_map: contiguous uint32 output rows")
            dtype, tail = (torch.int8, (2,)) if raw else (values.dtype, ())
            if out is None:
                if n_rows is None:
                    n_rows = (0 if not n else int(sel["out_row"].max()) + int(sc) if row_map is None else
                              int(row_map.view(torch.int32).max()) + 1 if row_map.numel() else 0)
                if n_cols is None:
                    n_cols = int((sel["out_col"] + sel["hi"] - sel["lo"]).max()) if n else 0
                out = torch.zeros((int(n_rows), int(n_cols)) + tail, dtype=dtype, device=self.device)
            want = f"out: a {str(dtype).split('.')[1]} device tensor [n_rows, row_stride{', 2' if raw else ''}] with dense rows"
            if (not torch.is_tensor(out) or out.dtype != dtype or out.dim() != 2 + len(tail) or tuple(out.shape[2:]) != tail
                    or not out.is_cuda or (n_rows is not None and int(n_rows) != out.shape[0])):
                raise ValueError(want)
            unit = 2 if raw else 1
            n_cols = int(out.shape[1]) if n_cols is None else int(n_cols)
            stride = out.stride(0) // unit if out.shape[0] > 1 else int(out.shape[1])
            dense = out.stride(-1) == 1 and (not raw or out.stride(1) == 2) and (out.shape[0] <= 1 or out.stride(0) % unit == 0)
            if not dense or n_cols > out.shape[1] or stride < out.shape[1]:
                raise ValueError(want + f" of at least {n_cols} columns")
            vmask, words = self._vmask_arg(vmask)
            return self._row_kernel(self.lib.hhgt_gather_calls, sel, sc, vc, typesize, blocksize, out, _ptr(vmask), words,
                                    _ptr(row_map), 0 if row_map is None else row_map.numel(), _ptr(values),
                                    2 if raw else values.element_size(), _ptr_if_any(out), out.shape[0], n_cols, stride)

    def pair_counts(self, planes, w_lo=0, w_hi=None, table=None):
        n, words, w_lo, w_hi = _plane_words(planes, w_lo, w_hi)
        with torch.cuda.device(self.device):
            table = self._out_arg(table, torch.int32, (n, n, 4), "table")
            check(self.lib.hhgt_pair_counts(self.h, _ptr_if_any(planes), n, words, w_lo, w_hi, _ptr_if_any(table), _stream()))
        return table

    def grm(self, planes, z, w_lo=0, w_hi=None, table=None):
        n, words, w_lo, w_hi = _plane_words(planes, w_lo, w_hi)
        if z.dtype != torch.float32 or tuple(z.shape) != (3, 32 * words) or not z.is_contiguous() or z.device != planes.device:
            raise ValueError(f"z: a contiguous float32 tensor [3, {32 * words}] on the planes' device")
        with torch.cuda.device(self.device):
            table = self._out_arg(table, torch.float64, (n, n), "table")
            check(self.lib.hhgt_grm(self.h, _ptr_if_any(planes), n, words, w_lo, w_hi, _ptr_if_any(z), _ptr_if_any(table),
                                    _stream()))
        return table

    def variant_planes(self, planes, w_lo=0, w_hi=None, vplanes=None):
        n, words, w_lo, w_hi = _plane_words(planes, w_lo, w_hi)
        with torch.cuda.device(self.device):
            shape = (3, 32 * max(w_hi - w_lo, 0), -(-n // 32))
            if vplanes is None:
                vplanes = torch.empty(shape, dtype=torch.int32, device=self.device)
            vplanes = self._out_arg(vplanes, torch.int32, shape, "vplanes")
            check(self.lib.hhgt_variant_planes(self.h, _ptr_if_any(planes), n, words, w_lo, w_hi, _ptr_if_any(vplanes), _stream()))
        return vplanes

    def ld_counts(self, vplanes, window, table=None):
        (n, sw), window = _planes_arg(vplanes, "vplanes: a contiguous int32 tensor [3, n_var, sw]"), int(window)
        if not 0 <= window < 1 << 32:
            raise ValueError(f"window {window}")
        with torch.cuda.device(self.device):
            if table is None:
                table = torch.zeros((n, max(min(window, 1024), 1), 8), dtype=torch.int32, device=self.device)
            table = self._out_arg(table, torch.int32, (n, window, 8), "table", loose=() if 1 <= window <= 1024 else (1,))
            check(self.lib.hhgt_ld_counts(self.h, _ptr_if_any(vplanes), n, sw, window, _ptr_if_any(table), _stream()))
        return table

    def assoc_sums(self, vplanes, w, sums=None):
        n, sw = _planes_arg(vplanes, "vplanes: a contiguous int32 tensor [3, n_var, sw]")
        n_cols = _weights_arg(w, (32 * sw,), vplanes)
        with torch.cuda.device(self.device):
            if sums is None:
                sums = torch.empty((n, 3, n_cols), dtype=torch.float64, device=self.device)
            sums = self._out_arg(sums, torch.float64, (n, 3, n_cols), "sums")
            check(self.lib.hhgt_assoc_sums(self.h, _ptr_if_any(vplanes), n, sw, _ptr_if_any(w), n_cols, _ptr_if_any(sums),
                                           _stream()))
        return sums

    def logistic_fit(self, vplanes, valid, X, y, beta0, out=None):
        n, sw = _planes_arg(vplanes, "vplanes: a contiguous int32 tensor [3, n_var, sw]")
        q = _weights_arg(X, (32 * sw,), vplanes)
        if (valid.dtype not in (torch.int32, torch.uint32) or tuple(valid.shape) != (sw,) or not valid.is_contiguous()
                or valid.device != vplanes.device):
            raise ValueError(f"valid: a contiguous int32 tensor [{sw}] on the planes' device")
        for name, t, shape in (("y", y, (32 * sw,)), ("beta0", beta0, (q,))):
            if t.dtype != torch.float64 or tuple(t.shape) != shape or not t.is_contiguous() or t.device != vplanes.device:
                raise ValueError(f"{name}: a contiguous float64 tensor {list(shape)} on the planes' device")
        with torch.cuda.device(self.device):
            if out is None:
                out = torch.empty((n, 9), dtype=torch.float64, device=self.device)
            out = self._out_arg(out, torch.float64, (n, 9), "out")
            check(self.lib.hhgt_logistic_fit(self.h, _ptr_if_any(vplanes), n, sw, _ptr_if_any(valid), _ptr_if_any(X), q,
                                             _ptr_if_any(y), _ptr(beta0), _ptr_if_any(out), _stream()))
        return out

    def score_sums(self, planes, w, w_lo=0, w_hi=None, sums=None):
        n, words, w_lo, w_hi = _plane_words(planes, w_lo, w_hi)
        n_cols = _weights_arg(w, (3, 32 * words), planes)
        with torch.cuda.device(self.device):
            sums = self._out_arg(sums, torch.float64, (n, n_cols), "sums")
            if sums.device != planes.device:
                raise ValueError("sums: on the planes' device")
            check(self.lib.hhgt_score_sums(self.h, _ptr_if_any(planes), n, words, w_lo, w_hi, _ptr_if_any(w), n_cols,
                                           _ptr_if_any(sums), _stream()))
        return sums

    def ld_prune(self, table, r2, keep=None):
        if (table.dtype not in (torch.int32, torch.uint32) or table.dim() != 3 or table.shape[2] != 8
                or table.shape[0] < table.shape[1] or not table.is_contiguous()):
            raise ValueError("table: a contiguous int32 tensor [window + n, window, 8]")
        window = int(table.shape[1])
        n = int(table.shape[0]) - window
        with torch.cuda.device(self.device):
            keep = self._out_arg(keep, torch.uint8, (window + n,), "keep")
            check(self.lib.hhgt_ld_prune(self.h, _ptr_if_any(table), n, window, float(r2), _ptr_if_any(keep), _stream()))
        return keep

    def ld_decisions(self, table, r2, pos=None, max_dist=None, bits=None):
        if (table.dtype not in (torch.int32, torch.uint32) or table.dim() != 3 or table.shape[2] != 8
                or table.shape[0] < table.shape[1] or table.shape[1] < 1 or not table.is_contiguous()):
            raise ValueError("table: a contiguous int32 tensor [window + n, window, 8]")
        window = int(table.shape[1])
        n = int(table.shape[0]) - window
        if (pos is None) != (max_dist is None):
            raise ValueError("pos and max_dist: both or neither")
        if pos is not None and (pos.dtype != torch.int64 or tuple(pos.shape) != (window + n,) or not pos.is_contiguous()
                                or pos.device != table.device):
            raise ValueError(f"pos: a contiguous int64 tensor [{window + n}] on the table's device")
        if max_dist is not None and not 0 <= int(max_dist) < 1 << 63:
            raise ValueError(f"max_dist {max_dist} (at least 0)")
        with torch.cuda.device(self.device):
            shape = (n, -(-window // 64))
            if bits is None:
                bits = torch.empty(shape, dtype=torch.int64, device=self.device)
            bits = self._out_arg(bits, torch.int64, shape, "bits")
            check(self.lib.hhgt_ld_decisions(self.h, _ptr_if_any(table), n, window, float(r2), None if pos is None else _ptr(pos),
                                             0 if max_dist is None else int(max_dist), _ptr_if_any(bits), _stream()))
        return bits

    def ld_clump(self, bits, window, rank, eligible, owner=None):
        window = int(window)
        if not 0 <= window < 1 << 32:
            raise ValueError(f"window {window}")
        nq = -(-max(min(window, 1024), 1) // 64)
        if bits.dtype != torch.int64 or bits.dim() != 2 or bits.shape[1] != nq or not bits.is_contiguous():
            raise ValueError(f"bits: a contiguous int64 tensor [n, {nq}]")
        n = int(bits.shape[0])
        for name, t, dtypes in (("rank", rank, (torch.int32, torch.uint32)), ("eligible", eligible, (torch.uint8, torch.bool))):
            if t.dtype not in dtypes or tuple(t.shape) != (n,) or not t.is_contiguous() or t.device != bits.device:
                raise ValueError(f"{name}: a contiguous {str(dtypes[0]).split('.')[1]} tensor [{n}] on the bits' device")
        rounds = C.c_uint32(0)
        with torch.cuda.device(self.device):
            if owner is None:
                owner = torch.empty((n,), dtype=torch.int32, device=self.device)
            owner = self._out_arg(owner, torch.int32, (n,), "owner")
            check(self.lib.hhgt_ld_clump(self.h, _ptr_if_any(bits), n, window, _ptr_if_any(rank), _ptr_if_any(eligible),
                                         _ptr_if_any(owner), C.byref(rounds), _stream()))
        return owner, int(rounds.value)

    def inflate_bgzf(self, raw, return_status=False, check_crc=True):
# ... 86 lines not shown
```

### include/hhgt.h

```cpp
#ifndef HHGT_H
#define HHGT_H
#include <stddef.h>
#include <stdint.h>

#ifdef __cplusplus
extern "C" {
#endif

#define HHGT_OK 0
#define HHGT_ERR_ARG (-1)
#define HHGT_ERR_HIP (-2)
#define HHGT_ERR_CAPACITY (-3)
#define HHGT_ERR_MALFORMED (-4)
#define HHGT_ERR_LINE_DENSITY (-5)
#define HHGT_ERR_NO_DEVICE (-6)
#define HHGT_ERR_IO (-7)

#define HHGT_BLOSC1 1
#define HHGT_BLOSC2 2

typedef struct hhgt_ctx hhgt_ctx;

const char *hhgt_version(void);
const char *hhgt_last_error(void);
int hhgt_device_count(void);

int hhgt_ctx_create(int device, hhgt_ctx **out);
void hhgt_ctx_destroy(hhgt_ctx *ctx);

typedef struct {
    int32_t n_samples;
    int32_t sc;
    int32_t vc;
    int32_t ring;
    uint64_t v_capacity;
} hhgt_layout;

uint64_t hhgt_layout_bytes(const hhgt_layout *lay);
uint64_t hhgt_layout_offset(const hhgt_layout *lay, uint32_t s, uint64_t v);

typedef struct {
    uint64_t n_lines;
    uint64_t n_records;
    uint64_t n_kept;
    uint64_t n_drop_region;
    uint64_t n_drop_filter;
    uint64_t n_haploid_padded;
    uint64_t n_malformed;
    uint64_t n_general_lines;
    uint64_t n_chrom_runs;
} hhgt_encode_stats;

int hhgt_encode_text(hhgt_ctx *ctx, const void *d_text, uint64_t nbytes, const char *region,
                     const hhgt_layout *lay, uint64_t v_base, void *d_G, uint32_t *d_start,
                     uint32_t *d_stop, uint8_t *d_ref, uint8_t *d_alt, hhgt_encode_stats *stats,
                     void *stream);

#define HHGT_RESULT_RUNS 16
typedef struct {
    hhgt_encode_stats stats;
    uint64_t cursor_before, cursor_after;
    uint64_t n_lines_over;
    uint64_t err_density;
    uint64_t run_first[HHGT_RESULT_RUNS];
    char run_names[HHGT_RESULT_RUNS][32];
    uint64_t v_capacity;
    uint32_t done, reserved;
} hhgt_encode_result;

int hhgt_encode_text_async(hhgt_ctx *ctx, const void *d_text, uint64_t nbytes, const char *region,
                           const hhgt_layout *lay, uint64_t *d_cursor, uint32_t max_lines, void *d_G,
                           uint32_t *d_start, uint32_t *d_stop, uint8_t *d_ref, uint8_t *d_alt,
                           hhgt_encode_result *h_result, void *stream);
int hhgt_encode_result_status(const hhgt_encode_result *r);

int hhgt_encode_chrom_runs(hhgt_ctx *ctx, uint32_t max_runs, uint64_t *first_kept, char *names,
                           uint32_t *n_runs);

int hhgt_pad_tail(hhgt_ctx *ctx, const hhgt_layout *lay, uint64_t v_end, uint64_t vcol_begin,
                  uint64_t vcol_end, void *d_G, void *stream);
int hhgt_pad_tail_cursor(hhgt_ctx *ctx, const hhgt_layout *lay, const uint64_t *d_cursor, void *d_G, void *stream);

uint64_t hhgt_compress_bound(uint64_t n_chunks, uint64_t chunk_nbytes, int typesize, int blocksize);
int hhgt_set_clevel(hhgt_ctx *ctx, int clevel);
int hhgt_reserve(hhgt_ctx *ctx, uint64_t text_bytes, uint32_t max_lines, uint64_t n_chunks, uint64_t chunk_nbytes, int typesize,
                 int blocksize);
int hhgt_set_keep_multiallelic(hhgt_ctx *ctx, int on);
int hhgt_set_index_mode(hhgt_ctx *ctx, int mode);
int hhgt_compress_chunks(hhgt_ctx *ctx, const void *d_src, uint64_t n_chunks, uint64_t chunk_nbytes,
                         int typesize, int blocksize, int format, void *d_dst, uint64_t dst_cap,
                         uint64_t *d_chunk_off, uint64_t *total_bytes, void *stream);

int hhgt_decompress_chunks(hhgt_ctx *ctx, const void *d_src, const uint64_t *d_chunk_off,
                           uint64_t n_chunks, uint64_t chunk_nbytes, int typesize, int blocksize,
                           void *d_dst, uint64_t *n_bad, void *stream);

typedef struct {
    uint64_t src_ptr;
    uint64_t src_bytes;
    uint64_t dst_off;
    uint32_t block;
    uint32_t lo, hi;
    uint32_t reserved;
} hhgt_block_sel;
int hhgt_decompress_blocks(hhgt_ctx *ctx, const hhgt_block_sel *d_sel, uint32_t n_sel, uint64_t chunk_nbytes,
                           int typesize, int blocksize, void *d_dst, uint64_t *n_bad, void *stream);

typedef struct {
    uint64_t src_ptr;
    uint64_t src_bytes;
    uint64_t row_mask;
    uint64_t out_row;
    uint32_t part;
    uint32_t lo, hi;
    uint32_t reserved;
} hhgt_count_sel;
int hhgt_count_alleles(hhgt_ctx *ctx, const hhgt_count_sel *d_sel, uint32_t n_sel, uint32_t sc, uint32_t vc,
                       int typesize, int blocksize, uint32_t *d_counts, uint64_t n_out, uint64_t *n_bad, void *stream);

typedef struct {
    uint64_t src_ptr;
    uint64_t src_bytes;
    uint64_t row_mask;
    uint64_t out_row;
    uint64_t mask_word;
    uint32_t part;
    uint32_t lo, hi;
    uint32_t reserved;
} hhgt_sample_sel;
int hhgt_count_samples(hhgt_ctx *ctx, const hhgt_sample_sel *d_sel, uint32_t n_sel, uint32_t sc, uint32_t vc,
                       int typesize, int blocksize, const uint32_t *d_vmask, uint64_t vmask_words,
                       uint32_t *d_counts, uint64_t n_out, uint64_t *n_bad, void *stream);

typedef struct {
    uint64_t src_ptr;
    uint64_t src_bytes;
    uint64_t row_mask;
    uint64_t out_row;
    uint64_t mask_word;
    uint64_t out_word;
    uint32_t part;
    uint32_t lo, hi;
    uint32_t reserved;
} hhgt_plane_sel;
int hhgt_genotype_planes(hhgt_ctx *ctx, const hhgt_plane_sel *d_sel, uint32_t n_sel, uint32_t sc, uint32_t vc,
                         int typesize, int blocksize, const uint32_t *d_vmask, uint64_t vmask_words,
                         uint32_t *d_planes, uint64_t n_rows, uint64_t row_words, uint64_t *n_bad, void *stream);

typedef struct {
    uint64_t src_ptr;
    uint64_t src_bytes;
    uint64_t row_mask;
    uint64_t out_row;
    uint64_t mask_word;
    uint64_t out_col;
    uint32_t part;
    uint32_t lo, hi;
    uint32_t reserved;
} hhgt_gather_sel;
int hhgt_gather_calls(hhgt_ctx *ctx, const hhgt_gather_sel *d_sel, uint32_t n_sel, uint32_t sc, uint32_t vc,
                      int typesize, int blocksize, const uint32_t *d_vmask, uint64_t vmask_words,
                      const uint32_t *d_row_map, uint64_t n_map, const void *d_values, int elem_bytes,
                      void *d_out, uint64_t n_rows, uint64_t n_cols, uint64_t row_stride,
                      uint64_t *n_bad, void *stream);

int hhgt_pair_counts(hhgt_ctx *ctx, const uint32_t *d_planes, uint64_t n_rows, uint64_t row_words, uint64_t w_lo,
                     uint64_t w_hi, uint32_t *d_table, void *stream);

#define HHGT_GRM_SPAN 128
int hhgt_grm(hhgt_ctx *ctx, const uint32_t *d_planes, uint64_t n_rows, uint64_t row_words, uint64_t w_lo, uint64_t w_hi,
             const float *d_z, double *d_table, void *stream);

int hhgt_variant_planes(hhgt_ctx *ctx, const uint32_t *d_planes, uint64_t n_rows, uint64_t row_words, uint64_t w_lo,
                        uint64_t w_hi, uint32_t *d_vplanes, void *stream);

int hhgt_ld_counts(hhgt_ctx *ctx, const uint32_t *d_vplanes, uint64_t n_var, uint64_t sw, uint32_t window, uint32_t *d_table,
                   void *stream);

int hhgt_ld_prune(hhgt_ctx *ctx, const uint32_t *d_table, uint64_t n_var, uint32_t window, double r2, uint8_t *d_keep,
                  void *stream);

int hhgt_ld_decisions(hhgt_ctx *ctx, const uint32_t *d_table, uint64_t n_var, uint32_t window, double r2, const int64_t *d_pos,
                      int64_t max_dist, uint64_t *d_bits, void *stream);

int hhgt_ld_clump(hhgt_ctx *ctx, const uint64_t *d_bits, uint64_t n_var, uint32_t window, const uint32_t *d_rank,
                  const uint8_t *d_eligible, int32_t *d_owner, uint32_t *rounds, void *stream);

int hhgt_assoc_sums(hhgt_ctx *ctx, const uint32_t *d_vplanes, uint64_t n_var, uint64_t sw, const double *d_w, uint32_t n_cols,
                    double *d_sums, void *stream);

#define HHGT_SCORE_SLICE 1
#define HHGT_SCORE_SPAN 64
#define HHGT_SCORE_MAX_SPANS 65535
int hhgt_score_sums(hhgt_ctx *ctx, const uint32_t *d_planes, uint64_t n_rows, uint64_t row_words, uint64_t w_lo, uint64_t w_hi,
                    const double *d_w, uint32_t n_cols, double *d_sums, void *stream);

#define HHGT_LOGIT_MAX_COLS 15
#define HHGT_LOGIT_MAX_STEPS 25
#define HHGT_LOGIT_REC 9
#define HHGT_LOGIT_GAMMA 0
#define HHGT_LOGIT_HINV 1
#define HHGT_LOGIT_U0 2
#define HHGT_LOGIT_HINV0 3
#define HHGT_LOGIT_STEPS 4
#define HHGT_LOGIT_STATUS 5
#define HHGT_LOGIT_N_COMPLETE 6
#define HHGT_LOGIT_N_HET 7
#define HHGT_LOGIT_N_ALT 8
#define HHGT_LOGIT_TESTED 0
#define HHGT_LOGIT_NO_CALL 1
#define HHGT_LOGIT_ONE_CLASS 2
#define HHGT_LOGIT_COLLINEAR 3
#define HHGT_LOGIT_NOT_CONVERGED 4
int hhgt_logistic_fit(hhgt_ctx *ctx, const uint32_t *d_vplanes, uint64_t n_var, uint64_t sw, const uint32_t *d_valid,
                      const double *d_x, uint32_t q, const double *d_y, const double *d_beta0, double *d_out, void *stream);

uint64_t hhgt_planes_bytes(const hhgt_layout *lay);
int hhgt_encode_text_planes_async(hhgt_ctx *ctx, const void *d_text, uint64_t nbytes, const char *region,
                                  const hhgt_layout *lay, uint64_t *d_cursor, uint32_t max_lines, void *d_P, void *d_G,
                                  uint32_t *d_start, uint32_t *d_stop, uint8_t *d_ref, uint8_t *d_alt,
                                  hhgt_encode_result *h_result, void *stream);
int hhgt_pad_tail_planes_cursor(hhgt_ctx *ctx, const hhgt_layout *lay, const uint64_t *d_cursor, void *d_P, void *stream);
int hhgt_pad_tail_planes(hhgt_ctx *ctx, const hhgt_layout *lay, uint64_t v_end, uint64_t vcol_begin, uint64_t vcol_end,
                         void *d_P, void *stream);
int hhgt_compress_planes(hhgt_ctx *ctx, const hhgt_layout *lay, const void *d_P, const void *d_G, uint32_t col0, uint32_t n_cols,
                         int format, void *d_dst, uint64_t dst_cap, uint64_t *d_chunk_off, uint64_t *total_bytes,
                         void *stream);
int hhgt_planes_expand(hhgt_ctx *ctx, const hhgt_layout *lay, const void *d_P, const void *d_G, uint32_t col0, uint32_t n_cols,
                       void *d_out, void *stream);

typedef struct {
    uint64_t ref_ptr;
    uint64_t ref_len;
    int64_t win_start;
    uint64_t var_start_ptr;
    uint64_t var_ref_ptr;
    uint64_t var_alt_ptr;
    uint64_t geno_ptr;
    uint32_t geno_first;
    uint32_t var_lo, var_hi;
    uint32_t reserved;
} hhgt_window;

int hhgt_onehot_windows(hhgt_ctx *ctx, const hhgt_window *d_items, uint32_t n_items, uint32_t seq_len,
                        const uint8_t *lut, int n_channels, float *d_hap1, float *d_hap2, void *stream);

int hhgt_onehot_bases_u8(hhgt_ctx *ctx, const uint8_t *d_bases, uint64_t n, const uint8_t *lut, int n_channels,
                         uint8_t *d_out, void *stream);

int hhgt_bgzf_scan(const void *host, uint64_t nbytes, uint64_t max_members, uint64_t *comp_off, uint32_t *comp_len,
                   uint32_t *isize, uint32_t *crc32 , uint64_t *n_members, uint64_t *consumed);
int hhgt_inflate_members(hhgt_ctx *ctx, const void *d_src, uint64_t src_bytes, const uint64_t *d_comp_off,
                         const uint32_t *d_comp_len, const uint64_t *d_out_off, const uint32_t *d_isize,
                         uint64_t n_members, void *d_dst, uint64_t dst_bytes, const uint32_t *d_crc32 ,
                         uint32_t *d_status, uint64_t *n_bad, void *stream);

#define HHGT_STAGE_INDEX 0
#define HHGT_STAGE_FIXED 1
#define HHGT_STAGE_ENCODE 2
#define HHGT_STAGE_GENERAL 3
#define HHGT_STAGE_LZ4 4
#define HHGT_STAGE_FRAME 5
#define HHGT_STAGE_DECODE 6
#define HHGT_STAGE_ONEHOT 7
#define HHGT_STAGE_INFLATE 8
#define HHGT_STAGE_PAIRS 9
#define HHGT_STAGE_LD_TRANSPOSE 10
#define HHGT_STAGE_LD 11
#define HHGT_STAGE_LD_PRUNE 12
#define HHGT_STAGE_LD_WALK 13
#define HHGT_STAGE_GRM 14
#define HHGT_STAGE_ASSOC 15
#define HHGT_N_STAGES 16
int hhgt_profile_enable(hhgt_ctx *ctx, int on);
int hhgt_profile_reset(hhgt_ctx *ctx);
int hhgt_profile_read(hhgt_ctx *ctx, double *ms , uint64_t *launches );

#define HHGT_STREAM_ENCODE 0
#define HHGT_STREAM_COMPRESS 1
#define HHGT_STREAM_FRAME 2
int hhgt_stream_create(hhgt_ctx *ctx, int kind, void **stream);
int hhgt_stream_destroy(hhgt_ctx *ctx, void *stream);
int hhgt_set_frame_stream(hhgt_ctx *ctx, void *stream);

#ifdef __cplusplus
}
#endif
#endif
```

Before: 170.9 million.

## Add eight-line batched walk step to newline index kernel with DPP group reductions

Reworks the batched walk in the newline-index kernel into a templated step that can cover eight lines per wavefront, using 8-lane groups instead of four 16-lane groups when line lengths are steady and headers are short. Cross-lane min, or and prefix-sum now use DPP, and per-region counts move from a register readlane scheme to shared memory. The wave count per launch and waves_per_eu occupancy hints are also tuned. Optional counters record how many lines each path handled, plus a new mode that forces four-line steps. The aim is to cut per-line serial work in the index stage, at the cost of more complex chaining logic and new fallback edge cases.

```diff
diff --git a/haplohyped_varawareml_amd/_lib.py b/haplohyped_varawareml_amd/_lib.py
--- a/haplohyped_varawareml_amd/_lib.py
+++ b/haplohyped_varawareml_amd/_lib.py
@@ -108,6 +108,7 @@
     "hhgt_reserve": (_i32, [_vp, _u64, _u32, _u64, _u64, _i32, _i32]),
     "hhgt_set_keep_multiallelic": (_i32, [_vp, _i32]),
     "hhgt_set_index_mode": (_i32, [_vp, _i32]),
+    "hhgt_index_walk_counts": (_i32, [_vp, _pu64]),
     "hhgt_stream_create": (_i32, [_vp, _i32, C.POINTER(_vp)]),
     "hhgt_stream_destroy": (_i32, [_vp, _vp]),
     "hhgt_set_frame_stream": (_i32, [_vp, _vp]),
diff --git a/haplohyped_varawareml_amd/csrc/api.hip b/haplohyped_varawareml_amd/csrc/api.hip
--- a/haplohyped_varawareml_amd/csrc/api.hip
+++ b/haplohyped_varawareml_amd/csrc/api.hip
@@ -435,12 +435,12 @@
 }
 
 static int encode_stage_index(hhgt_ctx *c, const uint8_t *text, uint64_t nbytes, uint32_t n_regions, uint32_t min_line, uint32_t S,
-                              DevCounters *cnt, hipStream_t st)
+                              bool count_walk, DevCounters *cnt, hipStream_t st)
 {
     EncodeWs &w = c->enc;
     TRY(w.ensure_index(n_regions, st));
     return launch_index_newlines(text, nbytes, w.slots.as<uint32_t>(), w.counts.as<uint32_t>(), w.region_tot.as<uint32_t>(), n_regions,
-                                 min_line, S, c->index_mode, cnt, st);
+                                 min_line, S, c->index_mode, count_walk, cnt, st);
 }
 
 static int encode_stage_rest(hhgt_ctx *c, const uint8_t *text, uint64_t nbytes, uint32_t n_regions, uint32_t max_lines,
@@ -607,7 +607,7 @@
     TRY(encode_begin_clean(c, cnt, st));
     const uint32_t n_regions = index_regions(nbytes);
     if (nbytes) {
-        TRY(timed(c, st, HHGT_STAGE_INDEX, [&] { return encode_stage_index(c, text, nbytes, n_regions, L.S ? 2u * L.S + 17u : 0u, L.S, cnt, st); }));
+        TRY(timed(c, st, HHGT_STAGE_INDEX, [&] { return encode_stage_index(c, text, nbytes, n_regions, L.S ? 2u * L.S + 17u : 0u, L.S, false, cnt, st); }));
         TRY(encode_stage_rest(c, text, nbytes, n_regions, max_lines, rf, L, d_cursor, d_G, planes ? d_P : nullptr, d_start, d_stop, d_ref,
                               d_alt, cnt, st));
     }
@@ -692,6 +692,7 @@
     hipStream_t st = reinterpret_cast<hipStream_t>(stream);
     HIP_TRY(hipSetDevice(c->device));
     if (stats) memset(stats, 0, sizeof(*stats));
+    c->walk_counts[0] = c->walk_counts[1] = c->walk_counts[2] = 0;
     LayoutDev L;
     RegionFilter rf;
     TRY(encode_check_args(c, d_text, nbytes, lay, &L, region, &rf, d_G));
@@ -708,13 +709,15 @@
     uint32_t n_lines = 0;
     {
         StageTimer t(c, st, HHGT_STAGE_INDEX);
-        TRY(encode_stage_index(c, text, nbytes, n_regions, L.S ? 2u * L.S + 17u : 0u, L.S, cnt, st));
+        TRY(encode_stage_index(c, text, nbytes, n_regions, L.S ? 2u * L.S + 17u : 0u, L.S, true, cnt, st));
         std::vector<uint32_t> totals(chain_groups(n_regions));
         c->h_counters->err_density = 0;
         HIP_TRY(hipMemcpyAsync(totals.data(), c->enc.region_tot.p, totals.size() * 4, hipMemcpyDeviceToHost, st));
         HIP_TRY(hipMemcpyAsync(&c->h_counters->err_density, &cnt->err_density, 8, hipMemcpyDeviceToHost, st));
+        HIP_TRY(hipMemcpyAsync(c->h_counters->walk_lines, cnt->walk_lines, sizeof(cnt->walk_lines), hipMemcpyDeviceToHost, st));
         HIP_TRY(hipStreamSynchronize(st));
         t.stop();
+        for (int k = 0; k < 3; ++k) c->walk_counts[k] = c->h_counters->walk_lines[k];
         for (uint32_t x : totals) n_lines += x;
         if (c->h_counters->err_density) {
             hhgt_set_error("encode: more than %u newlines inside one %u-byte region (not VCF text)", INDEX_CAP,
@@ -1016,11 +1019,18 @@
 
 extern "C" int hhgt_set_index_mode(hhgt_ctx *c, int mode)
 {
-    if (!c || mode < -1 || mode > 2) {
-        hhgt_set_error("index mode must be -1 (default), 0 (scan), 1 (hop) or 2 (walk)");
+    if (!c || mode < -1 || mode > 3) {
+        hhgt_set_error("index mode must be -1 (default), 0 (scan), 1 (hop), 2 (walk) or 3 (walk, four-line steps only)");
         return HHGT_ERR_ARG;
     }
     c->index_mode = mode;
+    return HHGT_OK;
+}
+
+extern "C" int hhgt_index_walk_counts(hhgt_ctx *c, uint64_t *out)
+{
+    if (!c || !out) return HHGT_ERR_ARG;
+    for (int k = 0; k < 3; ++k) out[k] = c->walk_counts[k];
     return HHGT_OK;
 }
 
diff --git a/haplohyped_varawareml_amd/csrc/common.h b/haplohyped_varawareml_amd/csrc/common.h
--- a/haplohyped_varawareml_amd/csrc/common.h
+++ b/haplohyped_varawareml_amd/csrc/common.h
@@ -99,7 +99,7 @@
     unsigned long long err_lines;
     unsigned long long cursor_after;
     unsigned long long n_other;
-    unsigned long long pad[3];
+    unsigned long long walk_lines[3];
 };
 
 #define MAX_CHROM_RUNS 4096u
@@ -296,6 +296,7 @@
     int clevel = 5;
     int keep_multi = 0;
     int index_mode = -1;
+    uint64_t walk_counts[3] = {0, 0, 0};
     bool counters_clean = false;
     int profiling = 0;
     double stage_ms[HHGT_N_STAGES] = {0};
@@ -322,7 +323,7 @@
 size_t scan_tmp_elems(uint64_t n);
 
 int launch_index_newlines(const uint8_t *d_text, uint64_t n, uint32_t *d_slots, uint32_t *d_counts, uint32_t *d_region_tot,
-                          uint32_t n_regions, uint32_t min_line, uint32_t S, int mode, DevCounters *d_cnt, hipStream_t st);
+                          uint32_t n_regions, uint32_t min_line, uint32_t S, int mode, bool count_walk, DevCounters *d_cnt, hipStream_t st);
 int index_mode_default();
 int launch_compact_newlines(const uint32_t *d_slots, const uint32_t *d_counts, const uint32_t *d_region_tot,
                             uint32_t n_regions, uint32_t *d_nl, uint32_t max_lines, uint32_t *d_nlines, hipStream_t st);
diff --git a/haplohyped_varawareml_amd/csrc/index.hip b/haplohyped_varawareml_amd/csrc/index.hip
--- a/haplohyped_varawareml_amd/csrc/index.hip
+++ b/haplohyped_varawareml_amd/csrc/index.hip
@@ -1,4 +1,6 @@
 #include "common.h"
+#include "walk_window.h"
+#include <type_traits>
 
 typedef uint32_t u32x4_unaligned __attribute__((ext_vector_type(4), aligned(1)));
 typedef uint32_t u32x4_t __attribute__((ext_vector_type(4)));
@@ -106,16 +108,68 @@
 #ifndef WALK_BATCH
 #define WALK_BATCH 1
 #endif
+#ifdef WALK_MARKS
+#define WALK_MARK(name) asm volatile("; ==MARK " name)
+#else
+#define WALK_MARK(name)
+#endif
+
+template <uint32_t LPG>
+__device__ __forceinline__ uint32_t group_min(uint32_t x)
+{
+    uint32_t t;
+    t = (uint32_t)__builtin_amdgcn_update_dpp(0, (int)x, 0xB1, 0xf, 0xf, false);
+    x = t < x ? t : x;
+    t = (uint32_t)__builtin_amdgcn_update_dpp(0, (int)x, 0x4E, 0xf, 0xf, false);
+    x = t < x ? t : x;
+    t = (uint32_t)__builtin_amdgcn_update_dpp(0, (int)x, 0x141, 0xf, 0xf, false);
+    x = t < x ? t : x;
+    if (LPG == 16u) {
+        t = (uint32_t)__builtin_amdgcn_update_dpp(0, (int)x, 0x140, 0xf, 0xf, false);
+        x = t < x ? t : x;
+    }
+    return x;
+}
+
+template <uint32_t LPG>
+__device__ __forceinline__ uint32_t group_or(uint32_t x)
+{
+    x |= (uint32_t)__builtin_amdgcn_update_dpp(0, (int)x, 0xB1, 0xf, 0xf, false);
+    x |= (uint32_t)__builtin_amdgcn_update_dpp(0, (int)x, 0x4E, 0xf, 0xf, false);
+    x |= (uint32_t)__builtin_amdgcn_update_dpp(0, (int)x, 0x141, 0xf, 0xf, false);
+    if (LPG == 16u) x |= (uint32_t)__builtin_amdgcn_update_dpp(0, (int)x, 0x140, 0xf, 0xf, false);
+    return x;
+}
+
+template <uint32_t LPG>
+__device__ __forceinline__ uint32_t group_scan_sum(uint32_t x, uint32_t lane)
+{
+    x += (uint32_t)__builtin_amdgcn_update_dpp(0, (int)x, 0x111, 0xf, 0xf, false);
+    x += (uint32_t)__builtin_amdgcn_update_dpp(0, (int)x, 0x112, 0xf, 0xf, false);
+    x += (uint32_t)__builtin_amdgcn_update_dpp(0, (int)x, 0x114, 0xf, 0xf, false);
+    x += (uint32_t)__builtin_amdgcn_update_dpp(0, (int)x, 0x118, 0xf, 0xf, false);
+    if (LPG == 8u) {
+        const uint32_t low = (uint32_t)__builtin_amdgcn_update_dpp(0, (int)x, 0x157, 0xf, 0xf, false);
+        x -= (lane & 8u) ? low : 0u;
+    }
+    return x;
+}
+#ifndef WALK_WAVES
+#define WALK_WAVES 4096u
+#endif
 #ifndef WALK_PF
 #define WALK_PF 0
 #endif
 template <int U, bool WALK>
-__global__ __launch_bounds__(256) void k_index_hop(const uint8_t *__restrict__ text, uint64_t n, uint32_t *__restrict__ slots,
+__global__ __launch_bounds__(256) __attribute__((amdgpu_waves_per_eu(5))) void k_index_hop(const uint8_t *__restrict__ text, uint64_t n, uint32_t *__restrict__ slots,
                                                    uint32_t *__restrict__ counts, uint32_t *__restrict__ region_tot, uint32_t n_regions,
-                                                   uint32_t skip, uint32_t S, DevCounters *cnt, uint32_t HOP_K)
+                                                   uint32_t skip, uint32_t S, DevCounters *cnt, uint32_t HOP_K, uint32_t opts)
 {
     HHGT_WAVE_PRIO();
+    __shared__ uint32_t s_cnt[4][64];
     const uint32_t lane = threadIdx.x & 63u;
+    uint32_t *const my_cnt = s_cnt[threadIdx.x >> 6];
+    my_cnt[lane] = 0u;
     const uint32_t w = (uint32_t)__builtin_amdgcn_readfirstlane((int)(blockIdx.x * 4u + (threadIdx.x >> 6)));
     const uint32_t r_first = w * HOP_K;
     if (r_first >= n_regions) return;
@@ -125,7 +179,6 @@
     uint64_t endw = beg + (uint64_t)r_cnt * INDEX_REGION;
     if (endw > n + 1) endw = n + 1;
     const uint64_t last_term = virt ? n : n - 1;
-    uint32_t cntv = 0;
     bool overflow = false;
     uint64_t pos = beg;
     uint64_t cand = 0, fb = 0;
@@ -133,121 +186,159 @@
     uint64_t est_len = 0, pf_wb = 0;
     bool pf_valid = false;
     u32x4_t pf = u32x4_t{0u, 0u, 0u, 0u};
+    uint32_t n_one = 0, n_four = 0, n_eight = 0;
     auto record = [&](uint64_t q) {
+        WALK_MARK("record");
         const uint32_t rr = (uint32_t)(q / INDEX_REGION), local = rr - r_first;
-        const uint32_t c = (uint32_t)__builtin_amdgcn_readlane((int)cntv, (int)local);
-        if (c < INDEX_CAP) {
-            if (lane == 0) slots[(size_t)rr * INDEX_CAP + c] = (uint32_t)q;
-        } else
-            overflow = true;
-        cntv += lane == local ? 1u : 0u;
+        if (lane == 0) {
+            const uint32_t c = my_cnt[local];
+            my_cnt[local] = c + 1u;
+            if (c < INDEX_CAP) slots[(size_t)rr * INDEX_CAP + c] = (uint32_t)q;
+            else overflow = true;
+        }
+        ++n_one;
+        WALK_MARK("record_end");
     };
     bool no_batch = false, bat_off = false;
     uint32_t bat_fail = 0;
     uint64_t head_p = 0;
     bool cand_batch = false;
     bool rehead = false;
+    uint32_t head_len = ~0u;
+    bool steady = false;
+    const bool narrow_ok = (opts & 1u) == 0u;
+    auto batch_step = [&](auto GC) -> bool {
+        constexpr uint32_t G = decltype(GC)::value, LPG = walk_lanes(G), WIN = walk_bytes(G), FRONT = walk_front(G);
+        constexpr unsigned long long LEAD = G == 8u ? 0x0101010101010101ull : 0x0001000100010001ull;
+        WALK_MARK("step");
+        const uint32_t g = lane / LPG, li = lane % LPG, l0 = 16u * li;
+        const uint32_t L0 = (uint32_t)est_len;
+        const uint64_t base = cand - FRONT;
+        const int64_t dlen = (int64_t)(4ull * S) - (int64_t)est_len;
+        const int32_t d32 = dlen > -65536 && dlen < 65536 ? (int32_t)dlen : 0x7FFFFFFF;
+        const uint32_t limit = endw <= base ? 0u : (endw - base > 0xFFFFFFFFull ? 0xFFFFFFFFu : (uint32_t)(endw - base));
+        const u32x4_t v = *reinterpret_cast<const u32x4_unaligned *>(text + walk_load_offset(cand, L0, G, lane));
+        const uint32_t nlm = eq_mask16(v, 0x0A0A0A0Au), tbm = eq_mask16(v, 0x09090909u);
+        const uint32_t pw = (uint32_t)__builtin_amdgcn_update_dpp(0, (int)v.w, 0x111, 0xf, 0xf, false);
+        const uint32_t jn = (uint32_t)__builtin_ctz(nlm | 0x10000u);
+        const uint32_t ib = (jn - 1u) & 15u, iq = ib >> 2;
+        const uint32_t dq = iq == 0u ? v.x : (iq == 1u ? v.y : (iq == 2u ? v.z : v.w));
+        const uint32_t bprev = jn == 0u ? pw >> 24 : (dq >> (8u * (ib & 3u))) & 0xFFu;
+        const uint32_t crbit = bprev == '\r' && l0 + jn != 0u ? 1u : 0u;
+        const uint32_t oc = group_min<LPG>(nlm != 0u ? ((l0 + jn) << 1) | crbit : 0x20000u);
+        const uint32_t o = oc >> 1;
+        const uint32_t keep = l0 > o ? 0xFFFFu : (l0 + 15u <= o ? 0u : (0xFFFFu << (o - l0 + 1u)) & 0xFFFFu);
+        const uint32_t tk = tbm & keep, tc = (uint32_t)__popc(tk);
+        const uint32_t incl = group_scan_sum<LPG>(tc, lane);
+        const uint32_t cum = incl - tc;
+        const bool has9 = cum < 9u && incl >= 9u;
+        uint32_t m9 = tk;
+        const uint32_t r1 = 8u - cum;
+#pragma unroll
+        for (uint32_t i = 0; i < 8u; ++i) m9 = i < r1 ? (m9 & (m9 - 1u)) : m9;
+        const uint32_t j9 = (uint32_t)__builtin_ctz(m9 | 0x10000u) & 15u;
+        const uint32_t ptb = (uint32_t)__builtin_amdgcn_update_dpp(0, (int)tbm, 0x111, 0xf, 0xf, false);
+        const uint32_t tb20 = (tbm << 4) | (ptb >> 12);
+        const bool tab8 = ((tb20 >> (j9 + 1u)) & 1u) != 0u;
+        const uint32_t ix = j9 + 2u, di = ix >> 2;
+        const uint32_t w0 = di == 0u ? pw : (di == 1u ? v.x : (di == 2u ? v.y : (di == 3u ? v.z : v.w)));
+        const uint32_t w1 = di == 0u ? v.x : (di == 1u ? v.y : (di == 2u ? v.z : v.w));
+        const uint32_t gt2 = __builtin_amdgcn_alignbyte(w1, w0, ix & 3u) & 0xFFFFu;
+        const bool ok9 = has9 && tab8 && gt2 == 0x5447u;
+        const uint32_t t9 = l0 + j9;
+        const uint32_t o_next = (uint32_t)__builtin_amdgcn_ds_bpermute((int)(((lane + LPG) & 63u) << 2), (int)o);
+        const bool link = ok9 && (int32_t)(o_next - t9) == d32;
+        const uint32_t f = group_or<LPG>(((nlm & keep) != 0u ? 1u : 0u) | (ok9 ? 2u | (t9 << 8) : 0u) | (link ? 4u : 0u) | (has9 ? 16u : 0u));
+        const bool v_nl = o < WIN && (oc & 1u) == 0u && (g != 0u || o == FRONT);
+        const uint32_t verdicts = (v_nl ? 1u : 0u) | (v_nl && g * L0 + o < limit ? 2u : 0u) | (f & 4u) | ((f & 3u) == 2u ? 8u : 0u);
+        const unsigned long long vb = __builtin_amdgcn_ballot_w64(((verdicts >> li) & 1u) != 0u);
+        WALK_MARK("chain");
+        const unsigned long long nl8 = vb & LEAD, in8 = (vb >> 1) & LEAD, link8 = (vb >> 2) & LEAD, head8 = (vb >> 3) & LEAD;
+        const unsigned long long at8 = nl8 & ((link8 << LPG) | 1ull);
+        const unsigned long long bad = ~(at8 & in8 & head8) & LEAD;
+        const uint32_t n_rec = bad != 0ull ? (uint32_t)__builtin_ctzll(bad) / LPG : G;
+        if (G == 8u) n_eight += n_rec;
+        else n_four += n_rec;
+        WALK_MARK("store");
+        if (n_rec != 0u) {
+            const uint64_t q = base + (uint64_t)(g * L0 + o);
+            const uint32_t rr = (uint32_t)(q / INDEX_REGION);
+            const uint32_t rr_i = (uint32_t)__builtin_amdgcn_ds_bpermute((int)(((li * LPG) & 63u) << 2), (int)rr);
+            const unsigned long long same = __builtin_amdgcn_ballot_w64(li < n_rec && rr_i == rr);
+            const uint32_t mine = (uint32_t)(same >> (LPG * g)) & ((1u << G) - 1u);
+            if (li == 0u && g < n_rec) {
+                const uint32_t local = rr - r_first;
+                const uint32_t c = my_cnt[local] + (uint32_t)__popc(mine & ((1u << g) - 1u));
+                if ((mine >> (g + 1u)) == 0u) my_cnt[local] = c + 1u;
+                if (c < INDEX_CAP) slots[(size_t)rr * INDEX_CAP + c] = (uint32_t)q;
+                else overflow = true;
+            }
+        }
+        WALK_MARK("tail");
+        uint64_t expected = cand, fbx = fb, exp_head = head_p;
+        bool exp_batch = cand_batch;
+        if (n_rec != 0u) {
+            const int lj = (int)(LPG * (n_rec - 1u));
+            const uint32_t oj = (uint32_t)__builtin_amdgcn_readlane((int)o, lj), t9j = (uint32_t)__builtin_amdgcn_readlane((int)f, lj) >> 8;
+            const uint64_t wj = base + (uint64_t)(n_rec - 1u) * L0;
+            const uint64_t soff = wj + t9j + 1ull;
+            exp_head = wj + oj;
+            exp_batch = true;
+            expected = soff + 4ull * S - 1ull;
+            fbx = soff + 2ull * S - 17ull;
+            est_len = expected - exp_head;
+            head_len = t9j - oj;
+            steady = est_len == (uint64_t)L0;
+        }
+        bool handed = false, cand_bad = false;
+        if (n_rec < G) {
+            const uint32_t bit = LPG * n_rec;
+            handed = true;
+            if (((at8 >> bit) & 1ull) == 0ull) {
+                cand_bad = n_rec == 0u;
+            } else if (((in8 >> bit) & 1ull) == 0ull) {
+                return true;
+            } else if (G == 4u || ((uint32_t)__builtin_amdgcn_readlane((int)f, (int)bit) & 17u) != 0u) {
+                have_cand = false;
+                pos = expected;
+                expected = ~0ull;
+            }
+        }
+        if (expected != ~0ull) {
+            if (expected > last_term) {
+                have_cand = false;
+                pos = fbx;
+                if (pos > last_term) pos = last_term;
+            } else {
+                cand = expected;
+                fb = fbx > last_term ? last_term : fbx;
+                have_cand = true;
+            }
+            head_p = exp_head;
+            cand_batch = exp_batch;
+        }
+        if (G == 8u) {
+            no_batch = cand_bad;
+            if (handed && !cand_bad) steady = false;
+            bat_fail = n_rec != 0u ? 0u : (cand_bad ? bat_fail + 1u : bat_fail);
+        } else {
+            no_batch = handed;
+            bat_fail = n_rec != 0u ? 0u : bat_fail + 1u;
+        }
+        bat_off = bat_fail >= 2u;
+        WALK_MARK("step_end");
+        return false;
+    };
     while (have_cand || pos < endw) {
-        if (WALK && WALK_BATCH && have_cand && !no_batch && !bat_off && est_len != 0ull && cand >= 40ull && cand + 3ull * est_len + 216ull <= n) {
-            const uint32_t g = lane >> 4, li = lane & 15u;
-            const uint64_t L0 = est_len;
-            const uint8_t *wbase = text + (cand - 40ull);
-            const uint64_t voff = (uint64_t)g * L0 + 16ull * li;
-            const u32x4_t v = *reinterpret_cast<const u32x4_unaligned *>(wbase + voff);
-            const uint32_t nlm = eq_mask16(v, 0x0A0A0A0Au), tbm = eq_mask16(v, 0x09090909u);
-            const unsigned long long nlb = __builtin_amdgcn_ballot_w64(nlm != 0u);
-            uint32_t og[4];
-            bool vg[4];
-#pragma unroll
-            for (int k = 0; k < 4; ++k) {
-                const uint32_t mg = (uint32_t)(nlb >> (16 * k)) & 0xFFFFu;
-                vg[k] = mg != 0u;
-                const int fl = 16 * k + __builtin_ctz(mg | 0x10000u);
-                og[k] = 16u * ((uint32_t)fl & 15u) + (uint32_t)__builtin_ctz((uint32_t)__builtin_amdgcn_readlane((int)nlm, fl & 63) | 0x10000u);
-            }
-            const uint32_t o = g == 0u ? og[0] : (g == 1u ? og[1] : (g == 2u ? og[2] : og[3]));
-            const uint32_t l0 = 16u * li;
-            const uint32_t keep = l0 > o ? 0xFFFFu : (l0 + 15u <= o ? 0u : (0xFFFFu << (o - l0 + 1u)) & 0xFFFFu);
-            const unsigned long long nl2 = __builtin_amdgcn_ballot_w64((nlm & keep) != 0u);
-            const uint32_t tk = tbm & keep, tc = (uint32_t)__popc(tk);
-            uint32_t incl = tc;
-            incl += (uint32_t)__builtin_amdgcn_update_dpp(0, (int)incl, 0x111, 0xf, 0xf, false);
-            incl += (uint32_t)__builtin_amdgcn_update_dpp(0, (int)incl, 0x112, 0xf, 0xf, false);
-            incl += (uint32_t)__builtin_amdgcn_update_dpp(0, (int)incl, 0x114, 0xf, 0xf, false);
-            incl += (uint32_t)__builtin_amdgcn_update_dpp(0, (int)incl, 0x118, 0xf, 0xf, false);
-            const uint32_t cum = incl - tc;
-            const bool has9 = cum < 9u && incl >= 9u;
-            uint32_t m9 = tk;
-            const uint32_t r1 = 8u - cum;
-#pragma unroll
-            for (uint32_t i = 0; i < 8u; ++i) m9 = i < r1 ? (m9 & (m9 - 1u)) : m9;
-            const uint32_t j9 = (uint32_t)__builtin_ctz(m9 | 0x10000u) & 15u;
-            const uint32_t pw = (uint32_t)__builtin_amdgcn_update_dpp(0, (int)v.w, 0x111, 0xf, 0xf, false);
-            const uint32_t ptb = (uint32_t)__builtin_amdgcn_update_dpp(0, (int)tbm, 0x111, 0xf, 0xf, false);
-            const uint32_t tb20 = (tbm << 4) | (ptb >> 12);
-            const bool tab8 = ((tb20 >> (j9 + 1u)) & 1u) != 0u;
-            const uint32_t ix = j9 + 2u, di = ix >> 2;
-            const uint32_t w0 = di == 0u ? pw : (di == 1u ? v.x : (di == 2u ? v.y : (di == 3u ? v.z : v.w)));
-            const uint32_t w1 = di == 0u ? v.x : (di == 1u ? v.y : (di == 2u ? v.z : v.w));
-            const uint32_t gt2 = __builtin_amdgcn_alignbyte(w1, w0, ix & 3u) & 0xFFFFu;
-            const bool ok9 = has9 && tab8 && gt2 == 0x5447u;
-            const uint32_t t9 = l0 + j9;
-            const unsigned long long b9 = __builtin_amdgcn_ballot_w64(ok9);
-            uint64_t expected = cand, fbx = fb, exp_head = head_p;
-            bool exp_batch = cand_batch;
-            bool stop = false, handed = false;
-            uint32_t advanced = 0;
-#pragma unroll
-            for (int k = 0; k < 4; ++k) {
-                if (stop || handed) continue;
-                const uint64_t nlpos = cand - 40ull + (uint64_t)k * L0 + og[k];
-                const bool cr = vg[k] && og[k] != 0u && head_byte(v, 256u * (uint32_t)k + og[k] - 1u) == '\r';
-                if (!vg[k] || nlpos != expected || cr) {
-                    handed = true;
-                    continue;
-                }
-                exp_head = expected;
-                exp_batch = true;
-                if (expected >= endw) {
-                    stop = true;
-                    continue;
-                }
-                const uint32_t bits = (uint32_t)(b9 >> (16 * k)) & 0xFFFFu;
-                if (bits == 0u || ((nl2 >> (16 * k)) & 0xFFFFull) != 0ull) {
-                    have_cand = false;
-                    pos = expected;
-                    handed = true;
-                    expected = ~0ull;
-                    continue;
-                }
-                record(expected);
-                ++advanced;
-                const int l9 = 16 * k + __builtin_ctz(bits);
-                const uint32_t t9s = (uint32_t)__builtin_amdgcn_readlane((int)t9, l9);
-                const uint64_t soff = cand - 40ull + (uint64_t)k * L0 + t9s + 1ull;
-                const uint64_t nxt = soff + 4ull * S - 1ull;
-                est_len = nxt - expected;
-                expected = nxt;
-                fbx = soff + 2ull * S - 17ull;
-            }
-            if (stop) break;
-            if (expected != ~0ull) {
-                if (expected > last_term) {
-                    have_cand = false;
-                    pos = fbx;
-                    if (pos > last_term) pos = last_term;
-                } else {
-                    cand = expected;
-                    fb = fbx > last_term ? last_term : fbx;
-                    have_cand = true;
-                }
-                head_p = exp_head;
-                cand_batch = exp_batch;
-            }
-            no_batch = handed;
-            bat_fail = advanced ? 0u : bat_fail + 1u;
-            bat_off = bat_fail >= 2u;
-            continue;
+        if (WALK && WALK_BATCH && have_cand && !no_batch && !bat_off) {
+            if (walk_step_lines(narrow_ok, steady, head_len) == 8u && walk_fits(cand, est_len, n, 8u)) {
+                if (batch_step(std::integral_constant<uint32_t, 8u>{})) break;
+                continue;
+            }
+            if (walk_fits(cand, est_len, n, 4u)) {
+                if (batch_step(std::integral_constant<uint32_t, 4u>{})) break;
+                continue;
+            }
         }
         no_batch = false;
         bool found = false, nb_have = false, have_head = false;
@@ -397,7 +488,9 @@
                                 cand = soff + 4ull * S - 1ull;
                                 fb = lo;
                                 have_cand = true;
+                                steady = est_len == cand - p;
                                 est_len = cand - p;
+                                head_len = t9 - ho;
                                 head_p = p;
                                 cand_batch = false;
                             } else {
@@ -418,7 +511,13 @@
         if (pos > last_term) pos = p + 1 > last_term ? p + 1 : last_term;
         if (have_cand && fb > last_term) fb = p + 1 > last_term ? p + 1 : last_term;
     }
-    if (overflow && lane == 0) atomicAdd(&cnt->err_density, 1ull);
+    if (__builtin_amdgcn_ballot_w64(overflow) != 0ull && lane == 0) atomicAdd(&cnt->err_density, 1ull);
+    if ((opts & 2u) != 0u && lane == 0) {
+        if (n_eight) atomicAdd(&cnt->walk_lines[0], (unsigned long long)n_eight);
+        if (n_four) atomicAdd(&cnt->walk_lines[1], (unsigned long long)n_four);
+        if (n_one) atomicAdd(&cnt->walk_lines[2], (unsigned long long)n_one);
+    }
+    const uint32_t cntv = my_cnt[lane];
     const uint32_t mine = lane < r_cnt ? (cntv < INDEX_CAP ? cntv : INDEX_CAP) : 0u;
     if (lane < r_cnt) counts[r_first + lane] = mine;
     const uint32_t g0 = r_first / CHAIN_GROUP;
@@ -772,7 +871,7 @@
         if (const char *e = getenv("HHGT_INDEX_HOP")) return atoi(e) ? 2 : 0;
         return 2;
     }();
-    return m < 0 ? 0 : (m > 2 ? 2 : m);
+    return m < 0 ? 0 : (m > 3 ? 2 : m);
 }
 
 static uint32_t index_hop_skip(uint32_t min_line, int mode)
@@ -782,17 +881,18 @@
 }
 
 int launch_index_newlines(const uint8_t *d_text, uint64_t n, uint32_t *d_slots, uint32_t *d_counts, uint32_t *d_region_tot,
-                          uint32_t n_regions, uint32_t min_line, uint32_t S, int mode, DevCounters *d_cnt, hipStream_t st)
+                          uint32_t n_regions, uint32_t min_line, uint32_t S, int mode, bool count_walk, DevCounters *d_cnt, hipStream_t st)
 {
     if (mode < 0) mode = index_mode_default();
     if (const uint32_t skip = index_hop_skip(min_line, mode)) {
         const bool walk = mode >= 2 && S > 0;
-        const uint32_t k_walk = (n_regions + 8191u) / 8192u;
+        const uint32_t k_walk = (n_regions + WALK_WAVES - 1u) / WALK_WAVES;
         uint32_t K = walk ? (k_walk < 6u ? 6u : k_walk) : 6u;
         K = K > 64u ? 64u : K;
+        const uint32_t opts = (mode == 3 ? 1u : 0u) | (count_walk ? 2u : 0u);
 #define HOP_LAUNCH(U, W)                                                                                                      \
     hipLaunchKernelGGL((k_index_hop<U, W>), dim3(((n_regions + K - 1) / K + 3) / 4), dim3(256), 0, st, d_text, n, d_slots, d_counts, \
-                       d_region_tot, n_regions, skip, S, d_cnt, K)
+                       d_region_tot, n_regions, skip, S, d_cnt, K, opts)
         if (min_line >= 4096u) {
             if (walk) HOP_LAUNCH(5, true);
             else HOP_LAUNCH(5, false);
diff --git a/haplohyped_varawareml_amd/csrc/walk_window.h b/haplohyped_varawareml_amd/csrc/walk_window.h
--- /dev/null
+++ b/haplohyped_varawareml_amd/csrc/walk_window.h
@@ -0,0 +1,31 @@
+#pragma once
+#include <stdint.h>
+
+#if defined(__HIPCC__) || defined(__CUDACC__)
+#define WALK_HD __host__ __device__
+#else
+#define WALK_HD
+#endif
+
+#define WALK_NARROW_HEAD 96u
+#define WALK_MAX_LINE (1ull << 28)
+
+WALK_HD constexpr uint32_t walk_lanes(uint32_t G) { return 64u / G; }
+WALK_HD constexpr uint32_t walk_bytes(uint32_t G) { return 16u * (64u / G); }
+WALK_HD constexpr uint32_t walk_front(uint32_t G) { return G == 8u ? 24u : 40u; }
+
+WALK_HD inline uint64_t walk_load_offset(uint64_t cand, uint64_t est_len, uint32_t G, uint32_t lane)
+{
+    return cand - walk_front(G) + (uint64_t)(lane / walk_lanes(G)) * est_len + 16ull * (lane % walk_lanes(G));
+}
+
+WALK_HD inline bool walk_fits(uint64_t cand, uint64_t est_len, uint64_t n, uint32_t G)
+{
+    return est_len != 0ull && est_len < WALK_MAX_LINE && cand >= walk_front(G) &&
+           cand + (uint64_t)(G - 1u) * est_len + (walk_bytes(G) - walk_front(G)) <= n;
+}
+
+WALK_HD inline uint32_t walk_step_lines(bool narrow_allowed, bool steady, uint32_t head_len)
+{
+    return narrow_allowed && steady && head_len <= WALK_NARROW_HEAD ? 8u : 4u;
+}
diff --git a/haplohyped_varawareml_amd/device.py b/haplohyped_varawareml_amd/device.py
--- a/haplohyped_varawareml_amd/device.py
+++ b/haplohyped_varawareml_amd/device.py
@@ -302,6 +302,11 @@
 
     def set_index_mode(self, mode):
         check(self.lib.hhgt_set_index_mode(self.h, int(mode)))
+
+    def index_walk_counts(self):
+        out = (C.c_uint64 * 3)()
+        check(self.lib.hhgt_index_walk_counts(self.h, out))
+        return tuple(int(x) for x in out)
 
     def set_clevel(self, clevel):
         check(self.lib.hhgt_set_clevel(self.h, int(clevel)))
diff --git a/include/hhgt.h b/include/hhgt.h
--- a/include/hhgt.h
+++ b/include/hhgt.h
@@ -87,6 +87,7 @@
                  int blocksize);
 int hhgt_set_keep_multiallelic(hhgt_ctx *ctx, int on);
 int hhgt_set_index_mode(hhgt_ctx *ctx, int mode);
+int hhgt_index_walk_counts(hhgt_ctx *ctx, uint64_t *out);
 int hhgt_compress_chunks(hhgt_ctx *ctx, const void *d_src, uint64_t n_chunks, uint64_t chunk_nbytes,
                          int typesize, int blocksize, int format, void *d_dst, uint64_t dst_cap,
                          uint64_t *d_chunk_off, uint64_t *total_bytes, void *stream);
```

Result: no change. 172.2 million, median of 6 (+0.8%).
